# tum-vision/dvo_slam

Hardware: AMD Instinct MI355X
Metric: frame-pair alignments/s (640x480, 4-level pyramid) + finest-level HBM GB/s vs roofline (higher is better)
Workload: dtype f32 (Gram operands exact f16 hi + lo pairs on every level, f32 accumulate); 1 GPU; 1024 pairs (BASELINE config 4): independent 640x480 RGB-D frame pairs, seeds 0..1023, pair i on rank i mod 1, 4-level pyramid, FirstLevel=3, LastLevel=0, MaxIterationsPerLevel=100, Precision=5e-7, Mu=0; step = every rank re-ingests the raw planes of its shard from HBM (pyramids, sampling planes, point selection) and aligns it as one batch; the build of step k+1 (build stream) overlaps the match of; pairs=1024, pairs_per_gpu=1024, width=640, height=480, lanes=1 lane

## Files before the change

dvo_slam_amd/csrc/align_small.hip:

```cpp
#include "fast_sweep.h"
#include "launch.h"

namespace dvo_hip {

constexpr int kSmallCells = 5376;
constexpr int kSmallLoads = kSmallCells / kBlock;

__global__ __launch_bounds__(kBlock, 3) void k_sweep_small(
    const LevelGeom g, const PairPtrs* __restrict__ pairs, const PairState* __restrict__ states, int n_pairs,
    float* __restrict__ partials, float2* __restrict__ scratch, int blocks_per_xcd, int rows_per_wave, int* __restrict__ f16_range_flag) {
  const int tiles = g.tiles_x * g.tiles_y;
  const int total = tiles * n_pairs;
  const int xcd = blockIdx.x & 7, slot = blockIdx.x >> 3;
  const int item = xcd * blocks_per_xcd + slot;
  if (item >= total) return;
  const int pair = item / tiles, tile = item - pair * tiles;
  const PairState& st = states[pair];
  if (!st.active || st.level != g.level) return;
  const PairPtrs pp = pairs[pair];
  __shared__ __attribute__((aligned(16))) float slab[4][kSlabFloatsF16];
  __shared__ __attribute__((aligned(16))) float2 img[kSmallCells];
  __shared__ int counts[4];
  const int lane = threadIdx.x & 63, wave = __builtin_amdgcn_readfirstlane(threadIdx.x >> 6);
  const int n_px = g.w * g.h, plane_bytes = n_px * 8;
  const __amdgpu_buffer_rsrc_t refR = __builtin_amdgcn_make_buffer_rsrc(const_cast<float2*>(pp.refR), 0, plane_bytes, 0x00020000);
  const __amdgpu_buffer_rsrc_t curC = __builtin_amdgcn_make_buffer_rsrc(const_cast<float2*>(pp.curC), 0, plane_bytes, 0x00020000);
  const __amdgpu_buffer_rsrc_t resid = __builtin_amdgcn_make_buffer_rsrc(scratch + size_t(pair) * size_t(n_px), 0, plane_bytes, 0x00020000);

  const int pitch = g.w + 2, cells = pitch * (g.h + 2);
  {
    const float inv_pitch = 1.0f / float(pitch);
    f32x2 v[kSmallLoads];
#pragma unroll
    for (int j = 0; j < kSmallLoads; ++j) {
      const int c = min(int(threadIdx.x) + j * kBlock, cells - 1);
      int cy = int(float(c) * inv_pitch);
      int cx = c - cy * pitch;
      if (cx < 0) { cx += pitch; cy -= 1; }
      if (cx >= pitch) { cx -= pitch; cy += 1; }
      const int x = min(max(cx - 1, 0), g.w - 1), y = min(max(cy - 1, 0), g.h - 1);
      v[j] = __builtin_bit_cast(f32x2, __builtin_amdgcn_raw_buffer_load_b64(curC, (y * g.w + x) * 8, 0, 0));
    }
#pragma unroll
    for (int j = 0; j < kSmallLoads; ++j) {
      const int c = int(threadIdx.x) + j * kBlock;
      if (c < cells) img[c] = make_float2(v[j].x, v[j].y);
    }
  }

  float KT[12];
#pragma unroll
  for (int i = 0; i < 12; ++i) KT[i] = st.KT[i];
  const FastWeights wt(st);
  const FastRcpSource no_table = {__builtin_amdgcn_make_buffer_rsrc(static_cast<float*>(nullptr), 0, 0, 0x00020000), nullptr, 0};
  const unsigned gram_entries = kGramEntryTable.e[min(int(threadIdx.x), kNumAcc - 1)];
  const unsigned w2_bits = __builtin_bit_cast(unsigned, float(g.w - 2)), h2_bits = __builtin_bit_cast(unsigned, float(g.h - 2));
  const float inv_w = 1.0f / float(g.w);
  const float nanv = __builtin_nanf("");
  const int segments = (n_px + kTileW - 1) / kTileW;
  const int seg0 = tile * (kWavesPerBlock * rows_per_wave) + wave;
  float* my = slab[wave];
  f32x4 acc0 = {0.0f, 0.0f, 0.0f, 0.0f}, acc1 = {0.0f, 0.0f, 0.0f, 0.0f};
  int n_valid = 0;
  auto load_f = [&](int pixel) { return __builtin_bit_cast(float, __builtin_amdgcn_raw_buffer_load_b32(refR, pixel * 8 + 4, 0, 0)); };
  struct Ref {
    float z, i, left, right, up, down, tx, ty;
  };
  auto load_ref = [&](int seg) {
    const int pc = min(seg * kTileW + lane, n_px - 1);
    int row = int(float(pc) * inv_w);
    int col = pc - row * g.w;
    if (col < 0) { col += g.w; row -= 1; }
    if (col >= g.w) { col -= g.w; row += 1; }
    Ref r;
    const f32x2 zi = __builtin_bit_cast(f32x2, __builtin_amdgcn_raw_buffer_load_b64(refR, pc * 8, 0, 0));
    r.z = zi.x; r.i = zi.y;
    r.left = load_f(pc - (col > 0 ? 1 : 0));
    r.right = load_f(pc + (col < g.w - 1 ? 1 : 0));
    r.up = load_f(pc - (row > 0 ? g.w : 0));
    r.down = load_f(pc + (row < g.h - 1 ? g.w : 0));
    r.tx = g.tx[col];
    r.ty = g.ty[row];
    return r;
  };
  __syncthreads();
  Ref next = load_ref(min(seg0, segments - 1));
#pragma unroll 1
  for (int k = 0; k < rows_per_wave; ++k) {
    const int seg = seg0 + k * kWavesPerBlock;
    if (seg >= segments) break;
    const Ref ref = next;
    if (k + 1 < rows_per_wave) next = load_ref(min(seg + kWavesPerBlock, segments - 1));
    const int idx = seg * kTileW + lane;
    const bool in_image = idx < n_px;
    const float z = in_image ? ref.z : nanv;
    const float tx = ref.tx, ty = ref.ty;
    float u, v, qz;
    fast_project<0>(g, no_table, KT, fmaf(KT[0], tx, KT[2]), fmaf(KT[4], tx, KT[6]), fmaf(KT[8], tx, KT[10]), z, tx, ty, u, v, qz);
    const unsigned long long ok_mask = __builtin_amdgcn_ballot_w64(__builtin_bit_cast(unsigned, u) <= w2_bits) &
                                       __builtin_amdgcn_ballot_w64(__builtin_bit_cast(unsigned, v) <= h2_bits);
    const bool ok = __builtin_amdgcn_inverse_ballot_w64(ok_mask);
    const int u0 = int(u), v0 = int(v);
    FastRow r;
    r.z = z; r.i = ref.i;
    r.gx = ref.right - ref.left;
    r.gy = ref.down - ref.up;
    r.qz = qz;
    r.a1 = __builtin_amdgcn_fractf(u);
    r.b1 = __builtin_amdgcn_fractf(v);
    r.idx = v0 * pitch + u0;
    f32x2 P[4][4];
    {
      FastLdsCellPtr q = (FastLdsCellPtr)(img + (ok ? r.idx : 0));
#pragma unroll
      for (int rr = 0; rr < 4; ++rr)
#pragma unroll
        for (int cc = 0; cc < 4; ++cc)
          if ((rr == 1 || rr == 2) || (cc == 1 || cc == 2)) P[rr][cc] = q[rr * pitch + cc];
    }
    fast_row_tail<2, false, 0, false>(g, no_table, P, r, ok_mask, tx, ty, fmaf(tx, tx, 1.0f), wt, resid, in_image ? idx * 8 : 0x7ffffff8, 0, my, lane, acc0, acc1, n_valid);
  }

#pragma unroll
  for (int i = 0; i < 4; ++i) {
    my[((lane >> 4) * 4 + i) * 16 + (lane & 15)] = acc0[i];
    my[256 + ((lane >> 4) * 4 + i) * 16 + (lane & 15)] = acc1[i];
  }
  if (lane == 0) counts[wave] = n_valid;
  __syncthreads();
  fast_epilogue(slab, counts, gram_entries, partials + (size_t(pair) * tiles + tile) * kAccStride, f16_range_flag ? f16_range_flag + pair : nullptr);
}

bool small_sweep_takes(int w, int h) {
  return w % 2 == 0 && w >= 4 && h >= 4 && (w + 2) * (h + 2) <= kSmallCells;
}

void launch_sweep_small(hipStream_t s, int rows_per_wave, const LevelGeom& g, const PairPtrs* pairs, const PairState* states, int n_pairs,
                        float* partials, float2* scratch, int* f16_range_flag) {
  const int total = g.tiles_x * g.tiles_y * n_pairs;
  const int per_xcd = (total + 7) / 8;
  k_sweep_small<<<dim3(per_xcd * 8), dim3(kBlock), 0, s>>>(g, pairs, states, n_pairs, partials, scratch, per_xcd, rows_per_wave, f16_range_flag);
}

}
```

dvo_slam_amd/csrc/batch_policy.h:

```cpp
#pragma once

namespace dvo_hip {

struct BatchPolicy {
  int cus;
  explicit BatchPolicy(int compute_units) : cus(compute_units > 0 ? compute_units : 256) {}

  int resident_direct_max_pairs() const { return cus / 16; }
  bool resident_takes_coarse_levels(int n) const { return n * 4 <= cus; }
  bool resident_first_level_fits(int n) const { return n * 2 * 8 <= cus * 7; }
  bool taps_missing_prefers_first_level_only(int n) const { return n * 8 >= cus; }
  bool ingest_skips_taps(int n_frames) const { return n_frames * 8 >= cus; }

  bool short_gather_tiles(int n) const { return n >= cus; }
  int min_workgroups(int n) const { return n <= cus / 32 ? 2 * cus : n * 4 < cus ? 4 * cus : 8 * cus; }
  bool level_hand_over(int n) const { return n <= cus; }
  bool fused_loglik_on_large_levels(int n) const { return n >= 2 * cus; }
  int loglik_blocks(int n) const { return n >= cus ? 8 : n * 16 >= cus * 3 ? 16 : 32; }
  int deferred_ingest_lead(int n) const { return n * 4 >= cus * 3 ? 7 : 3; }
  bool finish_launch(int n) const { return !level_hand_over(n); }
  bool solver_two_waves(int n) const { return n > 2 * cus; }

  int small_level_tiles(int n) const {
    const int t = (3 * cus + n / 2) / (n > 0 ? n : 1);
    return t < 3 ? 3 : t > 8 ? 8 : t;
  }

  int defer_ingest_max_pairs() const { return cus; }
  int background_build_workgroups() const { return cus; }
};

}
```

dvo_slam_amd/csrc/capi.hip:

```cpp
#include <hip/hip_runtime.h>
#ifdef DVO_WITH_ROCTX
#include <rocprofiler-sdk-roctx/roctx.h>
#endif
#include <xmmintrin.h>

#include <algorithm>
#include <functional>
#include <climits>
#include <cstddef>
#include <cmath>
#include <cstdio>
#include <atomic>
#include <chrono>
#include <thread>
#include <condition_variable>
#include <cstdlib>
#include <cstring>
#include <mutex>
#include <string>
#include <vector>

#include "../../include/dvo_hip.h"
#include "device_types.h"
#include "batch_policy.h"
// ... 344 lines not shown
    dvo_hip_config cfg;
    bool keep_raw_copy;
  };
  std::vector<DeferredIngest> deferred;
  int opt_defer_ingest = 0;
  int opt_defer_ingest_pixels = 0;
  int opt_keep_raw_copy = 1;
  long long deferred_ingests = 0;
  int opt_build_workgroups = 0;
  int opt_stream_policy = 1;
  int opt_tail_speculation = 0;
  int opt_solver_waves = 0;
  int opt_ll_blocks = 0;
  int opt_compact_residuals = 1;
  int opt_gram_lo_parts = 1;
  int opt_min_workgroups = 0;
  int opt_condition_number = 0;
  int opt_fused_ll_pixels = 0;
  float last_sel_ithr = 0.0f, last_sel_dthr = 0.0f;
  int f32_gram_hold = 0;
  long long warmup_wait_us = 0;
  int opt_variant = 8;
  int opt_resident = -1;
  int opt_resident_rows = 0;
  int opt_resident_group = 0;
  int resident_timeouts = 0;
  long long resident_launches = 0;
  long long resident_levels = 0;
  long long host_ns[4] = {0, 0, 0, 0};
  long long host_batches = 0;
  std::chrono::steady_clock::time_point batch_entry;
  int opt_resident_flags = 0;
  int opt_sweep_tail = 0;
  long long tail_steps = 0;
  int opt_overlap_tails = 0;
  int opt_overlap_fraction = 8;
  int opt_tail_lists = 0;
  long long listed_steps = 0;
  long long overlapped_tails = 0;
  long long overlapped_steps = 0;
  long long tail_drains = 0;
  long long tail_wait_ns = 0;
  int opt_batch_groups = 0;
  bool is_twin = false;
  std::vector<GroupWorker*> group_workers;
  hipEvent_t roles_ready = nullptr;
  long long grouped_batches = 0;
  int opt_small_sweep = 0;
  int opt_small_tiles = 0;
  int opt_coarse = 0;
  int opt_coarse_pixels = 0;
  int opt_coarse_wgs = 0;
  long long coarse_launches = 0, coarse_levels = 0;
  int opt_deterministic = 0;
  int opt_ref_compat = 0;
  int opt_ref_order = 0;
  long long ref_order_passes = 0;
  DevBuf ref_order_planes;
  DevBuf rcp_table;
  int rcp_shift = 0;
  int rcp_packed = 0;
  int opt_resident_cooperative = 0;
  int compute_units = 0;
  std::vector<CameraGeom*> cameras;
  struct PooledBlock { void* p; size_t bytes; };
  std::vector<PooledBlock> frame_pool;
  size_t frame_pool_bytes = 0;
  static constexpr size_t kFramePoolMaxBytes = size_t(1) << 30;
  static constexpr size_t kFramePoolMaxBlocks = 64;
  Workspace ws[1];
  DevBuf misc, role_tbl_cur, role_tbl_ref, prep_tbl_cur, prep_tbl_ref;
  DevBuf sel_tbl_main, sel_tbl_build;
  unsigned long long sel_visits = 0;
  DevBuf lens_tbl;
  DevBuf graph_jobs, graph_outs;
  DevBuf rig_tbl;
  DevBuf colour_tbl, colour_stage;
  DevBuf map_tbl, map_stage;
  DevBuf render_tbl, render_zbuf, render_planes;
  hipEvent_t render_done = nullptr;
  static const int kTableSlots = 4;
  DevBuf build_tbl[kTableSlots];
  DevBuf* build_tbl_cur = nullptr;
  unsigned build_tbl_next = 0;
  PinnedRing tables;
  std::vector<dvo_hip_frame*> build_tbl_frames;
  hipStream_t build_stream = nullptr;
  static const int kBuildRing = 16;
  hipEvent_t build_events[kBuildRing] = {};
  unsigned long long build_seq = 0;
  unsigned long long main_waited_seq = 0;
  hipStream_t upload_stream = nullptr;
  hipEvent_t upload_done = nullptr;
  static const int kUploadRing = 3;
  DevBuf upload_buf[kUploadRing];
  unsigned long long upload_buf_seq[kUploadRing] = {};
  unsigned upload_next = 0;
  unsigned long long upload_waited_seq = 0;
};

namespace {
int flush_deferred(dvo_hip_context* ctx);
}

#define DVO_FLUSH_DEFERRED(ctx)                                     \
  do {                                                              \
// ... 277 lines not shown
  if (!ctx) return;
  (void)hipSetDevice(ctx->device);
  ctx->deferred.clear();
  destroy_group_workers(ctx);
  if (ctx->upload_stream) (void)hipStreamSynchronize(ctx->upload_stream);
  if (ctx->build_stream) (void)hipStreamSynchronize(ctx->build_stream);
  for (Workspace& w : ctx->ws) workspace_destroy(w);
  if (ctx->upload_done) (void)hipEventDestroy(ctx->upload_done);
  if (ctx->upload_stream) (void)hipStreamDestroy(ctx->upload_stream);
  for (hipEvent_t ev : ctx->build_events)
    if (ev) (void)hipEventDestroy(ev);
  if (ctx->build_stream) (void)hipStreamDestroy(ctx->build_stream);
  for (DevBuf& b : ctx->build_tbl) b.release();
  for (DevBuf* b : {&ctx->misc, &ctx->role_tbl_cur, &ctx->role_tbl_ref, &ctx->prep_tbl_cur, &ctx->prep_tbl_ref, &ctx->rcp_table, &ctx->ref_order_planes,
                    &ctx->sel_tbl_main, &ctx->sel_tbl_build, &ctx->lens_tbl, &ctx->rig_tbl, &ctx->graph_jobs, &ctx->graph_outs, &ctx->map_tbl, &ctx->map_stage, &ctx->colour_tbl, &ctx->colour_stage, &ctx->render_tbl, &ctx->render_zbuf, &ctx->render_planes}) b->release();
  if (ctx->render_done) (void)hipEventDestroy(ctx->render_done);
  for (DevBuf& b : ctx->upload_buf) b.release();
  for (const dvo_hip_context::PooledBlock& b : ctx->frame_pool) (void)hipFree(b.p);
  ctx->frame_pool.clear();
  ctx->tables.release();
  for (CameraGeom* c : ctx->cameras) {
    c->tables.release();
    delete c;
  }
  delete ctx;
}

const char* dvo_hip_last_error(const dvo_hip_context* ctx) { return ctx ? ctx->err.c_str() : g_create_error.c_str(); }

void* dvo_hip_context_stream(dvo_hip_context* ctx) { return ctx ? static_cast<void*>(ctx->stream) : nullptr; }

int dvo_hip_context_device(const dvo_hip_context* ctx) { return ctx ? ctx->device : -1; }

#include "capi_options.inc"

namespace {

int check_prepare_args(dvo_hip_context* ctx, int n_frames, dvo_hip_frame* const* frames, int role, const dvo_hip_config* cfg, const char* who) {
  if (!ctx || n_frames < 1 || !frames || !cfg || (role != DVO_HIP_ROLE_CURRENT && role != DVO_HIP_ROLE_REFERENCE))
    return fail(ctx, DVO_HIP_ERR_INVALID, who, "bad argument");
  if (cfg->first_level < cfg->last_level || cfg->last_level < 0 || cfg->first_level >= kMaxLevels)
    return fail(ctx, DVO_HIP_ERR_INVALID, who, "need 0 <= last_level <= first_level < DVO_HIP_MAX_LEVELS");
  for (int i = 0; i < n_frames; ++i) {
    if (!frames[i]) return fail(ctx, DVO_HIP_ERR_INVALID, who, "null entry");
    if (frames[i]->cam != frames[0]->cam || frames[i]->levels <= cfg->first_level)
      return fail(ctx, DVO_HIP_ERR_INVALID, who, "frames must share the camera and have first_level + 1 levels");
  }
  return DVO_HIP_OK;
}

int prepare_roles(dvo_hip_context* ctx, int n_frames, dvo_hip_frame* const* frames, int role, const dvo_hip_config* cfg) {
  const bool ref = role == DVO_HIP_ROLE_REFERENCE;
  int want[kMaxLevels];
  for (int l = 0; l < kMaxLevels; ++l) want[l] = l < frames[0]->cam->levels ? eager_current_flavor(ctx, frames[0]->cam, l, n_frames) : kCurAB;
  float ithr = ref ? cfg->intensity_derivative_threshold : 0.0f, dthr = ref ? cfg->depth_derivative_threshold : 0.0f;
  std::vector<dvo_hip_frame*> speculative;
  if (ref && (ithr < 0.0f || dthr < 0.0f)) {
    ithr = ctx->last_sel_ithr; dthr = ctx->last_sel_dthr;
    for (int i = 0; i < n_frames; ++i) {
      bool any = false;
      for (int l = cfg->last_level; l <= cfg->first_level; ++l) any |= frames[i]->lv[l].selected;
      if (!any) speculative.push_back(frames[i]);
    }
    if (speculative.empty()) return DVO_HIP_OK;
    n_frames = int(speculative.size());
    frames = speculative.data();
  }
  const int rc = ensure_roles(ctx, n_frames, frames, ref ? 1 : 0, cfg->last_level, cfg->first_level, ithr, dthr, true, want);
  if (rc != DVO_HIP_OK) return rc;
  DVO_HIP_TRY(ctx, hipGetLastError());
  return DVO_HIP_OK;
}

}

#include "capi_ingest.inc"
#include "capi_map.inc"
#include "capi_colour.inc"
#include "capi_graph.inc"

int dvo_hip_upload_wait(dvo_hip_context* ctx) {
  DVO_ENTER(ctx);
  if (!ctx) return DVO_HIP_ERR_INVALID;
  DVO_HIP_TRY(ctx, hipSetDevice(ctx->device));
  DVO_HIP_TRY(ctx, hipStreamSynchronize(ctx->upload_stream));
  return DVO_HIP_OK;
}

int dvo_hip_host_alloc(dvo_hip_context* ctx, size_t bytes, void** out) {
  DVO_LOCK(ctx);
  if (!ctx || !out || bytes == 0) return fail(ctx, DVO_HIP_ERR_INVALID, "host_alloc: bad argument");
  DVO_HIP_TRY(ctx, hipSetDevice(ctx->device));
  DVO_HIP_TRY(ctx, hipHostMalloc(out, bytes, hipHostMallocDefault));
  return DVO_HIP_OK;
}

void dvo_hip_host_free(dvo_hip_context* ctx, void* p) {
  DVO_LOCK(ctx);
  if (!p) return;
  if (ctx) (void)hipSetDevice(ctx->device);
  (void)hipHostFree(p);
}

int dvo_hip_frames_prepare(dvo_hip_context* ctx, int n_frames, dvo_hip_frame* const* frames, int role, const dvo_hip_config* cfg) {
  DVO_ENTER(ctx);
  const int rc = check_prepare_args(ctx, n_frames, frames, role, cfg, "frames_prepare");
  if (rc != DVO_HIP_OK) return rc;
// ... 212 lines not shown
  for (int i = 0; i < n_frames; ++i) {
    frames[i]->rig_on = false;
    frames[i]->rig = dvo_hip_depth_rig{};
  }
  return DVO_HIP_OK;
}

int dvo_hip_frame_set_level_selection(dvo_hip_context* ctx, dvo_hip_frame* frame, int level, const uint8_t* accepted) {
  DVO_ENTER(ctx);
  if (!ctx || !frame || level < 0 || level >= frame->levels) return fail(ctx, DVO_HIP_ERR_INVALID, "frame_set_level_selection: bad argument");
  if (!accepted) {
    FrameLevel& L = frame->lv[level];
    if (L.explicit_sel) L.selected = L.explicit_sel = L.q3 = false;
    return DVO_HIP_OK;
  }
  DVO_HIP_TRY(ctx, hipSetDevice(ctx->device));
  dvo_hip_frame* one[1] = {frame};
  int rc = wait_for_build(ctx, 1, one);
  if (rc == DVO_HIP_OK) rc = ensure_roles(ctx, 1, one, 0, level, level, 0.0f, 0.0f);
  if (rc != DVO_HIP_OK) return rc;
  FrameLevel& L = frame->lv[level];
  const size_t n = size_t(L.w) * L.h;
  DVO_HIP_TRY(ctx, ctx->misc.reserve(n));
  DVO_HIP_TRY(ctx, hipMemcpyAsync(ctx->misc.p, accepted, n, hipMemcpyHostToDevice, ctx->stream));
  DVO_HIP_TRY(ctx, hipMemsetAsync(frame->sel_count + level, 0, sizeof(int), ctx->stream));
  launch_pack_accepted(ctx->stream, L.A, ctx->misc.as<uint8_t>(), int(n), L.R, frame->sel_count + level);
  DVO_HIP_TRY(ctx, hipGetLastError());
  DVO_HIP_TRY(ctx, hipStreamSynchronize(ctx->stream));
  mark_selected(L, 0.0f, 0.0f);
  L.explicit_sel = true;
  return DVO_HIP_OK;
}

int dvo_hip_match_batch(dvo_hip_context* ctx, int n_pairs, dvo_hip_frame* const* references, dvo_hip_frame* const* currents,
                        const dvo_hip_config* cfg, dvo_hip_result* results, dvo_hip_level_stats* levels, int cap_levels,
                        dvo_hip_iteration_stats* iters, int cap_iters) {
  DVO_LOCK(ctx);
  if (!results) return fail(ctx, DVO_HIP_ERR_INVALID, "match: results is null");
  int rc = validate_batch(ctx, n_pairs, references, currents, cfg);
  if (rc != DVO_HIP_OK) return rc;
  if (cfg->use_initial_estimate)
    for (int i = 0; i < n_pairs; ++i)
      for (int k = 0; k < 16; ++k)
        if (!std::isfinite(results[i].transformation[k]))
          return fail(ctx, DVO_HIP_ERR_INVALID, "match: provided initialization is NaN (dense_tracking.cpp:139)");
  ctx->batch_entry = std::chrono::steady_clock::now();
  DVO_HIP_TRY(ctx, hipSetDevice(ctx->device));
  if (!ctx->deferred.empty()) {
    bool mine = false;
    for (int i = 0; i < n_pairs && !mine; ++i) mine = references[i]->deferred || currents[i]->deferred;
    if (mine) DVO_FLUSH_DEFERRED(ctx);
  }
  EffectiveVariantScope effective_variant_scope(ctx);
  rc = ensure_batch_roles(ctx, n_pairs, references, currents, cfg);
  if (rc != DVO_HIP_OK) return rc;

  const int groups = batch_groups_of(ctx, n_pairs);
  if (groups > 1) {
    rc = run_batch_grouped(ctx, groups, n_pairs, references, currents, cfg, results, levels, cap_levels, iters, cap_iters);
  } else {
    rc = run_batch(ctx, n_pairs, references, currents, cfg, results, levels, cap_levels, iters, cap_iters);
    if (rc != DVO_HIP_OK) ctx->err = ctx->ws[0].err;
  }
  if (!ctx->deferred.empty()) {
    const int rc_deferred = flush_deferred(ctx);
    if (rc == DVO_HIP_OK) rc = rc_deferred;
  }
  return rc;
}

int dvo_hip_match(dvo_hip_context* ctx, dvo_hip_frame* reference, dvo_hip_frame* current, const dvo_hip_config* cfg,
                  dvo_hip_result* result, dvo_hip_level_stats* levels, int cap_levels, dvo_hip_iteration_stats* iters, int cap_iters) {
  auto alone = [&]() {
    dvo_hip_frame* r[1] = {reference};
    dvo_hip_frame* c[1] = {current};
    return dvo_hip_match_batch(ctx, 1, r, c, cfg, result, levels, cap_levels, iters, cap_iters);
  };
  if (!ctx || !reference || !current || !cfg || !result || !ctx->opt_rendezvous) return alone();
  typedef dvo_hip_context::MatchRequest Request;
  constexpr int kExpectCalls = 16;
  auto same_config = [](const dvo_hip_config& a, const dvo_hip_config& b) {
    return a.first_level == b.first_level && a.last_level == b.last_level && a.max_iterations_per_level == b.max_iterations_per_level &&
           a.use_initial_estimate == b.use_initial_estimate && a.precision == b.precision && a.mu == b.mu &&
           a.intensity_derivative_threshold == b.intensity_derivative_threshold && a.depth_derivative_threshold == b.depth_derivative_threshold;
  };
  constexpr auto kPartnerWait = std::chrono::microseconds(60);
  Request me;
  me.reference = reference; me.current = current; me.cfg = cfg; me.result = result;
  me.levels = levels; me.cap_levels = cap_levels; me.iters = iters; me.cap_iters = cap_iters;
  Request* partner = nullptr;
  bool waiting = false;
  {
    std::lock_guard<std::mutex> lock(ctx->rendezvous_mutex);
    Request* w = ctx->rendezvous_waiting;
    if (w && w->current == current && same_config(*w->cfg, *cfg)) {
      partner = w;
      ctx->rendezvous_waiting = nullptr;
      w->state.store(1, std::memory_order_release);
      ctx->rendezvous_expect = kExpectCalls;
    } else if (ctx->rendezvous_busy_current == current) {
      ctx->rendezvous_expect = kExpectCalls;
    } else if (!w && ctx->rendezvous_expect > 0) {
      ctx->rendezvous_expect -= 1;
      ctx->rendezvous_waiting = &me;
      waiting = true;
    }
// ... 245 lines not shown
```

dvo_slam_amd/csrc/capi_frames.inc:

```
int stamp_build(dvo_hip_context* ctx, int n, dvo_hip_frame* const* frames) {
  const unsigned long long seq = ++ctx->build_seq;
  DVO_HIP_TRY(ctx, hipEventRecord(ctx->build_events[seq % dvo_hip_context::kBuildRing], ctx->build_stream));
  for (int i = 0; i < n; ++i) frames[i]->built_seq = seq;
  return DVO_HIP_OK;
}

int wait_for_ticket(dvo_hip_context* ctx, unsigned long long need, bool upload) {
  unsigned long long& waited = upload ? ctx->upload_waited_seq : ctx->main_waited_seq;
  hipStream_t stream = upload ? ctx->upload_stream : ctx->stream;
  if (need <= waited) return DVO_HIP_OK;
  const unsigned long long oldest_live = ctx->build_seq >= dvo_hip_context::kBuildRing ? ctx->build_seq - dvo_hip_context::kBuildRing + 1 : 1;
  const unsigned long long use = need < oldest_live ? oldest_live : need;
  DVO_HIP_TRY(ctx, hipStreamWaitEvent(stream, ctx->build_events[use % dvo_hip_context::kBuildRing], 0));
  waited = use;
  return DVO_HIP_OK;
}

int wait_for_build(dvo_hip_context* ctx, int n, dvo_hip_frame* const* frames) {
  unsigned long long need = 0;
  for (int i = 0; i < n; ++i)
    if (frames[i] && frames[i]->built_seq > need) need = frames[i]->built_seq;
  return wait_for_ticket(ctx, need, false);
}

// ... 83 lines not shown
  }
  std::vector<float> host;
  char* base = c->tables.as<char>();
  size_t off = 0;
  for (int l = 0; l < levels; ++l) {
    const float fx = c->K[l][0], fy = c->K[l][1], ox = c->K[l][2], oy = c->K[l][3];
    host.resize(size_t(c->w[l]) + c->h[l]);
    for (int x = 0; x < c->w[l]; ++x) host[x] = (float(x) - ox) / fx;
    for (int y = 0; y < c->h[l]; ++y) host[c->w[l] + y] = (float(y) - oy) / fy;
    c->tx[l] = reinterpret_cast<float*>(base + off);
    off += align_up(size_t(c->w[l]) * 4, 256);
    c->ty[l] = reinterpret_cast<float*>(base + off);
    off += align_up(size_t(c->h[l]) * 4, 256);
    e = hipMemcpy(c->tx[l], host.data(), size_t(c->w[l]) * 4, hipMemcpyHostToDevice);
    if (e == hipSuccess) e = hipMemcpy(c->ty[l], host.data() + c->w[l], size_t(c->h[l]) * 4, hipMemcpyHostToDevice);
    if (e != hipSuccess) {
      c->tables.release();
      delete c;
      ctx->err = std::string("hipMemcpy(camera tables): ") + hipGetErrorString(e);
      return DVO_HIP_ERR_HIP;
    }
  }
  ctx->cameras.push_back(c);
  *out = c;
  return DVO_HIP_OK;
}

void level_tiles(int w, int h, int rows_per_wave, bool linear, int* tiles_x, int* tiles_y) {
  const int th = kWavesPerBlock * rows_per_wave;
  if (linear) {
    const int segments = (w * h + kTileW - 1) / kTileW;
    *tiles_x = 1;
    *tiles_y = (segments + th - 1) / th;
  } else {
    *tiles_x = (w + kTileW - 1) / kTileW;
    *tiles_y = (h + th - 1) / th;
  }
}

bool level_uses_fast_window(const dvo_hip_context* ctx, int w, int h) {
  return ctx->opt_variant >= 8 && fast_sweep_takes_width(w) && w < 32768 && h < 32768;
}

bool level_uses_small(const dvo_hip_context* ctx, int w, int h);

bool level_is_linear(const dvo_hip_context* ctx, int w) { return ctx->opt_variant >= 5 && w % kTileW != 0 && !level_uses_fast_window(ctx, w, 4); }

bool level_uses_window(const dvo_hip_context* ctx, int w, int h) {
  return (ctx->opt_variant >= 6 && w % kTileW == 0 && w < 32768 && h < 32768) || level_uses_fast_window(ctx, w, h);
}

bool level_uses_small(const dvo_hip_context* ctx, int w, int h) {
  return ctx->opt_small_sweep && ctx->opt_variant >= 8 && !ctx->opt_ref_compat && !ctx->opt_ref_order && !level_uses_window(ctx, w, h) && level_is_linear(ctx, w) && small_sweep_takes(w, h);
}

LevelGeom make_geom(const dvo_hip_context* ctx, const CameraGeom* cam, int level, int rows_per_wave) {
  LevelGeom g;
  g.w = cam->w[level]; g.h = cam->h[level];
  g.fx = cam->K[level][0]; g.fy = cam->K[level][1]; g.ox = cam->K[level][2]; g.oy = cam->K[level][3];
  g.wi_x = 0.5f * g.fx / 255.0f; g.wi_y = 0.5f * g.fy / 255.0f;
  g.half_wi_x = 0.5f * g.wi_x; g.half_wi_y = 0.5f * g.wi_y; g.half_fx = 0.5f * g.fx; g.half_fy = 0.5f * g.fy;
  g.tx = cam->tx[level]; g.ty = cam->ty[level];
  g.level = level;
  g.pair_list = nullptr;
  g.skip_flags = nullptr;
  g.linear = level_is_linear(ctx, g.w) ? 1 : 0;
  level_tiles(g.w, g.h, rows_per_wave, g.linear != 0, &g.tiles_x, &g.tiles_y);
  g.rcp_table = ctx->opt_ref_compat ? ctx->rcp_table.as<float>() : nullptr;
  g.rcp_shift = ctx->rcp_shift;
  g.rcp_packed = ctx->opt_ref_compat == 1 ? ctx->rcp_packed : 0;
  g.gram_hi_j = !ctx->opt_gram_lo_parts && !ctx->opt_deterministic && !ctx->opt_ref_compat && ctx->opt_variant == 8 && size_t(g.w) * g.h >= 150000 ? 1 : 0;
  g.small = level_uses_small(ctx, g.w, g.h) ? 1 : 0;
  g.compact = ctx->opt_compact_residuals && !ctx->opt_ref_order && ctx->opt_variant >= 8 && rows_per_wave == 4 && fast_sweep_supports(g) ? 1 : 0;
  return g;
}

int pick_rows_per_wave(const dvo_hip_context* ctx, const CameraGeom* cam, int level, int n_pairs) {
  if (level_uses_window(ctx, cam->w[level], cam->h[level])) return 4;
  if (level_uses_small(ctx, cam->w[level], cam->h[level]) && ctx->opt_rows_per_wave == 0) {
    const int tiles = ctx->opt_small_tiles > 0 ? ctx->opt_small_tiles : BatchPolicy(ctx->compute_units).small_level_tiles(n_pairs);
    const int segments = (cam->w[level] * cam->h[level] + kTileW - 1) / kTileW;
    const int rows = (segments + kWavesPerBlock * tiles - 1) / (kWavesPerBlock * tiles);
    return rows < 1 ? 1 : rows;
  }
  if (ctx->opt_deterministic) return ctx->opt_rows_per_wave > 0 ? ctx->opt_rows_per_wave : 4;
  if (ctx->opt_rows_per_wave > 0) return ctx->opt_rows_per_wave;
  if (BatchPolicy(ctx->compute_units).short_gather_tiles(n_pairs) && ctx->opt_variant >= 7) return 2;
  const int candidates[4] = {8, 4, 2, 1};
  const size_t enough = ctx->opt_min_workgroups > 0 ? size_t(ctx->opt_min_workgroups) : size_t(BatchPolicy(ctx->compute_units).min_workgroups(n_pairs));
  for (int r : candidates) {
    int tx, ty;
    level_tiles(cam->w[level], cam->h[level], r, level_is_linear(ctx, cam->w[level]), &tx, &ty);
    if (size_t(tx) * ty * n_pairs >= enough) return r;
  }
  return 1;
}

static bool width_may_use_window(int w) { return w % kTileW == 0 || fast_sweep_takes_width(w); }
static bool level_may_read_plane_c(int w, int h) { return width_may_use_window(w) || small_sweep_takes(w, h); }

int frame_alloc(dvo_hip_context* ctx, int w, int h, const float K[4], int levels, dvo_hip_frame** out, size_t* raw_off) {
  if (!ctx) return DVO_HIP_ERR_INVALID;
  if (w < 4 || h < 4 || levels < 1 || levels > kMaxLevels || (w >> (levels - 1)) < 2 || (h >> (levels - 1)) < 2)
    return fail(ctx, DVO_HIP_ERR_INVALID, "frame_create: bad width/height/levels");
  DVO_HIP_TRY(ctx, hipSetDevice(ctx->device));
  const CameraGeom* cam = nullptr;
// ... 19 lines not shown
  for (size_t k = 0; k < ctx->frame_pool.size(); ++k)
    if (ctx->frame_pool[k].bytes == total) {
      f->pool.p = ctx->frame_pool[k].p;
      f->pool.bytes = total;
      ctx->frame_pool_bytes -= total;
      ctx->frame_pool.erase(ctx->frame_pool.begin() + long(k));
      break;
    }
  if (!f->pool.p) e = f->pool.reserve(total);
  if (e != hipSuccess) {
    delete f;
    ctx->err = std::string("hipMalloc(frame): ") + hipGetErrorString(e);
    return DVO_HIP_ERR_HIP;
  }
  char* base = f->pool.as<char>();
  for (int l = 0; l < levels; ++l) {
    FrameLevel& L = f->lv[l];
    L.w = cam->w[l]; L.h = cam->h[l];
    L.I = reinterpret_cast<float*>(base + offs[l][0]);
    L.Z = reinterpret_cast<float*>(base + offs[l][1]);
    L.A = reinterpret_cast<float4*>(base + offs[l][2]);
    L.B = reinterpret_cast<float2*>(base + offs[l][3]);
    L.R = reinterpret_cast<float2*>(base + offs[l][4]);
    L.C = level_may_read_plane_c(cam->w[l], cam->h[l]) ? reinterpret_cast<float2*>(base + offs[l][5]) : nullptr;
  }
  f->sel_count = reinterpret_cast<int*>(base + cnt_off);
  *out = f;
  return DVO_HIP_OK;
}

void fill_build_ptrs(dvo_hip_frame* f, FrameBuildPtrs& p) {
  p.grey = nullptr;
  p.raw = nullptr;
  p.keep_grey = nullptr;
  p.keep_raw = nullptr;
  for (int l = 0; l < f->levels; ++l) {
    p.I[l] = f->lv[l].I; p.Z[l] = f->lv[l].Z; p.A[l] = f->lv[l].A; p.B[l] = f->lv[l].B; p.R[l] = f->lv[l].R; p.C[l] = f->lv[l].C;
  }
  for (int l = f->levels; l < kMaxLevels; ++l) p.C[l] = nullptr;
  p.sel_count = f->sel_count;
  p.colour = nullptr;
  p.colour_pitch = 0;
  p.colour_format = 0;
  p.depth_f32 = nullptr;
  p.depth_pitch = 0;
  p.keep_planes = 0;
}

uint16_t* staging_depth(dvo_hip_frame* f) { return f->pool.as<uint16_t>(); }
uint8_t* staging_grey(dvo_hip_frame* f) { return f->pool.as<uint8_t>() + size_t(f->lv[0].w) * f->lv[0].h * 2; }

bool aligned_to(const void* p, size_t a) { return reinterpret_cast<uintptr_t>(p) % a == 0; }

int eager_current_flavor(const dvo_hip_context* ctx, const CameraGeom* cam, int level, int n_frames) {
  if (level_uses_small(ctx, cam->w[level], cam->h[level]))
    return BatchPolicy(ctx->compute_units).resident_first_level_fits(n_frames) ? (kCurAB | kCurC) : kCurC;
  if (!level_uses_window(ctx, cam->w[level], cam->h[level])) return kCurAB;
  return BatchPolicy(ctx->compute_units).ingest_skips_taps(n_frames) ? kCurC : (kCurAB | kCurC);
}

int rectify_frames(dvo_hip_context* ctx, int n, dvo_hip_frame* const* frames, const IngestSource& src) {
  const CameraGeom* cam = frames[0]->cam;
  const dvo_hip_lens& lens = frames[0]->lens;
  const bool image_f32 = src.format == DVO_HIP_PIXEL_F32, depth_f32 = src.depth_format == DVO_HIP_DEPTH_F32;
  std::vector<RectifyPtrs> host(static_cast<size_t>(n));
  for (int i = 0; i < n; ++i) host[i] = RectifyPtrs{src.planes[i], src.depth[i], frames[i]->lv[0].I, frames[i]->lv[0].Z};
  RectifyArgs a;
  a.map = lens_prepare(cam->K0, lens.K_raw, lens.D);
  a.w = cam->w[0];
  a.h = cam->h[0];
  a.image_pitch = int(src.pitch);
  a.depth_pitch = depth_f32 ? int(src.depth_pitch) : cam->w[0] * 2;
  a.red_first = pixel_red_first(src.format) ? 1 : 0;
  a.rectify_depth = lens.rectify_depth;
  a.depth_scale = src.depth_scale;
  const size_t bytes = host.size() * sizeof(RectifyPtrs);
  DVO_HIP_TRY(ctx, ctx->lens_tbl.reserve(bytes));
  DVO_HIP_TRY(ctx, ctx->tables.upload(ctx->build_stream, ctx->lens_tbl.p, host.data(), bytes));
  launch_rectify(ctx->build_stream, ctx->lens_tbl.as<RectifyPtrs>(), n, a, image_f32 ? kChF32 : pixel_channels(src.format), depth_f32,
                 ctx->opt_build_workgroups, ctx->opt_stream_policy != 0);
  DVO_HIP_TRY(ctx, hipGetLastError());
  return DVO_HIP_OK;
}

int register_frames(dvo_hip_context* ctx, int n, dvo_hip_frame* const* frames, const IngestSource& src) {
  const CameraGeom* cam = frames[0]->cam;
  const bool depth_f32 = src.depth_format == DVO_HIP_DEPTH_F32;
  std::vector<DepthRigPtrs> host(static_cast<size_t>(n));
  for (int i = 0; i < n; ++i) host[i] = DepthRigPtrs{src.depth[i], frames[i]->lv[0].Z};
  DepthRigArgs a;
  a.map = depth_rig_prepare(cam->K0, frames[0]->rig);
  a.w = cam->w[0];
  a.h = cam->h[0];
  a.depth_pitch = depth_f32 ? int(src.depth_pitch) : cam->w[0] * 2;
  a.depth_scale = src.depth_scale;
  const size_t bytes = host.size() * sizeof(DepthRigPtrs);
  DVO_HIP_TRY(ctx, ctx->rig_tbl.reserve(bytes));
  DVO_HIP_TRY(ctx, ctx->tables.upload(ctx->build_stream, ctx->rig_tbl.p, host.data(), bytes));
  launch_depth_register(ctx->build_stream, ctx->rig_tbl.as<DepthRigPtrs>(), n, a, depth_f32, ctx->opt_build_workgroups, ctx->opt_stream_policy != 0);
  DVO_HIP_TRY(ctx, hipGetLastError());
  return DVO_HIP_OK;
}

int frames_build(dvo_hip_context* ctx, int n, dvo_hip_frame* const* frames, const IngestSource* src, int role = -1, float ithr = 0.0f,
                 float dthr = 0.0f, bool keep_raw_copy = true) {
  Range range("build");
  const CameraGeom* cam = frames[0]->cam;
  const int levels = frames[0]->levels;
  const bool rig = src != nullptr && frames[0]->rig_on;
  std::vector<const void*> reg_planes;
  IngestSource registered;
  if (rig) {
    const int rc = register_frames(ctx, n, frames, *src);
    if (rc != DVO_HIP_OK) return rc;
    reg_planes.resize(size_t(n));
    for (int i = 0; i < n; ++i) reg_planes[size_t(i)] = frames[i]->lv[0].Z;
    registered = IngestSource{src->planes, src->format, src->pitch, reg_planes.data(), 1.0f, DVO_HIP_DEPTH_F32, size_t(cam->w[0]) * 4};
    src = &registered;
  }
  const bool lens = src != nullptr && frames[0]->lens_on;
  std::vector<const void*> rect_planes;
  IngestSource rectified;
  if (lens) {
    const int rc = rectify_frames(ctx, n, frames, *src);
    if (rc != DVO_HIP_OK) return rc;
    rect_planes.resize(2 * size_t(n));
    for (int i = 0; i < n; ++i) {
      rect_planes[size_t(i)] = frames[i]->lv[0].I;
      rect_planes[size_t(n) + i] = frames[i]->lv[0].Z;
    }
    const size_t row = size_t(cam->w[0]) * 4;
    rectified = IngestSource{rect_planes.data(), DVO_HIP_PIXEL_F32, row, rect_planes.data() + n, 1.0f, DVO_HIP_DEPTH_F32, row};
    src = &rectified;
  }
  std::vector<FrameBuildPtrs> host(n);
  bool wide = cam->w[0] % 4 == 0;
  const bool from_raw = src != nullptr;
  const bool image_f32 = from_raw && src->format == DVO_HIP_PIXEL_F32;
  const bool depth_f32 = from_raw && src->depth_format == DVO_HIP_DEPTH_F32;
  const bool colour = from_raw && src->format != 0 && !image_f32;
  const int channels = image_f32 ? kChF32 : colour ? pixel_channels(src->format) : 0;
  if (image_f32) wide = cam->w[0] % 2 == 0;
  const float depth_scale = from_raw ? src->depth_scale : 0.0f;
  const int flavor0 = eager_current_flavor(ctx, cam, 0, n);
  for (int i = 0; i < n; ++i) {
    dvo_hip_frame* f = frames[i];
    fill_build_ptrs(f, host[i]);
    for (int l = 0; l < levels; ++l) {
      f->lv[l].cur_have = 0;
      f->lv[l].selected = false;
      f->lv[l].explicit_sel = false;
      f->lv[l].q3 = false;
    }
    f->raw0 = from_raw;
    f->raw_copy = false;
    f->depth_scale = depth_scale;
    if (!from_raw) continue;
    if (role == 0) f->lv[0].cur_have = flavor0;
    if (role == 1) mark_selected(f->lv[0], ithr, dthr);
    if (colour || image_f32) {
      host[i].colour = static_cast<const uint8_t*>(src->planes[i]);
      host[i].colour_pitch = int(src->pitch);
      host[i].colour_format = src->format;
    } else {
      host[i].grey = static_cast<const uint8_t*>(src->planes[i]);
      host[i].colour_pitch = int(src->pitch);
    }
    if (depth_f32) {
      host[i].depth_f32 = static_cast<const float*>(src->depth[i]);
      host[i].depth_pitch = int(src->depth_pitch);
      if (role < 0 || (role == 1 && keep_raw_copy)) {
        host[i].keep_planes = lens ? 0 : 1;
        f->raw0 = false;
      }
      wide = wide && f32_strips_aligned(host[i].depth_f32, src->depth_pitch) &&
             (image_f32 ? f32_strips_aligned(host[i].colour, src->pitch)
                        : colour ? colour_strips_aligned(host[i].colour, src->pitch, channels) : aligned_to(host[i].grey, 2) && src->pitch % 2 == 0);
      continue;
    }
    host[i].raw = static_cast<const uint16_t*>(src->depth[i]);
    const bool in_place = !colour && host[i].raw == staging_depth(f) && host[i].grey == staging_grey(f);
    if (in_place) {
      f->raw_copy = true;
    } else if (role < 0 || (role == 1 && keep_raw_copy)) {
      host[i].keep_grey = staging_grey(f);
      host[i].keep_raw = staging_depth(f);
      f->raw_copy = true;
    }
    wide = wide && (colour ? colour_strips_aligned(host[i].colour, src->pitch, channels) : aligned_to(host[i].grey, 4)) &&
           aligned_to(host[i].raw, 8) && aligned_to(staging_grey(f), 4);
  }
  hipStream_t bs = ctx->build_stream;
  int slot = ctx->tables.holder(ctx->build_tbl, dvo_hip_context::kTableSlots, bs, host.data(), size_t(n) * sizeof(FrameBuildPtrs));
  if (slot < 0) slot = int(ctx->build_tbl_next++ % dvo_hip_context::kTableSlots);
  DevBuf& build_tbl = ctx->build_tbl[slot];
  DVO_HIP_TRY(ctx, build_tbl.reserve(size_t(n) * sizeof(FrameBuildPtrs)));
  DVO_HIP_TRY(ctx, ctx->tables.upload(bs, build_tbl.p, host.data(), size_t(n) * sizeof(FrameBuildPtrs)));
  const FrameBuildPtrs* tbl = build_tbl.as<FrameBuildPtrs>();
  ctx->build_tbl_frames.assign(frames, frames + n);
  ctx->build_tbl_cur = &build_tbl;
  int built = 1;
  if (from_raw) {
    built = levels < 4 ? levels : 4;
    int c_levels = 0;
    const bool strips = ingest_strips_supports(cam->w[0], wide, image_f32);
    if (role == 0 && strips) {
      for (int l = 1; l < built; ++l)
        if (eager_current_flavor(ctx, cam, l, n) & kCurC) c_levels |= 1 << l;
      for (int i = 0; i < n; ++i)
        for (int l = 1; l < built; ++l)
          if ((c_levels >> l & 1) && frames[i]->lv[l].C) frames[i]->lv[l].cur_have |= kCurC;
    }
    launch_build_from_raw(bs, tbl, n, depth_scale, cam->w[0], cam->h[0], levels, role, strips, ithr, dthr, ctx->opt_build_workgroups, flavor0, c_levels,
                          channels, ctx->opt_stream_policy != 0, depth_f32);
    if (role == 1) {
      const int rc = apply_selection(ctx, bs, n, frames, 0, 0, ctx->opt_build_workgroups);
      if (rc != DVO_HIP_OK) return rc;
    }
    if (strips) ctx->strip_ingests += n;
    if (colour) ctx->colour_ingests += n;
    if (depth_f32) ctx->f32_ingests += n;
    if (lens) ctx->lens_ingests += n;
    if (rig) ctx->depth_registrations += n;
  }
  for (int l = built; l < levels; ++l) launch_pyr_down(bs, tbl, n, l, cam->w[l - 1], cam->h[l - 1]);
  DVO_HIP_TRY(ctx, hipGetLastError());
  return stamp_build(ctx, n, frames);
}

int ensure_roles(dvo_hip_context* ctx, int n, dvo_hip_frame* const* frames, int role, int l0, int l1, float ithr, float dthr, bool eager = false,
                 const int* cur_want = nullptr) {
  const CameraGeom* cam = frames[0]->cam;
  const size_t slice = size_t(n) * sizeof(FrameBuildPtrs);
  DevBuf& table = eager ? (role == 0 ? ctx->prep_tbl_cur : ctx->prep_tbl_ref) : (role == 0 ? ctx->role_tbl_cur : ctx->role_tbl_ref);
  hipStream_t stream = eager ? ctx->build_stream : ctx->stream;
  const int cap = eager ? ctx->opt_build_workgroups : 0;
  const bool stream_nt = eager && ctx->opt_stream_policy != 0;
  struct Lack { int miss; bool need; };
  auto lack_of = [&](const dvo_hip_frame* f, int l) -> Lack {
    const FrameLevel& L = f->lv[l];
    if (role != 0) return Lack{0, !ref_ready(L, ithr, dthr)};
    const int want = (cur_want ? cur_want[l] : kCurAB) & (L.C ? (kCurAB | kCurC) : kCurAB);
    return Lack{want & ~L.cur_have, (want & ~L.cur_have) != 0};
  };
  if (l0 == 0)
    for (int i = 0; i < n; ++i) {
      const dvo_hip_frame* f = frames[i];
      if (!f->raw0 || f->lv[0].cur_have != 0 || f->raw_copy) continue;
      if (lack_of(f, 0).need) return fail(ctx, DVO_HIP_ERR_INVALID, "frame has neither sampling planes nor a raw copy at level 0");
    }
  bool launched = false;
  int uploads = 0;
  auto upload = [&](const std::vector<FrameBuildPtrs>& host, const FrameBuildPtrs** tbl, bool plane_pointers_only = true) -> int {
    if (plane_pointers_only && eager && ctx->build_tbl_cur && int(host.size()) == n && ctx->build_tbl_frames.size() == size_t(n) &&
        std::equal(frames, frames + n, ctx->build_tbl_frames.begin())) {
      *tbl = ctx->build_tbl_cur->as<FrameBuildPtrs>();
      return DVO_HIP_OK;
    }
    constexpr int kSlices = 4 * kMaxLevels;
    if (uploads == kSlices) {
      DVO_HIP_TRY(ctx, hipStreamSynchronize(stream));
      uploads = 0;
    }
    DVO_HIP_TRY(ctx, table.reserve(slice * kSlices));
    FrameBuildPtrs* up = reinterpret_cast<FrameBuildPtrs*>(table.as<char>() + slice * uploads++);
    DVO_HIP_TRY(ctx, ctx->tables.upload(stream, up, host.data(), host.size() * sizeof(FrameBuildPtrs)));
    *tbl = up;
    return DVO_HIP_OK;
  };
  if (l1 > l0) {
    LevelSpan span = level_span(l0, l1, cam->w, cam->h);
    bool uniform = n <= 64;
    for (int i = 0; i < n && uniform; ++i)
      for (int j = 0; j < i && uniform; ++j) uniform = frames[i] != frames[j];
    for (int l = l0; l <= l1 && uniform; ++l) {
      int miss_all = -1;
      for (int i = 0; i < n && uniform; ++i) {
        const dvo_hip_frame* f = frames[i];
        const Lack lack = lack_of(f, l);
        uniform = lack.need && !(l == 0 && f->raw0) && (role == 1 || f->lv[l].cur_have == 0) && (miss_all < 0 || lack.miss == miss_all);
        miss_all = lack.miss;
      }
      span.flavor[l] = miss_all;
    }
    if (uniform) {
      std::vector<FrameBuildPtrs> host(n);
      for (int i = 0; i < n; ++i) fill_build_ptrs(frames[i], host[i]);
      const FrameBuildPtrs* tbl = nullptr;
      const int rc = upload(host, &tbl);
      if (rc != DVO_HIP_OK) return rc;
      launch_derive_levels(stream, tbl, n, span, role, ithr, dthr, cap);
      for (int i = 0; i < n; ++i)
        for (int l = l0; l <= l1; ++l) {
          FrameLevel& L = frames[i]->lv[l];
          if (role == 0) L.cur_have |= span.flavor[l];
          else mark_selected(L, ithr, dthr);
        }
      if (role == 1) {
        const int rc = apply_selection(ctx, stream, n, frames, l0, l1, cap);
        if (rc != DVO_HIP_OK) return rc;
      }
      if (eager) {
        const int rc2 = stamp_build(ctx, n, frames);
        if (rc2 != DVO_HIP_OK) return rc2;
      }
      DVO_HIP_TRY(ctx, hipGetLastError());
      return DVO_HIP_OK;
    }
  }
  for (int l = l0; l <= l1; ++l) {
    std::vector<FrameBuildPtrs> from_planes[4], from_raw[4], ab_from_c, c_from_a, ref_from_c;
    std::vector<dvo_hip_frame*> ref_from_ab, selected;
    float raw_scale = 0.0f;
    bool deferred = false;
    for (int i = 0; i < n; ++i) {
      dvo_hip_frame* f = frames[i];
      FrameLevel& L = f->lv[l];
      const Lack lack = lack_of(f, l);
      const int miss = lack.miss;
      if (!lack.need) continue;
      FrameBuildPtrs p;
      fill_build_ptrs(f, p);
      if (l == 0 && f->raw0) {
        if (role == 0 && (L.cur_have & kCurC)) {
          ab_from_c.push_back(p);
        } else if (role == 0 && (L.cur_have & kCurAB)) {
          c_from_a.push_back(p);
        } else if (role == 1 && (L.cur_have & kCurAB)) {
          ref_from_ab.push_back(f);
        } else if (role == 1 && (L.cur_have & kCurC)) {
          ref_from_c.push_back(p);
        } else if (f->raw_copy && (raw_scale == 0.0f || f->depth_scale == raw_scale)) {
          raw_scale = f->depth_scale;
          p.grey = staging_grey(f);
          p.raw = staging_depth(f);
          from_raw[miss].push_back(p);
        } else if (f->raw_copy) {
          deferred = true;
          continue;
        } else {
          return fail(ctx, DVO_HIP_ERR_INVALID, "frame has neither sampling planes nor a raw copy at level 0");
        }
      } else {
        from_planes[miss].push_back(p);
      }
      if (role == 0) {
        L.cur_have |= miss;
      } else {
        mark_selected(L, ithr, dthr);
        selected.push_back(f);
      }
    }
    const FrameBuildPtrs* tbl = nullptr;
    for (int miss = 0; miss < 4; ++miss) {
      if (!from_planes[miss].empty()) {
        int rc = upload(from_planes[miss], &tbl);
        if (rc != DVO_HIP_OK) return rc;
        if (role == 0) launch_derive_current(stream, tbl, int(from_planes[miss].size()), l, cam->w[l], cam->h[l], cap, miss, stream_nt);
        else launch_derive_reference(stream, tbl, int(from_planes[miss].size()), l, cam->w[l], cam->h[l], ithr, dthr, cap, stream_nt);
        launched = true;
      }
      if (!from_raw[miss].empty()) {
        int rc = upload(from_raw[miss], &tbl, false);
        if (rc != DVO_HIP_OK) return rc;
        launch_build_from_raw(stream, tbl, int(from_raw[miss].size()), raw_scale, cam->w[0], cam->h[0], 1, role,
                              ingest_strips_supports(cam->w[0], true), ithr, dthr, cap, miss, 0, 0, stream_nt);
        launched = true;
      }
    }
    const struct { std::vector<FrameBuildPtrs>* list; int mode; } conversions[3] = {{&ab_from_c, 0}, {&c_from_a, 1}, {&ref_from_c, 2}};
    for (const auto& c : conversions) {
      if (c.list->empty()) continue;
      int rc = upload(*c.list, &tbl);
      if (rc != DVO_HIP_OK) return rc;
      launch_from_current_plane(stream, tbl, int(c.list->size()), l, cam->w[l], cam->h[l], c.mode, ithr, dthr, cap);
      launched = true;
    }
    for (dvo_hip_frame* f : ref_from_ab) {
      FrameLevel& L = f->lv[0];
      DVO_HIP_TRY(ctx, hipMemsetAsync(f->sel_count, 0, sizeof(int), stream));
      launch_select_pack(stream, L.A, L.B, L.w * L.h, ithr, dthr, L.R, f->sel_count, nullptr);
      launched = true;
    }
    if (!selected.empty()) {
      const int rc = apply_selection(ctx, stream, int(selected.size()), selected.data(), l, l, cap);
      if (rc != DVO_HIP_OK) return rc;
    }
    if (deferred) {
      if (eager && launched) {
        const int rc = stamp_build(ctx, n, frames);
        if (rc != DVO_HIP_OK) return rc;
      }
      DVO_HIP_TRY(ctx, hipStreamSynchronize(stream));
      return ensure_roles(ctx, n, frames, role, l0, l1, ithr, dthr, eager, cur_want);
    }
  }
  if (eager && launched) {
    const int rc = stamp_build(ctx, n, frames);
    if (rc != DVO_HIP_OK) return rc;
  }
// ... 5 lines not shown
```

dvo_slam_amd/csrc/capi_groups.inc:

```
void mirror_options(const dvo_hip_context* from, dvo_hip_context* to) {
#define DVO_MIRROR(f) to->f = from->f
  DVO_MIRROR(opt_rows_per_wave); DVO_MIRROR(opt_iters_per_sync); DVO_MIRROR(opt_tail_speculation); DVO_MIRROR(opt_solver_waves);
  DVO_MIRROR(opt_ll_blocks); DVO_MIRROR(opt_compact_residuals); DVO_MIRROR(opt_gram_lo_parts); DVO_MIRROR(opt_min_workgroups);
  DVO_MIRROR(opt_condition_number); DVO_MIRROR(opt_fused_ll_pixels); DVO_MIRROR(opt_variant); DVO_MIRROR(opt_resident);
  DVO_MIRROR(opt_resident_rows); DVO_MIRROR(opt_resident_group); DVO_MIRROR(opt_resident_flags); DVO_MIRROR(opt_resident_cooperative);
  DVO_MIRROR(opt_sweep_tail); DVO_MIRROR(opt_coarse); DVO_MIRROR(opt_coarse_pixels); DVO_MIRROR(opt_coarse_wgs);
  DVO_MIRROR(opt_deterministic); DVO_MIRROR(opt_ref_order); DVO_MIRROR(opt_small_sweep); DVO_MIRROR(opt_small_tiles); DVO_MIRROR(compute_units);
  DVO_MIRROR(opt_overlap_tails); DVO_MIRROR(opt_overlap_fraction); DVO_MIRROR(opt_tail_lists); DVO_MIRROR(opt_defer_ingest_pixels);
#undef DVO_MIRROR
}

void group_worker_main(GroupWorker* gw) {
  (void)hipSetDevice(gw->twin->device);
  for (;;) {
    std::unique_lock<std::mutex> lock(gw->m);
    gw->cv.wait(lock, [&] { return gw->has_job || gw->quit; });
    if (gw->quit) return;
    gw->has_job = false;
    lock.unlock();
    dvo_hip_context* t = gw->twin;
    t->batch_entry = std::chrono::steady_clock::now();
    int rc = DVO_HIP_OK;
    if (hipStreamWaitEvent(t->stream, gw->after, 0) != hipSuccess) {
      t->err = "match: a pair group could not wait for the batch's role planes";
      rc = DVO_HIP_ERR_HIP;
    }
    if (rc == DVO_HIP_OK) {
      rc = run_batch(t, gw->n, gw->refs, gw->curs, gw->cfg, gw->results, gw->levels, gw->cap_levels, gw->iters, gw->cap_iters);
      if (rc != DVO_HIP_OK) t->err = t->ws[0].err;
    }
    lock.lock();
    gw->rc = rc;
    gw->done = true;
    lock.unlock();
    gw->cv.notify_all();
  }
}

int batch_groups_of(const dvo_hip_context* ctx, int n) {
  if (ctx->is_twin || ctx->opt_ref_compat || ctx->opt_deterministic || ctx->opt_ref_order) return 1;
  return ctx->opt_batch_groups > 1 ? std::min(ctx->opt_batch_groups, std::max(1, n / 64)) : 1;
}

int ensure_group_workers(dvo_hip_context* ctx, int groups) {
  while (int(ctx->group_workers.size()) < groups - 1) {
    dvo_hip_context* twin = nullptr;
    const int rc = dvo_hip_context_create(ctx->device, &twin);
    if (rc != DVO_HIP_OK) return fail(ctx, rc, "match: could not create a pair group's context");
    twin->is_twin = true;
    GroupWorker* gw = new GroupWorker();
    gw->twin = twin;
    gw->thread = std::thread(group_worker_main, gw);
    ctx->group_workers.push_back(gw);
  }
  if (!ctx->roles_ready) DVO_HIP_TRY(ctx, hipEventCreateWithFlags(&ctx->roles_ready, hipEventDisableTiming));
  return DVO_HIP_OK;
}

void destroy_group_workers(dvo_hip_context* ctx) {
  for (GroupWorker* gw : ctx->group_workers) {
    {
// ... 57 lines not shown
```

dvo_slam_amd/csrc/capi_options.inc:

```
int dvo_hip_get_counter(dvo_hip_context* ctx, const char* key, long long* value) {
  if (!ctx || !key || !value) return DVO_HIP_ERR_INVALID;
  std::unique_lock<std::recursive_mutex> guard(ctx->mutex);
  if (std::strcmp(key, "resident_launches") == 0) *value = ctx->resident_launches;
  else if (std::strcmp(key, "resident_levels") == 0) *value = ctx->resident_levels;
  else if (std::strcmp(key, "resident_timeouts") == 0) *value = ctx->resident_timeouts;
  else if (std::strcmp(key, "grouped_batches") == 0) *value = ctx->grouped_batches;
  else if (std::strcmp(key, "compute_units") == 0) *value = BatchPolicy(ctx->compute_units).cus;
  else if (std::strcmp(key, "defer_ingest_max_pairs") == 0) *value = BatchPolicy(ctx->compute_units).defer_ingest_max_pairs();
  else if (std::strcmp(key, "background_build_workgroups") == 0) *value = BatchPolicy(ctx->compute_units).background_build_workgroups();
  else if (std::strcmp(key, "tail_steps") == 0) {
    *value = ctx->tail_steps;
    for (const GroupWorker* gw : ctx->group_workers) *value += gw->twin->tail_steps;
  }
  else if (std::strcmp(key, "overlapped_tails") == 0) *value = ctx->overlapped_tails;
  else if (std::strcmp(key, "overlapped_steps") == 0) *value = ctx->overlapped_steps;
  else if (std::strcmp(key, "listed_steps") == 0) *value = ctx->listed_steps;
  else if (std::strcmp(key, "tail_drains") == 0) *value = ctx->tail_drains;
  else if (std::strcmp(key, "tail_wait_us") == 0) *value = ctx->tail_wait_ns / 1000;
  else if (std::strcmp(key, "ref_order_passes") == 0) *value = ctx->ref_order_passes;
  else if (std::strcmp(key, "coarse_launches") == 0) *value = ctx->coarse_launches;
  else if (std::strcmp(key, "coarse_levels") == 0) *value = ctx->coarse_levels;
  else if (std::strcmp(key, "window_fallbacks") == 0) {
    unsigned long long v = 0;
    if (ctx->ws[0].win_fallbacks.p) {
      DVO_HIP_TRY(ctx, hipStreamSynchronize(ctx->stream));
      DVO_HIP_TRY(ctx, hipMemcpy(&v, ctx->ws[0].win_fallbacks.p, sizeof(v), hipMemcpyDeviceToHost));
    }
    *value = (long long)v;
  }
  else if (std::strcmp(key, "strip_ingests") == 0) *value = ctx->strip_ingests;
  else if (std::strcmp(key, "colour_ingests") == 0) *value = ctx->colour_ingests;
  else if (std::strcmp(key, "f32_ingests") == 0) *value = ctx->f32_ingests;
  else if (std::strcmp(key, "lens_ingests") == 0) *value = ctx->lens_ingests;
  else if (std::strcmp(key, "depth_registrations") == 0) *value = ctx->depth_registrations;
  else if (std::strcmp(key, "depth_rig_table_bytes") == 0) *value = (long long)ctx->rig_tbl.bytes;
  else if (std::strcmp(key, "map_inserts") == 0) *value = ctx->map_inserts;
  else if (std::strcmp(key, "map_removes") == 0) *value = ctx->map_removes;
  else if (std::strcmp(key, "map_rehashes") == 0) *value = ctx->map_rehashes;
  else if (std::strcmp(key, "map_renders") == 0) *value = ctx->map_renders;
  else if (std::strcmp(key, "map_points") == 0) *value = ctx->map_points;
  else if (std::strcmp(key, "map_dropped") == 0) *value = ctx->map_dropped;
  else if (std::strcmp(key, "graph_resident_solves") == 0) *value = ctx->graph_resident_solves;
  else if (std::strcmp(key, "warmup_wait_us") == 0) *value = ctx->warmup_wait_us;
  else if (std::strcmp(key, "rendezvous_pairs") == 0) {
    std::lock_guard<std::mutex> lock(ctx->rendezvous_mutex);
    *value = ctx->rendezvous_pairs;
  }
  else if (std::strcmp(key, "f16_range_repeats") == 0) *value = ctx->f16_range_repeats;
  else if (std::strcmp(key, "table_uploads_skipped") == 0) *value = ctx->tables.skipped;
  else if (std::strcmp(key, "deferred_ingests") == 0) *value = ctx->deferred_ingests;
  else if (std::strcmp(key, "host_batches") == 0) *value = ctx->host_batches;
  else if (std::strcmp(key, "host_ns_prepare") == 0) *value = ctx->host_ns[0];
  else if (std::strcmp(key, "host_ns_enqueue") == 0) *value = ctx->host_ns[1];
  else if (std::strcmp(key, "host_ns_wait") == 0) *value = ctx->host_ns[2];
  else if (std::strcmp(key, "host_ns_finish") == 0) *value = ctx->host_ns[3];
  else return fail(ctx, DVO_HIP_ERR_INVALID, "unknown counter");
  return DVO_HIP_OK;
}

int dvo_hip_set_option(dvo_hip_context* ctx, const char* key, int value) {
  DVO_LOCK(ctx);
  if (!ctx || !key) return DVO_HIP_ERR_INVALID;
  if (std::strcmp(key, "rows_per_wave") == 0) {
    if (value != 0 && value != 1 && value != 2 && value != 4 && value != 8 && value != 16)
      return fail(ctx, DVO_HIP_ERR_INVALID, "rows_per_wave must be 0,1,2,4,8,16");
    ctx->opt_rows_per_wave = value;
    return DVO_HIP_OK;
  }
  if (std::strcmp(key, "iters_per_sync") == 0) {
    if (value < 0) return fail(ctx, DVO_HIP_ERR_INVALID, "iters_per_sync must be >= 0");
    ctx->opt_iters_per_sync = value;
    return DVO_HIP_OK;
  }
  if (std::strcmp(key, "variant") == 0) {
// ... 34 lines not shown
    ctx->opt_resident = value;
    return DVO_HIP_OK;
  }
  if (std::strcmp(key, "small_sweep") == 0) {
    if (value != 0 && value != 1) return fail(ctx, DVO_HIP_ERR_INVALID, "small_sweep must be 0 or 1");
    ctx->opt_small_sweep = value;
    return DVO_HIP_OK;
  }
  if (std::strcmp(key, "small_tiles") == 0) {
    if (value < 0 || value > 32) return fail(ctx, DVO_HIP_ERR_INVALID, "small_tiles must be 0 (by batch size) .. 32");
    ctx->opt_small_tiles = value;
    return DVO_HIP_OK;
  }
  if (std::strcmp(key, "batch_groups") == 0) {
    if (value < 0 || value > 4) return fail(ctx, DVO_HIP_ERR_INVALID, "batch_groups must be 0 or 1 (one group) .. 4");
    ctx->opt_batch_groups = value;
    return DVO_HIP_OK;
  }
  if (std::strcmp(key, "solver_occupancy") == 0) {
    if (value != 0 && value != 3) return fail(ctx, DVO_HIP_ERR_INVALID, "solver_occupancy must be 0 or 3");
    g_solver_occupancy = value;
    return DVO_HIP_OK;
  }
  if (std::strcmp(key, "sweep_tail") == 0) {
    if (value < 0 || value > 2) return fail(ctx, DVO_HIP_ERR_INVALID, "sweep_tail must be 0, 1 (the whole step in the sweep's tail) or 2 (its wide half; the serial half in a launch behind it)");
    ctx->opt_sweep_tail = value;
    return DVO_HIP_OK;
  }
  if (std::strcmp(key, "overlap_tails") == 0) {
    if (value < 0 || value > 1) return fail(ctx, DVO_HIP_ERR_INVALID, "overlap_tails must be 0 (off) or 1 (a level's stragglers finish beside the next level)");
    ctx->opt_overlap_tails = value;
    return DVO_HIP_OK;
  }
  if (std::strcmp(key, "defer_ingest_pixels") == 0) {
    if (value < 0) return fail(ctx, DVO_HIP_ERR_INVALID, "defer_ingest_pixels must be >= 0");
    ctx->opt_defer_ingest_pixels = value;
    return DVO_HIP_OK;
  }
  if (std::strcmp(key, "tail_lists") == 0) {
    if (value < 0 || value > 1) return fail(ctx, DVO_HIP_ERR_INVALID, "tail_lists must be 0 or 1 (the last steps of a costly level are launched over the list of pairs still on it)");
    ctx->opt_tail_lists = value;
    return DVO_HIP_OK;
  }
  if (std::strcmp(key, "overlap_fraction") == 0) {
    if (value < 2 || value > 64) return fail(ctx, DVO_HIP_ERR_INVALID, "overlap_fraction must be in [2, 64]: a level's tail is split off once at most 1/value of the pairs is on it");
    ctx->opt_overlap_fraction = value;
    return DVO_HIP_OK;
  }
  if (std::strcmp(key, "coarse") == 0) {
    if (value < 0 || value > 1) return fail(ctx, DVO_HIP_ERR_INVALID, "coarse must be 0 (off) or 1 (whenever the levels admit it)");
    ctx->opt_coarse = value;
    return DVO_HIP_OK;
  }
  if (std::strcmp(key, "coarse_pixels") == 0) {
    if (value < 0) return fail(ctx, DVO_HIP_ERR_INVALID, "coarse_pixels must be >= 0");
    ctx->opt_coarse_pixels = value;
    return DVO_HIP_OK;
  }
  if (std::strcmp(key, "coarse_workgroups") == 0) {
    if (value != 0 && value != 3 && value != 4) return fail(ctx, DVO_HIP_ERR_INVALID, "coarse_workgroups must be 0, 3 or 4");
    ctx->opt_coarse_wgs = value;
    return DVO_HIP_OK;
  }
  if (std::strcmp(key, "resident_flags") == 0) {
    ctx->opt_resident_flags = value;
    return DVO_HIP_OK;
  }
  if (std::strcmp(key, "resident_cooperative") == 0) {
    ctx->opt_resident_cooperative = value != 0;
    return DVO_HIP_OK;
  }
  if (std::strcmp(key, "resident_rows") == 0) {
    if (value < 0) return fail(ctx, DVO_HIP_ERR_INVALID, "resident_rows must be >= 0");
    ctx->opt_resident_rows = value;
    return DVO_HIP_OK;
  }
  if (std::strcmp(key, "resident_group") == 0) {
    if (value < 0 || value > kResidentMaxGroup || (value & (value - 1))) return fail(ctx, DVO_HIP_ERR_INVALID, "resident_group must be 0 or a power of two <= 64");
    ctx->opt_resident_group = value;
    return DVO_HIP_OK;
  }
  if (std::strcmp(key, "build_workgroups") == 0) {
    if (value < 0) return fail(ctx, DVO_HIP_ERR_INVALID, "build_workgroups must be >= 0");
    ctx->opt_build_workgroups = value;
    return DVO_HIP_OK;
  }
  if (std::strcmp(key, "tail_speculation") == 0) {
    if (value < 0) return fail(ctx, DVO_HIP_ERR_INVALID, "tail_speculation must be >= 0");
    ctx->opt_tail_speculation = value;
    return DVO_HIP_OK;
  }
  if (std::strcmp(key, "solver_waves") == 0) {
    if (value != 0 && value != 2 && value != 4) return fail(ctx, DVO_HIP_ERR_INVALID, "solver_waves must be 0, 2 or 4");
    ctx->opt_solver_waves = value;
    return DVO_HIP_OK;
  }
  if (std::strcmp(key, "ll_blocks") == 0) {
    if (value < 0 || value > kLlBlocksPerPair) return fail(ctx, DVO_HIP_ERR_INVALID, "ll_blocks must be 0..32");
    ctx->opt_ll_blocks = value;
    return DVO_HIP_OK;
  }
  if (std::strcmp(key, "gram_lo_parts") == 0) {
    if (value != 0 && value != 1) return fail(ctx, DVO_HIP_ERR_INVALID, "gram_lo_parts must be 0 or 1");
    ctx->opt_gram_lo_parts = value;
    return DVO_HIP_OK;
  }
// ... 50 lines not shown
```

dvo_slam_amd/csrc/capi_schedule.inc:

```
struct BatchPlan {
  int n = 0, nlev = 0, cap_levels = 0, cap_iters = 0;
  SolverParams prm;
  const CameraGeom* cam = nullptr;
  std::vector<int> rpw;
  std::vector<LevelGeom> geom;
  PairPtrs* pair_ptrs = nullptr;
  std::vector<PairPtrs> host_ptrs;
  int coarse_levels = 0;
  bool ref_order = false;
};

int validate_batch(dvo_hip_context* ctx, int n, dvo_hip_frame* const* refs, dvo_hip_frame* const* curs, const dvo_hip_config* cfg) {
  if (!ctx || n < 1 || !refs || !curs || !cfg) return fail(ctx, DVO_HIP_ERR_INVALID, "match: null argument");
  if (cfg->first_level < cfg->last_level || cfg->last_level < 0 || cfg->first_level >= kMaxLevels)
    return fail(ctx, DVO_HIP_ERR_INVALID, "match: need 0 <= last_level <= first_level < DVO_HIP_MAX_LEVELS");
  if (cfg->max_iterations_per_level < 1) return fail(ctx, DVO_HIP_ERR_INVALID, "match: max_iterations_per_level < 1");
  const int need_levels = cfg->first_level + 1;
  const CameraGeom* cam = refs[0] ? refs[0]->cam : nullptr;
  for (int i = 0; i < n; ++i) {
    if (!refs[i] || !curs[i]) return fail(ctx, DVO_HIP_ERR_INVALID, "match: null frame");
    if (refs[i]->levels < need_levels || curs[i]->levels < need_levels)
      return fail(ctx, DVO_HIP_ERR_INVALID, "match: frame pyramid has fewer levels than first_level + 1");
    if (refs[i]->cam != cam || curs[i]->cam != cam)
      return fail(ctx, DVO_HIP_ERR_INVALID, "match: all frames of a batch must share size and intrinsics");
  }
  return DVO_HIP_OK;
}

void make_plan(const dvo_hip_context* ctx, const CameraGeom* cam, const dvo_hip_config* cfg, int n, BatchPlan& bp) {
  const int need_levels = cfg->first_level + 1;
  bp.n = n;
  bp.cam = cam;
  bp.nlev = cfg->first_level - cfg->last_level + 1;
  bp.cap_levels = bp.nlev;
  bp.cap_iters = bp.nlev * cfg->max_iterations_per_level;
  bp.prm.max_iterations = cfg->max_iterations_per_level;
  bp.prm.first_level = cfg->first_level;
  bp.prm.last_level = cfg->last_level;
  bp.prm.use_initial_estimate = cfg->use_initial_estimate;
  bp.prm.precision = cfg->precision;
  bp.prm.mu = cfg->mu;
  bp.ref_order = ctx->opt_ref_order != 0;
  bp.prm.cap_iters = bp.cap_iters;
  bp.prm.cap_levels = bp.cap_levels;
  bp.prm.max_points_level0 = cam->w0 * cam->h0;
  bp.prm.want_condition_number = ctx->opt_condition_number;
  bp.prm.record_prefilled = 0;
  bp.rpw.assign(need_levels, 1);
  bp.geom.resize(need_levels);
  for (int l = cfg->last_level; l <= cfg->first_level; ++l) {
    bp.rpw[l] = pick_rows_per_wave(ctx, cam, l, n);
    bp.geom[l] = make_geom(ctx, cam, l, bp.rpw[l]);
  }
}

int resident_levels_of(const dvo_hip_context* ctx, const dvo_hip_config* cfg, const CameraGeom* cam, int n, bool taps_missing);
bool window_taps_missing(const dvo_hip_context* ctx, const dvo_hip_config* cfg, int n, dvo_hip_frame* const* curs);

int ref_order_planes(dvo_hip_context* ctx, int n, dvo_hip_frame* const* refs, const dvo_hip_config* cfg) {
  const bool edit = ctx->opt_ref_order != 0;
  std::vector<RefOrderPlane> host;
  for (int i = 0; i < n; ++i)
    for (int l = cfg->last_level; l <= cfg->first_level; ++l) {
      FrameLevel& L = refs[i]->lv[l];
      if (L.q3 == edit) continue;
      L.q3 = edit;
      RefOrderPlane p;
      p.R = L.R;
      p.count = refs[i]->sel_count + l;
      p.saved = ref_order_saved_slot(refs[i]->sel_count, l);
      p.npx = L.w * L.h;
      p.pad = 0;
      host.push_back(p);
    }
  if (host.empty()) return DVO_HIP_OK;
  DVO_HIP_TRY(ctx, ctx->ref_order_planes.reserve(host.size() * sizeof(RefOrderPlane)));
  DVO_HIP_TRY(ctx, ctx->tables.upload(ctx->stream, ctx->ref_order_planes.p, host.data(), host.size() * sizeof(RefOrderPlane)));
  if (edit) launch_ref_order_drop_last(ctx->stream, ctx->ref_order_planes.as<RefOrderPlane>(), int(host.size()));
  else launch_ref_order_restore(ctx->stream, ctx->ref_order_planes.as<RefOrderPlane>(), int(host.size()));
  DVO_HIP_TRY(ctx, hipGetLastError());
  return DVO_HIP_OK;
}

int ensure_batch_roles(dvo_hip_context* ctx, int n, dvo_hip_frame* const* refs, dvo_hip_frame* const* curs, const dvo_hip_config* cfg,
                       bool launch_path_only = false) {
  Range range("build");
  ctx->last_sel_ithr = cfg->intensity_derivative_threshold;
  ctx->last_sel_dthr = cfg->depth_derivative_threshold;
  int rc = wait_for_build(ctx, n, refs);
  if (rc == DVO_HIP_OK) rc = wait_for_build(ctx, n, curs);
  if (rc != DVO_HIP_OK) return rc;
  const CameraGeom* cam = curs[0]->cam;
  const int resident = launch_path_only ? 0 : resident_levels_of(ctx, cfg, cam, n, window_taps_missing(ctx, cfg, n, curs));
  int want[kMaxLevels];
  for (int l = 0; l < kMaxLevels; ++l)
    want[l] = l > cfg->first_level - resident || l >= cam->levels || !(level_uses_window(ctx, cam->w[l], cam->h[l]) || level_uses_small(ctx, cam->w[l], cam->h[l])) ? kCurAB : kCurC;
  rc = ensure_roles(ctx, n, curs, 0, cfg->last_level, cfg->first_level, 0.0f, 0.0f, false, want);
  if (rc == DVO_HIP_OK)
    rc = ensure_roles(ctx, n, refs, 1, cfg->last_level, cfg->first_level, cfg->intensity_derivative_threshold, cfg->depth_derivative_threshold);
  if (rc == DVO_HIP_OK) rc = ref_order_planes(ctx, n, refs, cfg);
  return rc;
}

int prepare_buffers(Workspace& w, const dvo_hip_config* cfg, dvo_hip_frame* const* refs, dvo_hip_frame* const* curs, BatchPlan& bp,
                    bool upload_table = true) {
  const int n = bp.n, need_levels = cfg->first_level + 1;
  size_t max_tiles = 1;
  for (int l = cfg->last_level; l <= cfg->first_level; ++l) max_tiles = std::max(max_tiles, size_t(bp.geom[l].tiles_x) * bp.geom[l].tiles_y);
  size_t npx = 0;
  for (int l = cfg->last_level; l <= cfg->first_level; ++l) npx = std::max(npx, residual_entries(bp.geom[l]));
  DVO_WS_TRY(w, w.states.reserve(size_t(n) * sizeof(PairState)));

  DVO_WS_TRY(w, w.partials.reserve(size_t(n) * max_tiles * kAccStride * sizeof(float)));
  DVO_WS_TRY(w, w.scratch.reserve(size_t(n) * npx * sizeof(float2)));
  DVO_WS_TRY(w, w.ll_partials.reserve(size_t(n) * kLlBlocksPerPair * sizeof(double)));
  DVO_WS_TRY(w, w.lvl_stats.reserve(size_t(n) * bp.cap_levels * sizeof(dvo_hip_level_stats)));
  DVO_WS_TRY(w, w.it_stats.reserve(size_t(n) * bp.cap_iters * sizeof(dvo_hip_iteration_stats)));
  DVO_WS_TRY(w, w.results.reserve(size_t(n) * sizeof(dvo_hip_result)));
  DVO_WS_TRY(w, w.pair_sums.reserve(size_t(n) * kPairSumsStride * sizeof(double)));
  if (bp.ref_order) {
    int max_h = 1;
    for (int l = cfg->last_level; l <= cfg->first_level; ++l) max_h = std::max(max_h, bp.geom[l].h);
    DVO_WS_TRY(w, w.ref_rows.reserve(size_t(n) * max_h * sizeof(RefOrderSeg)));
    DVO_WS_TRY(w, w.ref_pairs.reserve(size_t(n) * sizeof(RefOrderPair)));
  }
  DVO_WS_TRY(w, w.t_init.reserve(size_t(n) * 16 * sizeof(double)));
  DVO_WS_TRY(w, w.counters.reserve(size_t(bp.cap_iters + 8 + kResidentErrorWords) * sizeof(unsigned long long) + align_up(size_t(n) * sizeof(int), 8)));
  if (!w.win_fallbacks.p) {
    DVO_WS_TRY(w, w.win_fallbacks.reserve(64));
    DVO_WS_TRY(w, hipMemsetAsync(w.win_fallbacks.p, 0, 64, w.stream));
  }
  if (w.f16_range_words < size_t(n)) {
    if (w.f16_range_flag) {
      DVO_WS_TRY(w, hipStreamSynchronize(w.stream));
      (void)hipHostFree(w.f16_range_flag);
      w.f16_range_flag = nullptr;
      w.f16_range_words = 0;
    }
    const size_t words = std::max<size_t>(64, size_t(n));
    DVO_WS_TRY(w, hipHostMalloc(reinterpret_cast<void**>(&w.f16_range_flag), words * sizeof(int), hipHostMallocCoherent | hipHostMallocMapped));
    std::memset(w.f16_range_flag, 0, words * sizeof(int));
    w.f16_range_words = words;
  }
  std::vector<PairPtrs>& host = bp.host_ptrs;
  host.assign(size_t(n) * need_levels, PairPtrs());
  for (int l = cfg->last_level; l <= cfg->first_level; ++l)
    for (int i = 0; i < n; ++i) {
      PairPtrs& p = host[size_t(l) * n + i];
      p.refR = refs[i]->lv[l].R;
// ... 140 lines not shown
ResidentPlan plan_resident(const dvo_hip_context* ctx, const dvo_hip_config* cfg, const BatchPlan& bp, bool taps_missing) {
  ResidentPlan rp;
  if (ctx->opt_resident == 0 || ctx->opt_deterministic || ctx->opt_ref_order) return rp;
  const int cus = ctx->compute_units > 0 ? ctx->compute_units : 256;
  const BatchPolicy policy(ctx->compute_units);
  const bool first_level_only = ctx->opt_resident < 0 && ctx->opt_resident_group == 0 &&
                                (!policy.resident_takes_coarse_levels(bp.n) || (policy.taps_missing_prefers_first_level_only(bp.n) && taps_missing));
  if (first_level_only && (!policy.resident_first_level_fits(bp.n) || level_uses_window(ctx, bp.cam->w[cfg->first_level], bp.cam->h[cfg->first_level]))) return rp;
  int group = 1;
  while (group * 2 <= kResidentMaxGroup && bp.n * group * 2 <= cus) group *= 2;
  if (ctx->opt_resident_group > 0) group = std::min(group, ctx->opt_resident_group);
  if (first_level_only) {
    group = 1;
    while (group * 2 <= kResidentMaxGroup && bp.n * group * 2 * 8 <= cus * 7) group *= 2;
  }
  rp.group = group;
  const int rows_max = ctx->opt_resident_rows > 0 ? ctx->opt_resident_rows : kResidentRowsDefault;
  for (int level = cfg->first_level; level >= cfg->last_level; --level) {
    const int segments = (bp.cam->w[level] * bp.cam->h[level] + kTileW - 1) / kTileW;
    const int rows = (segments + group * kResidentSweepers - 1) / (group * kResidentSweepers);
    if (ctx->opt_resident != 1 && rows > rows_max) break;
    if (first_level_only && rp.levels == 1) break;
    if (size_t(bp.cam->w[level]) * bp.cam->h[level] >= (size_t(1) << 24)) break;
    rp.levels += 1;
  }
  static const bool trace_plan = std::getenv("DVO_HIP_TRACE_PLAN") != nullptr;
  if (trace_plan)
    std::fprintf(stderr, "plan_resident: %d pairs, taps missing %d -> %s, %d workgroup(s) per pair, %d level(s) resident\n", bp.n, int(taps_missing),
                 first_level_only ? "first level only" : "coarse levels", rp.group, rp.levels);
  rp.direct = rp.levels == cfg->first_level - cfg->last_level + 1 && bp.n <= policy.resident_direct_max_pairs() &&
              size_t(bp.n) * bp.cap_iters * sizeof(dvo_hip_iteration_stats) <= kResidentDirectStatsBytes;
  return rp;
}

constexpr int kCoarseMaxPixels = 160 * 120;

void plan_coarse(const dvo_hip_context* ctx, const dvo_hip_config* cfg, BatchPlan& bp, const ResidentPlan& rp) {
  bp.coarse_levels = 0;
  if (ctx->opt_coarse == 0 || rp.levels > 0 || ctx->opt_variant != 8 || ctx->opt_ref_order) return;
  const int max_pixels = ctx->opt_coarse_pixels > 0 ? ctx->opt_coarse_pixels : kCoarseMaxPixels;
  for (int level = cfg->first_level; level >= cfg->last_level; --level) {
    if (bp.cam->w[level] * bp.cam->h[level] > max_pixels) break;
    const bool window_level = level_uses_window(ctx, bp.cam->w[level], bp.cam->h[level]);
    const int rpw = window_level ? 4 : kCoarseRowsPerWave;
    if (!window_level && ctx->opt_rows_per_wave > 0 && ctx->opt_rows_per_wave != rpw) break;
    const LevelGeom g = make_geom(ctx, bp.cam, level, rpw);
    if (!coarse_kernel_takes(g, window_level)) break;
    bp.rpw[level] = rpw;
    bp.geom[level] = g;
    bp.coarse_levels += 1;
  }
}

ResidentPlan plan_paths(const dvo_hip_context* ctx, const dvo_hip_config* cfg, BatchPlan& bp, bool taps_missing) {
  ResidentPlan rp = plan_resident(ctx, cfg, bp, taps_missing);
  if (ctx->opt_coarse == 1) {
    const ResidentPlan none;
    plan_coarse(ctx, cfg, bp, none);
    if (bp.coarse_levels > 0) rp = none;
  } else {
    plan_coarse(ctx, cfg, bp, rp);
  }
  return rp;
}

int resident_levels_of(const dvo_hip_context* ctx, const dvo_hip_config* cfg, const CameraGeom* cam, int n, bool taps_missing) {
  BatchPlan bp;
  make_plan(ctx, cam, cfg, n, bp);
  return plan_paths(ctx, cfg, bp, taps_missing).levels;
}

int run_resident(dvo_hip_context* ctx, Workspace& w, const dvo_hip_config* cfg, const BatchPlan& bp, const ResidentPlan& rp,
                 const double* tinit, bool want_stats) {
  hipStream_t s = w.stream;
  ResidentArgs args;
  std::memset(&args, 0, sizeof(args));
  for (int l = cfg->last_level; l <= cfg->first_level; ++l) args.geom[l] = bp.geom[l];
  args.pair_ptrs = bp.pair_ptrs;
  args.states = w.states.as<PairState>();
  args.levels = w.lvl_stats.as<dvo_hip_level_stats>();
  args.iters = w.it_stats.as<dvo_hip_iteration_stats>();
  args.T_init = w.t_init.as<double>();
  args.scratch = w.scratch.as<float2>();
  args.error_word = w.host_status + w.resident_error_word;
  args.prm = bp.prm;
  args.n_pairs = bp.n;
  args.group = rp.group;
  args.first_level = cfg->first_level;
  args.last_level = cfg->first_level - rp.levels + 1;
  args.flags = ctx->opt_resident_flags;
  args.results = args.last_level == cfg->last_level ? w.results.as<dvo_hip_result>() : nullptr;
  if (bp.n <= kResidentInline) {
    args.use_inline = 1;
    for (int l = cfg->last_level; l <= cfg->first_level; ++l)
      for (int i = 0; i < bp.n; ++i) args.inline_ptrs[l * bp.n + i] = bp.host_ptrs[size_t(l) * bp.n + i];
    std::memcpy(args.inline_T, tinit, size_t(bp.n) * 16 * sizeof(double));
  }
  if (rp.direct) {
    DVO_WS_TRY(w, w.direct_results.reserve(size_t(bp.n) * sizeof(dvo_hip_result)));
    DVO_WS_TRY(w, w.direct_done.reserve(64));
    args.results = w.direct_results.as<dvo_hip_result>();
    args.done_word = w.direct_done.as<int>();
    *static_cast<volatile int*>(args.done_word) = 0;
    if (want_stats) {
      DVO_WS_TRY(w, w.direct_levels.reserve(size_t(bp.n) * bp.cap_levels * sizeof(dvo_hip_level_stats)));
      DVO_WS_TRY(w, w.direct_iters.reserve(size_t(bp.n) * bp.cap_iters * sizeof(dvo_hip_iteration_stats)));
      args.host_levels = w.direct_levels.as<dvo_hip_level_stats>();
      args.host_iters = w.direct_iters.as<dvo_hip_iteration_stats>();
    }
  }
  ctx->resident_launches += 1;
  ctx->resident_levels += rp.levels;
  if (rp.group > 1) {
    const size_t bytes = size_t(bp.n) * rp.group * kResidentRing * kResidentSlots * sizeof(unsigned long long) + align_up(size_t(bp.n) * rp.group * sizeof(unsigned), 256);
    const bool grown = bytes > w.exchange.bytes;
    DVO_WS_TRY(w, w.exchange.reserve(bytes));
    const unsigned long long need64 = 2ull * unsigned(rp.levels) * unsigned(cfg->max_iterations_per_level) + 4ull;
    const unsigned need = need64 < 0x40000000ull ? unsigned(need64) : 0x40000000u;
    const long long shape = (long long)bp.n * rp.group;
    if (grown || shape != w.exchange_shape || need64 >= 0x40000000ull || w.resident_sequence > 0xffffffffu - need - 1u) {
      DVO_WS_TRY(w, hipMemsetAsync(w.exchange.p, 0, w.exchange.bytes, s));
      w.resident_sequence = 0;
      w.exchange_shape = shape;
    }
    args.exchange = w.exchange.as<unsigned long long>();
    args.sequence_base = w.resident_sequence;
    w.resident_sequence += need;
  }
  DVO_WS_TRY(w, launch_match_resident(s, args, ctx->opt_resident_cooperative != 0));
  return DVO_HIP_OK;
}

int run_coarse(dvo_hip_context* ctx, Workspace& w, const dvo_hip_config* cfg, const BatchPlan& bp) {
  CoarseArgs args;
  std::memset(&args, 0, sizeof(args));
  for (int l = cfg->last_level; l <= cfg->first_level; ++l) args.geom[l] = bp.geom[l];
  args.pair_ptrs = bp.pair_ptrs;
  args.states = w.states.as<PairState>();
  args.levels = w.lvl_stats.as<dvo_hip_level_stats>();
  args.iters = w.it_stats.as<dvo_hip_iteration_stats>();
  args.T_init = w.t_init.as<double>();
  args.partials = w.partials.as<float>();
  args.scratch = w.scratch.as<float2>();
  args.fallback_count = w.win_fallbacks.as<unsigned long long>();
  args.f16_range_flag = w.f16_range_flag;
  args.prm = bp.prm;
  args.n_pairs = bp.n;
  args.first_level = cfg->first_level;
  args.last_level = cfg->first_level - bp.coarse_levels + 1;
  for (int l = args.last_level; l <= args.first_level; ++l) {
    args.max_tiles = std::max(args.max_tiles, bp.geom[l].tiles_x * bp.geom[l].tiles_y);
    args.max_entries = std::max(args.max_entries, residual_entries(bp.geom[l]));
  }
  args.results = args.last_level == cfg->last_level ? w.results.as<dvo_hip_result>() : nullptr;
  ctx->coarse_launches += 1;
  ctx->coarse_levels += bp.coarse_levels;
  DVO_WS_TRY(w, launch_match_coarse(w.stream, args, ctx->opt_coarse_wgs == 3 ? 3 : 4));
  return DVO_HIP_OK;
}

std::mutex g_rare_path_mutex;

constexpr int kF32GramHoldBatches = 32;

struct BatchRun {
  dvo_hip_context* const ctx;
  Workspace& w;
  const hipStream_t s;
  const dvo_hip_config* const cfg;
  const int n;
  const BatchPolicy policy;
  BatchPlan bp;
  ResidentPlan rp;
  std::vector<double> tinit;
  size_t main_steps = 0, n_steps = 0;
  int level_from = 0;
  PairState* states = nullptr;
  dvo_hip_level_stats* d_levels = nullptr;
  dvo_hip_iteration_stats* d_iters = nullptr;
  float* partials = nullptr;
  float2* scratch = nullptr;
  double* ll_partials = nullptr;
  RefOrderPair* ref_order = nullptr;
  unsigned long long* tallies = nullptr;
  int* arrivals = nullptr;
  int per_level = 0, per_sync = 1;
  int step = kResidentErrorWords;
  BatchRun(dvo_hip_context* c, const dvo_hip_config* config, int n_pairs)
      : ctx(c), w(c->ws[0]), s(c->ws[0].stream), cfg(config), n(n_pairs), policy(c->compute_units) {}
};

struct LevelSchedule {
  bool fused_ll = false, two_waves = false;
  int ll_blocks = 0;
};
LevelSchedule schedule_of(const BatchRun& b, int level) {
  const dvo_hip_context* ctx = b.ctx;
  const LevelGeom& g = b.bp.geom[level];
  LevelSchedule ls;
  const int fuse_opt = ctx->opt_fused_ll_pixels;
  ls.fused_ll = !b.bp.ref_order && g.w * g.h <= (fuse_opt > 0 ? fuse_opt : (b.policy.fused_loglik_on_large_levels(b.n) && !ctx->opt_deterministic ? kFusedLoglikMaxPixelsBatch : kFusedLoglikMaxPixels));
  ls.ll_blocks = ctx->opt_ll_blocks > 0 ? std::min(ctx->opt_ll_blocks, kLlBlocksPerPair)
                 : (!g.compact || ctx->opt_deterministic ? kLlBlocksPerPair : b.policy.loglik_blocks(b.n));
  ls.two_waves = ctx->opt_solver_waves == 2 ||
                 (ctx->opt_solver_waves == 0 && ls.fused_ll && !g.compact && g.tiles_x * g.tiles_y <= 32 && b.policy.solver_two_waves(b.n));
  return ls;
}

#include "capi_lane.inc"

hipEvent_t g_trace_ev[2] = {nullptr, nullptr};
struct PrepTrace {
  const dvo_hip_context* ctx;
  hipStream_t s;
  double limit_ms;
  double ms[5] = {0, 0, 0, 0, 0};
  PrepTrace(const dvo_hip_context* c, hipStream_t stream) : ctx(c), s(stream) {
    static const double trace_slow_ms = std::getenv("DVO_HIP_TRACE_SLOW") ? std::atof(std::getenv("DVO_HIP_TRACE_SLOW")) : 0.0;
    limit_ms = trace_slow_ms;
    mark(0);
    if (limit_ms > 0.0) {
      if (!g_trace_ev[0]) { (void)hipEventCreate(&g_trace_ev[0]); (void)hipEventCreate(&g_trace_ev[1]); }
      (void)hipEventRecord(g_trace_ev[0], s);
    }
  }
  void mark(int k) { if (limit_ms > 0.0) ms[k] = std::chrono::duration<double, std::milli>(std::chrono::steady_clock::now() - ctx->batch_entry).count(); }
  void before_stream_wait() { if (limit_ms > 0.0) (void)hipEventRecord(g_trace_ev[1], s); }
  void after_stream_wait() {
    if (limit_ms <= 0.0) return;
    mark(4);
    float gpu_ms = -1.0f;
    if (ms[4] - ms[3] > limit_ms && hipEventElapsedTime(&gpu_ms, g_trace_ev[0], g_trace_ev[1]) == hipSuccess)
      std::fprintf(stderr, "dvo_hip: the stream wait took %.3f ms on the host; on the device %.3f ms passed between the batch's first and last command so far\n",
                   ms[4] - ms[3], gpu_ms);
  }
  void report(int n) {
    mark(4);
    if (limit_ms > 0.0 && ms[4] > limit_ms)
      std::fprintf(stderr, "dvo_hip: slow preparation of a %d-pair batch: roles %.3f, plan + buffers + tables %.3f, initial guesses + drain %.3f, status words %.3f, "
                   "stream wait + reset %.3f ms\n", n, ms[0], ms[1] - ms[0], ms[2] - ms[1], ms[3] - ms[2], ms[4] - ms[3]);
  }
};

int prepare_batch(BatchRun& b, SlowLane& lane, dvo_hip_frame* const* refs, dvo_hip_frame* const* curs, const dvo_hip_result* results) {
  dvo_hip_context* ctx = b.ctx;
  Workspace& w = b.w;
  const dvo_hip_config* cfg = b.cfg;
  const int n = b.n;
  BatchPlan& bp = b.bp;
  PrepTrace trace(ctx, b.s);
  make_plan(ctx, refs[0]->cam, cfg, n, bp);
  b.rp = plan_paths(ctx, cfg, bp, window_taps_missing(ctx, cfg, n, curs));
  const bool tables_inline = b.rp.direct && n <= kResidentInline;
  int rc = prepare_buffers(w, cfg, refs, curs, bp, !tables_inline);
  if (rc != DVO_HIP_OK) return rc;
  trace.mark(1);

  b.tinit.resize(size_t(n) * 16);
  for (int i = 0; i < n; ++i) std::memcpy(&b.tinit[size_t(i) * 16], results[i].transformation, 16 * sizeof(double));
  if (!tables_inline) DVO_WS_TRY(w, w.tables->upload(b.s, w.t_init.p, b.tinit.data(), b.tinit.size() * sizeof(double)));
  b.main_steps = size_t(bp.cap_iters) + 8 + kResidentErrorWords;
  rc = lane.reserve();
  if (rc != DVO_HIP_OK) return rc;
  b.n_steps = b.main_steps + lane.steps_cap();
  if (ctx->opt_tail_lists) DVO_WS_TRY(w, w.chain_list.reserve(align_up(size_t(n), 64) * sizeof(int)));
  if (w.needs_drain) {
    DVO_WS_TRY(w, w.lane.quiesce());
    DVO_WS_TRY(w, sync_stream(b.s));
    if (w.f16_range_flag) std::memset(w.f16_range_flag, 0, w.f16_range_words * sizeof(int));
  }
  w.needs_drain = true;
  trace.mark(2);
  rc = ensure_host_status(w, b.n_steps);
  if (rc != DVO_HIP_OK) return rc;
  trace.mark(3);
  w.resident_error_word = int(w.resident_launch_counter++ % kResidentErrorWords);
  if (b.rp.direct) {
    w.host_status[w.resident_error_word] = 0;
  } else {
    trace.before_stream_wait();
    if (w.device_may_lag) DVO_WS_TRY(w, sync_stream(b.s));
    w.device_may_lag = false;
    trace.after_stream_wait();
    std::memset(w.host_status, 0, b.n_steps * sizeof(int));
    DVO_WS_TRY(w, hipMemsetAsync(w.counters.p, 0, b.n_steps * sizeof(unsigned long long) + align_up(size_t(n) * sizeof(int), 8), b.s));
  }

  b.states = w.states.as<PairState>();
  b.d_levels = w.lvl_stats.as<dvo_hip_level_stats>();
  b.d_iters = w.it_stats.as<dvo_hip_iteration_stats>();
  b.partials = w.partials.as<float>();
  b.scratch = w.scratch.as<float2>();
  b.ll_partials = w.ll_partials.as<double>();
  b.ref_order = bp.ref_order ? w.ref_pairs.as<RefOrderPair>() : nullptr;
  b.tallies = w.counters.as<unsigned long long>();
  b.arrivals = reinterpret_cast<int*>(b.tallies + b.n_steps);
  b.per_level = cfg->max_iterations_per_level;
  b.per_sync = ctx->opt_iters_per_sync > 0 ? ctx->opt_iters_per_sync : 1;
  trace.report(n);
  return DVO_HIP_OK;
}

int flush_recorded_ingest(BatchRun& b) {
  if (b.ctx->deferred.empty()) return DVO_HIP_OK;
  const int rc_deferred = flush_deferred(b.ctx);
  if (rc_deferred != DVO_HIP_OK) b.w.err = b.ctx->err;
  return rc_deferred;
}

int run_prefixes(BatchRun& b, bool want_stats) {
  const dvo_hip_config* cfg = b.cfg;
  b.level_from = cfg->first_level;
  if (b.rp.levels > 0) {
    Range range("resident");
    int rc = run_resident(b.ctx, b.w, cfg, b.bp, b.rp, b.tinit.data(), want_stats);
    if (rc == DVO_HIP_OK) rc = flush_recorded_ingest(b);
    if (rc != DVO_HIP_OK) return rc;
    b.level_from = cfg->first_level - b.rp.levels;
  }
  if (b.bp.coarse_levels > 0) {
    Range range("coarse");
    int rc = run_coarse(b.ctx, b.w, cfg, b.bp);
    if (rc == DVO_HIP_OK) rc = flush_recorded_ingest(b);
    if (rc != DVO_HIP_OK) return rc;
    b.level_from = cfg->first_level - b.bp.coarse_levels;
  }
  return DVO_HIP_OK;
}

const char* const kRangePrep[kMaxLevels] = {"prep L0", "prep L1", "prep L2", "prep L3", "prep L4", "prep L5", "prep L6", "prep L7"};
const char* const kRangeErr[kMaxLevels] = {"err L0", "err L1", "err L2", "err L3", "err L4", "err L5", "err L6", "err L7"};
const char* const kRangeLinsys[kMaxLevels] = {"linsys L0", "linsys L1", "linsys L2", "linsys L3", "linsys L4", "linsys L5", "linsys L6", "linsys L7"};

struct LevelRun {
  int level = 0;
  LevelGeom g;
  const PairPtrs* pp = nullptr;
  NextLevel next;
  LevelSchedule schedule;
  bool tail = false;
  double* pair_sums = nullptr;
  LevelGeom g_run;
  int n_run = 0;
};

void enqueue_step_in_sweep(BatchRun& b, const LevelRun& L) {
  Workspace& w = b.w;
  Range range(kRangeErr[L.level]);
  const SolverStepArgs a = make_solver_step_args(b.states, b.n, b.bp.prm, b.partials, b.ll_partials, L.schedule.ll_blocks, b.scratch, b.d_levels, b.d_iters, b.tallies + b.step,
                                                 w.host_status + b.step, b.cfg->first_level - L.level, &L.next, b.arrivals, L.pair_sums);
  launch_residual_reduce(b.s, b.ctx->opt_variant, b.bp.rpw[L.level], L.level == 0, L.g, L.pp, b.states, b.n, b.partials, b.scratch, w.win_fallbacks.as<unsigned long long>(),
                         w.f16_range_flag, &a);
  if (L.pair_sums) {
    Range range2(kRangeLinsys[L.level]);
    launch_solver_serial(b.s, b.n, L.g, a);
  }
  b.ctx->tail_steps += 1;
}

void enqueue_step(BatchRun& b, const LevelRun& L) {
  dvo_hip_context* ctx = b.ctx;
  Workspace& w = b.w;
  const bool fused_ll = L.schedule.fused_ll;
  {
    Range range(kRangeErr[L.level]);
    launch_residual_reduce(b.s, ctx->opt_variant, b.bp.rpw[L.level], L.level == 0, L.g_run, L.pp, b.states, L.n_run, b.partials, b.scratch, w.win_fallbacks.as<unsigned long long>(),
                           w.f16_range_flag);
    if (b.ref_order) {
      launch_ref_order(b.s, L.g_run, b.states, L.n_run, b.scratch, w.ref_rows.as<RefOrderSeg>(), b.ref_order);
      ctx->ref_order_passes += 1;
    }
    if (!fused_ll) launch_loglik(b.s, L.g_run, b.states, L.n_run, b.partials, b.scratch, b.ll_partials, L.schedule.ll_blocks, ctx->opt_deterministic != 0, b.ref_order);
  }
  if (L.g_run.pair_list) ctx->listed_steps += 1;
  Range range(kRangeLinsys[L.level]);
  launch_solver_step(b.s, b.states, L.n_run, b.bp.prm, L.g_run, b.partials, b.ll_partials, L.schedule.ll_blocks, fused_ll ? b.scratch : nullptr, b.d_levels, b.d_iters,
                     b.tallies + b.step, w.host_status + b.step, L.schedule.two_waves, b.cfg->first_level - L.level, &L.next, b.ref_order);
}
// ... 294 lines not shown
```

dvo_slam_amd/csrc/device_types.h:

```cpp
#pragma once

#include <stdint.h>

#include "hd_compat.h"
#include "lens.h"
#include "depth_rig.h"
#include "cloud_map.h"
#include "cloud_colour.h"
#include "map_render.h"

#include "../../include/dvo_hip.h"

namespace dvo_hip {

constexpr int kMaxLevels = DVO_HIP_MAX_LEVELS;
constexpr int kBlock = 256;
constexpr int kWavesPerBlock = 4;
constexpr int kTileW = 64;

constexpr int kAccN = 0, kAccS = 1, kAccJ00 = 4, kAccJ11 = 25, kAccJ01 = 46, kAccB00 = 67, kAccB01 = 73, kAccB11 = 79;
constexpr int kNumAcc = 85;
constexpr int kAccStride = 88;

struct LevelGeom {
// ... 230 lines not shown
constexpr int kResidentMaxGroup = 64;
constexpr int kResidentRing = 4;
constexpr int kResidentSlots = 96;
constexpr int kResidentSlotLl = 88;

constexpr int kResidentInline = 4;
constexpr int kResidentFlagNoQuietPoll = 2;
constexpr int kResidentFlagWithhold = 4;

struct ResidentArgs {
  LevelGeom geom[kMaxLevels];
  const PairPtrs* pair_ptrs;
  PairState* states;
  dvo_hip_level_stats* levels;
  dvo_hip_iteration_stats* iters;
  const double* T_init;
  float2* scratch;
  unsigned long long* exchange;
  int* error_word;
  SolverParams prm;
  int n_pairs, group;
  int first_level, last_level;
  unsigned sequence_base;
  dvo_hip_result* results;
  PairPtrs inline_ptrs[kMaxLevels * kResidentInline];
  double inline_T[kResidentInline * 16];
  int use_inline;
  dvo_hip_level_stats* host_levels;
  dvo_hip_iteration_stats* host_iters;
  int* done_word;
  int flags;
};

constexpr int kCoarseRowsPerWave = 2;
struct CoarseArgs {
  LevelGeom geom[kMaxLevels];
  const PairPtrs* pair_ptrs;
  PairState* states;
  dvo_hip_level_stats* levels;
  dvo_hip_iteration_stats* iters;
  const double* T_init;
  float* partials;
  float2* scratch;
  int max_tiles;
  size_t max_entries;
  unsigned long long* fallback_count;
  int* f16_range_flag;
  SolverParams prm;
  int n_pairs;
  int first_level, last_level;
  dvo_hip_result* results;
};

}
```

dvo_slam_amd/csrc/fast_sweep.h:

```cpp
#pragma once
#include <type_traits>

#include "gram_f16.h"


namespace dvo_hip {

constexpr int kFastTileRows = 16;
constexpr int kFastPitch = 96;
constexpr int kFastCols = 84;
constexpr int kFastPairs = kFastCols / 2;
constexpr int kFastRows = 28;
constexpr int kFastRowGroups = 6;
constexpr int kFastLoads = (kFastRows + kFastRowGroups - 1) / kFastRowGroups;
constexpr int kFastCells = kFastPitch * kFastRows;

typedef short __attribute__((ext_vector_type(2))) fast_i16x2;
typedef unsigned __attribute__((ext_vector_type(2))) fast_u32x2;
typedef unsigned __attribute__((__vector_size__(2 * sizeof(unsigned)))) fast_u32v2;
typedef const volatile __attribute__((address_space(3))) f32x2* FastLdsCellPtr;

__device__ __forceinline__ void fast_wave_min2max2_lane63(int& a, int& b, int& c, int& d) {
#define DVO_STAGE(ctrl)                                                                                            \
  asm volatile("s_nop 1\n\t"                                                                                       \
// ... 275 lines not shown
  const f32x2 d1 = fast_lerp2(P[1][2] - P[1][0], P[1][3] - P[1][1], a1);
  const f32x2 d2 = fast_lerp2(P[2][2] - P[2][0], P[2][3] - P[2][1], a1);
  const f32x2 cVx = fast_lerp2(d1, d2, b1);
  const float cI = cV.x, cZ = cV.y, cIx = cVx.x, cZx = cVx.y, cIy = cVy.x, cZy = cVy.y;
  const float r0 = (cI - r.i) * (1.0f / 255.0f);
  const float r1 = cZ - r.qz;
  const float dz = r.z - 0.4f;
  const float thr = fmaf(dz * -0.038f, dz, -0.024f);
  const unsigned long long valid_mask = ok_mask & __builtin_amdgcn_ballot_w64(r1 > thr) & __builtin_amdgcn_ballot_w64(!__builtin_isunordered(cZx, cZy));
  const bool valid = __builtin_amdgcn_inverse_ballot_w64(valid_mask);
  if constexpr (COMPACT) {
    const int below = __builtin_amdgcn_mbcnt_hi(unsigned(valid_mask >> 32), __builtin_amdgcn_mbcnt_lo(unsigned(valid_mask), 0));
    const f32x2 rr2 = {r0, r1};
    __builtin_amdgcn_raw_buffer_store_b64(__builtin_bit_cast(fast_u32v2, rr2), resid, valid ? below * 8 : 0x7ffffff8, off_s + n_valid * 8, AUX);
  } else {
    const f32x2 rr2 = {valid ? r0 : __builtin_nanf(""), r1};
    __builtin_amdgcn_raw_buffer_store_b64(__builtin_bit_cast(fast_u32v2, rr2), resid, off_v, off_s, AUX);
  }
  n_valid += __popcll(valid_mask);
  const float tq = fmaf(wt.P2x, r1, wt.P00 * r0);
  float sw_any;
  if constexpr (COMPAT != 0) {
    const float arg = fmaf(tq, r0, fmaf(wt.P11 * r1, r1, 5.0f));
    sw_any = __builtin_amdgcn_sqrtf(fmaf(wt.wm, fast_rcp_host<COMPAT>(table, arg), wt.wa));
  } else {
    sw_any = wt.wc * fast_rsqrt(fmaf(tq, r0, fmaf(wt.P11 * r1, r1, wt.wk)));
  }
  const float sw = valid ? sw_any : 0.0f;
  const float gix = mul_legacy(sw * g.half_wi_x, cIx + r.gx), giy = mul_legacy(sw * g.half_wi_y, cIy + r.gy);
  const float gzx = mul_legacy(sw * g.half_fx, cZx), gzy = mul_legacy(sw * g.half_fy, cZy);
  const float iz = rcp_for_inline_asm(r.z);
  const float txy = tx * ty, cy = fmaf(ty, ty, 1.0f);
  const float sz = mul_legacy(sw, r.z);
  float c[14];
  c[0] = mul_legacy(gix, iz);
  c[1] = mul_legacy(giy, iz);
  c[2] = fmaf(-ty, c[1], -tx * c[0]);
  c[3] = fmaf(-giy, cy, -gix * txy);
  c[4] = fmaf(gix, cx, giy * txy);
  c[5] = fmaf(giy, tx, -gix * ty);
  c[6] = mul_legacy(gzx, iz);
  c[7] = mul_legacy(gzy, iz);
  c[8] = fmaf(-ty, c[7], fmaf(-tx, c[6], -sw));
  c[9] = fmaf(-ty, fmaf(gzx, tx, sz), -gzy * cy);
  c[10] = fmaf(tx, fmaf(gzy, ty, sz), gzx * cx);
  c[11] = fmaf(gzy, tx, -gzx * ty);
  const float sr = sw * kResidualScale;
  c[12] = mul_legacy(sr, r0);
  c[13] = mul_legacy(sr, r1);
  fast_gram_row<STORE, HI_J>(my, lane, c, acc0, acc1);
}

template <bool WT = false>
__device__ __forceinline__ void fast_epilogue(float (*slab)[kSlabFloatsF16], const int* counts, unsigned gram_entries, float* __restrict__ out_row,
                                              int* __restrict__ f16_range_flag) {
  auto put = [&](int i, float v) {
    if constexpr (WT) __hip_atomic_store(out_row + i, v, __ATOMIC_RELAXED, __HIP_MEMORY_SCOPE_AGENT);
    else out_row[i] = v;
  };
  const int kk = threadIdx.x;
  if (kk < kNumAcc) {
    auto G = [&](int e) {
      const int et = (e & 15) * 16 + (e >> 4);
      float t = 0.0f;
#pragma unroll
      for (int w4 = 0; w4 < 4; ++w4) t += (slab[w4][e] + slab[w4][256 + e]) + slab[w4][256 + et];
      const float s = ((e & 15) >= 12 ? 1.0f / kResidualScale : 1.0f) * ((e >> 4) >= 12 ? 1.0f / kResidualScale : 1.0f);
      return t * s;
    };
    float v;
    if (kk == kAccN) {
      v = float((counts[0] + counts[1]) + (counts[2] + counts[3]));
    } else {
      const int e1 = gram_entries & 0xff, e2 = gram_entries >> 8;
      v = G(e1);
      if (e2 != 0xff) v += G(e2);
      if (f16_range_flag && !(__builtin_fabsf(v) < __builtin_inff())) __hip_atomic_store(f16_range_flag, 1, __ATOMIC_RELAXED, __HIP_MEMORY_SCOPE_SYSTEM);
    }
    put(kk, v);
  } else if (kk < kNumAcc + 2) {
    const int q = (kk - kNumAcc) * 2;
    put(kAccCounts + (kk - kNumAcc), float(counts[q] + 512 * counts[q + 1]));
  }
}

__device__ __forceinline__ void fast_count_fallbacks(unsigned long long* __restrict__ fallback_count, unsigned n_fallback, int lane) {
  const unsigned long long lanes = __ballot(n_fallback != 0);
  if (lanes) {
    unsigned t = n_fallback;
    for (int off = 32; off > 0; off >>= 1) t += __shfl_down(t, off, 64);
    if (lane == 0) atomicAdd(fallback_count, (unsigned long long)t);
  }
}

struct FastLds {
  float (*slab)[kSlabFloatsF16];
  float2* win;
  int (*bbox)[2];
  int* counts;
};

template <int STORE, bool PARTIAL, bool COMPACT, int COMPAT, bool HI_J, bool WT = false>
__device__ __forceinline__ void fast_sweep_tile(const LevelGeom& g, const float* KT, const FastWeights& wt, const PairPtrs& pp, int pair, int tile,
                                                float* __restrict__ partials, float2* __restrict__ scratch, const FastLds& lds,
                                                const FastRcpSource& rcp_table, unsigned long long* __restrict__ fallback_count,
                                                int* __restrict__ f16_range_flag) {
  constexpr int RPW = kFastTileRows / 4;
  const int tiles = g.tiles_x * g.tiles_y;
  const int tile_x = tile % g.tiles_x, tile_y = tile / g.tiles_x;
  const int plane_bytes = g.w * g.h * 8;
  const __amdgpu_buffer_rsrc_t refR = __builtin_amdgcn_make_buffer_rsrc(const_cast<float2*>(pp.refR), 0, plane_bytes, 0x00020000);
  const __amdgpu_buffer_rsrc_t curC = __builtin_amdgcn_make_buffer_rsrc(const_cast<float2*>(pp.curC), 0, plane_bytes, 0x00020000);
  const __amdgpu_buffer_rsrc_t resid = COMPACT ? __builtin_amdgcn_make_buffer_rsrc(scratch + size_t(pair) * tiles * kCompactTileEntries, 0, tiles * kCompactTileEntries * 8, 0x00020000)
                                               : __builtin_amdgcn_make_buffer_rsrc(scratch + size_t(pair) * size_t(g.w) * g.h, 0, plane_bytes, 0x00020000);
  const __amdgpu_buffer_rsrc_t resid_none = __builtin_amdgcn_make_buffer_rsrc(scratch, 0, 0, 0x00020000);
  const int lane = threadIdx.x & 63, wave = __builtin_amdgcn_readfirstlane(threadIdx.x >> 6);
  const unsigned gram_entries = kGramEntryTable.e[min(int(threadIdx.x), kNumAcc - 1)];
  const int u_r = PARTIAL ? min(tile_x * kTileW + lane, g.w - 1) : tile_x * kTileW + lane;
  const unsigned long long col_mask = PARTIAL ? __builtin_amdgcn_ballot_w64(tile_x * kTileW + lane < g.w) : ~0ull;
  const int row_bytes = g.w * 8;
  const float tx_u = g.tx[u_r];
  const float cx_u = fmaf(tx_u, tx_u, 1.0f);

  float (*slab)[kSlabFloatsF16] = lds.slab;
  float2* win = lds.win;
  int (*bbox)[2] = lds.bbox;
  int* counts = lds.counts;
  float* my = slab[wave];
  const int off_px = u_r * 8;
  const int off_store = !PARTIAL || tile_x * kTileW + lane < g.w ? off_px : plane_bytes;
  const int off_edge = (lane == 0 ? max(u_r - 1, 0) : lane == 63 ? min(u_r + 1, g.w - 1) : u_r) * 8 + 4;

  const int row0 = tile_y * kFastTileRows + wave;
  float ty_rows[RPW];
#pragma unroll
  for (int k = 0; k < RPW; ++k) ty_rows[k] = g.ty[min(row0 + k * 4, g.h - 1)];
// ... 92 lines not shown
```

dvo_slam_amd/csrc/launch.h:

```cpp
#pragma once

#include <hip/hip_runtime.h>

#include "device_types.h"

namespace dvo_hip {

struct RefOrderSeg;
struct RefOrderPair;
struct RefOrderPlane;

void launch_pyr_down(hipStream_t s, const FrameBuildPtrs* tbl, int n_frames, int level, int w, int h);
void launch_build_from_raw(hipStream_t s, const FrameBuildPtrs* tbl, int n_frames, float scale, int w0, int h0, int levels, int role, bool strips,
                           float ithr, float dthr, int max_workgroups, int cur_flavor = kCurAB, int c_levels = 0, int colour_channels = 0,
                           bool stream_nt = false, bool depth_f32 = false);
bool derive_strips_supports(int w);
void launch_derive_strips(hipStream_t s, const FrameBuildPtrs* tbl, int n_frames, int level, int w, int h, int role, float ithr, float dthr,
                          int max_workgroups, int cur_flavor, bool stream_nt = false);
bool ingest_strips_supports(int w0, bool wide, bool f32_image = false);
bool f32_strips_aligned(const void* plane, size_t pitch);
bool colour_strips_aligned(const void* colour, size_t pitch, int channels);
void launch_ingest_strips(hipStream_t s, const FrameBuildPtrs* tbl, int n_frames, float scale, int w0, int h0, int levels, int role,
                          float ithr, float dthr, int max_workgroups, int cur_flavor, int c_levels, int colour_channels = 0, bool stream_nt = false,
                          bool depth_f32 = false);
// ... 42 lines not shown
void launch_map_render(hipStream_t s, const MapTable& m, const MapView* views, const RenderPlanes* out, int n_views, long long pixels, const RenderArgs& a,
                       unsigned long long* zbuf, bool colour);
bool map_render_preloads();

struct PgGraph;
struct PgCgState;
void launch_pg_linearise(hipStream_t s, const PgGraph& g, const double* poses, bool with_blocks, double* cost_partials);
void launch_pg_gather(hipStream_t s, const PgGraph& g, double* max_partials);
void launch_pg_cg_init(hipStream_t s, const PgGraph& g, PgCgState* st, double lambda, double* rz_partials);
void launch_pg_multiply(hipStream_t s, const PgGraph& g, PgCgState* st, const double* rz_partials, double* pap_partials, int it, double lambda,
                        double tolerance, bool given);
void launch_pg_cg_update(hipStream_t s, const PgGraph& g, PgCgState* st, const double* pap_partials, double* rz_partials, int it);
void launch_pg_apply(hipStream_t s, const PgGraph& g, double lambda, const double* poses, double* out, double* scale_partials);
void launch_pg_reduce(hipStream_t s, const double* a, int n_a, const double* b, int n_b, double* out);
struct PgResidentJob;
struct PgResidentOut;
struct PgResidentIteration;
void launch_pg_resident(hipStream_t s, const PgResidentJob* jobs, int n_graphs, PgResidentOut* outs, PgResidentIteration* records, int max_records,
                        size_t stage_bytes);

void launch_residual_reduce(hipStream_t s, int variant, int rows_per_wave, bool finest_level, const LevelGeom& g, const PairPtrs* pairs,
                            const PairState* states, int n_pairs, float* partials, float2* scratch, unsigned long long* window_fallbacks = nullptr,
                            int* f16_range_flag = nullptr, const SolverStepArgs* tail = nullptr);
bool sweep_has_tail(int variant, int rows_per_wave, const LevelGeom& g);
bool sweep_fast_has_tail(int variant, const LevelGeom& g);
bool mfma_sweep_has_tail(int variant, int rows_per_wave, const LevelGeom& g);
void launch_residual_reduce_mfma(hipStream_t s, int rows_per_wave, bool finest_level, const LevelGeom& g, const PairPtrs* pairs,
                                 const PairState* states, int n_pairs, float* partials, float2* scratch, int mode = 0,
                                 int* f16_range_flag = nullptr, const SolverStepArgs* tail = nullptr);
bool window_sweep_supports(const LevelGeom& g);
void launch_sweep_window(hipStream_t s, bool f16, const LevelGeom& g, const PairPtrs* pairs, const PairState* states, int n_pairs,
                         float* partials, float2* scratch, unsigned long long* fallback_count, int* f16_range_flag = nullptr);
bool fast_sweep_takes_width(int w);
bool fast_sweep_supports(const LevelGeom& g);
void launch_sweep_fast(hipStream_t s, int variant, const LevelGeom& g, const PairPtrs* pairs, const PairState* states, int n_pairs,
                       float* partials, float2* scratch, unsigned long long* fallback_count, int* f16_range_flag = nullptr,
                       const SolverStepArgs* tail = nullptr);
bool small_sweep_takes(int w, int h);
void launch_sweep_small(hipStream_t s, int rows_per_wave, const LevelGeom& g, const PairPtrs* pairs, const PairState* states, int n_pairs,
                        float* partials, float2* scratch, int* f16_range_flag = nullptr);
void launch_stream_mix(hipStream_t s, const PairPtrs* pairs, int n_pairs, int n_px, float2* scratch, float* sink, bool window_planes = false);
void launch_loglik(hipStream_t s, const LevelGeom& g, const PairState* states, int n_pairs, const float* partials,
                   const float2* scratch, double* ll_partials, int blocks_per_pair, bool one_schedule = false, const RefOrderPair* ref_order = nullptr);

void launch_ref_order(hipStream_t s, const LevelGeom& g, const PairState* states, int n_pairs, const float2* scratch, RefOrderSeg* rows, RefOrderPair* out);
void launch_ref_order_drop_last(hipStream_t s, const RefOrderPlane* planes, int n_planes);
void launch_ref_order_restore(hipStream_t s, const RefOrderPlane* planes, int n_planes);

hipError_t launch_match_resident(hipStream_t s, const ResidentArgs& args, bool cooperative);

bool coarse_kernel_takes(const LevelGeom& g, bool window_level);
hipError_t launch_match_coarse(hipStream_t s, const CoarseArgs& args, int workgroups_per_cu);

extern int g_solver_occupancy;
void launch_init_pairs(hipStream_t s, PairState* states, int n_pairs, SolverParams prm, const double* T_init);
void launch_level_begin(hipStream_t s, PairState* states, int n_pairs, SolverParams prm, LevelGeom g, int level,
                        const PairPtrs* pairs, dvo_hip_level_stats* levels, const double* T_init_or_null = nullptr,
                        const unsigned char* flags = nullptr, int which = 0, int from_level = -1);
void launch_mark_stragglers(hipStream_t s, const PairState* states, int n_pairs, int level, unsigned char* flags, int* list, int cap, bool list_only = false);
void launch_clear_flags(hipStream_t s, unsigned char* flags, int n_pairs);
bool sweep_takes_pair_list(int variant, int rows_per_wave, const LevelGeom& g);
void launch_solver_step(hipStream_t s, PairState* states, int n_pairs, SolverParams prm, LevelGeom g,
                        const float* partials, const double* ll_partials, int ll_blocks_per_pair, const float2* scratch_for_fused_ll,
                        dvo_hip_level_stats* levels, dvo_hip_iteration_stats* iters, unsigned long long* step_tally,
                        int* host_status, bool two_waves = false, int level_slot_hint = -1, const NextLevel* next_or_null = nullptr,
                        const RefOrderPair* ref_order = nullptr);
void launch_solver_serial(hipStream_t s, int n_pairs, LevelGeom g, const SolverStepArgs& a);
void launch_finish(hipStream_t s, const PairState* states, int n_pairs, SolverParams prm,
                   const dvo_hip_level_stats* levels, const dvo_hip_iteration_stats* iters, dvo_hip_result* results);
void launch_force_active(hipStream_t s, PairState* states, int n_pairs);
void launch_set_fixed_state(hipStream_t s, PairState* states, LevelGeom g, const float* T34_dev, const float* Pprev_dev, int first);
void launch_single_shot_out(hipStream_t s, LevelGeom g, const float* partials, const double* ll_partials, int ll_blocks_per_pair,
                            int n_selected, dvo_hip_iteration_out* out_dev, const RefOrderPair* ref_order = nullptr);

}
```

dvo_slam_amd/csrc/mfma_sweep.h:

```cpp
#pragma once
#include "gram_f16.h"

namespace dvo_hip {

struct RefRow {
  float z, i, up, down, left_or_edge, right;
};

template <int MODE>
__host__ __device__ constexpr int mfma_slab_floats() { return MODE >= 1 ? kSlabFloatsF16 : kSlabFloats; }

template <int RPW, bool LINEAR, int MODE, bool WT = false>
__device__ __forceinline__ void mfma_sweep_tile(const LevelGeom& g, const float* KT_src, const float* P_prev_src, bool first, const PairPtrs& pp, int pair,
                                                int tile, float* __restrict__ partials, float2* __restrict__ scratch, float* slab_mem, int* counts,
                                                int* __restrict__ f16_range_flag) {
  constexpr bool F16 = MODE >= 1;
  constexpr bool FAST = MODE == 2;
  const int tiles = g.tiles_x * g.tiles_y;
  float KT[12], Pp[4];
#pragma unroll
  for (int i = 0; i < 12; ++i) KT[i] = KT_src[i];
#pragma unroll
  for (int i = 0; i < 4; ++i) Pp[i] = P_prev_src[i];
  const __amdgpu_buffer_rsrc_t refR = __builtin_amdgcn_make_buffer_rsrc(const_cast<float2*>(pp.refR), 0, g.w * g.h * 8, 0x00020000);
  TapPlanes taps;
  taps.A = __builtin_amdgcn_make_buffer_rsrc(const_cast<float4*>(pp.curA), 0, g.w * g.h * 16, 0x00020000);
  taps.B = __builtin_amdgcn_make_buffer_rsrc(const_cast<float2*>(pp.curB), 0, g.w * g.h * 8, 0x00020000);
  taps.rowA = g.w * 16;
  taps.rowB = g.w * 8;

  const int lane = threadIdx.x & 63, wave = __builtin_amdgcn_readfirstlane(threadIdx.x >> 6);
  const int u_r = LINEAR ? lane : (tile % g.tiles_x) * kTileW + lane;
  const int row0 = (tile / g.tiles_x) * (kWavesPerBlock * RPW) + wave;
  const size_t pix_base = size_t(pair) * size_t(g.w) * g.h;
  const float nanv = __builtin_nanf("");
  const bool col_ok = LINEAR || u_r < g.w;
  const int n_px = g.w * g.h;
  const float inv_w = 1.0f / float(g.w);
  const float tx_u = LINEAR ? 0.0f : g.tx[col_ok ? u_r : 0];
  const float cx_u = fmaf(tx_u, tx_u, 1.0f);
  const float P2x = Pp[1] + Pp[2];

  constexpr int kMySlabFloats = F16 ? kSlabFloatsF16 : kSlabFloats;
  float (*slab)[kMySlabFloats] = reinterpret_cast<float (*)[kMySlabFloats]>(slab_mem);
  float* my = slab[wave];
  f32x4* wr = reinterpret_cast<f32x4*>(my + lane * 4);
  const float* rd = my + ((lane >> 2) & 3) * kQuadStride + (lane >> 4) * 4 + (lane & 3);

  f32x4 acc0 = {0.0f, 0.0f, 0.0f, 0.0f}, acc1 = {0.0f, 0.0f, 0.0f, 0.0f};
  int n_valid = 0;

  const float P00 = Pp[0], P11 = Pp[3];
  const int u_c = LINEAR ? lane : min(u_r, g.w - 1);
  auto load_f = [&](int pixel) { return __builtin_bit_cast(float, __builtin_amdgcn_raw_buffer_load_b32(refR, pixel * 8 + 4, 0, 0)); };
  auto load_ref = [&](int v_r) {
    RefRow r;
    if constexpr (LINEAR) {
      const int idx = min(v_r * kTileW + lane, n_px - 1);
      int row = int(float(idx) * inv_w);
      int col = idx - row * g.w;
      if (col < 0) { col += g.w; row -= 1; }
      if (col >= g.w) { col -= g.w; row += 1; }
      const f32x2 zi = __builtin_bit_cast(f32x2, __builtin_amdgcn_raw_buffer_load_b64(refR, idx * 8, 0, 0));
      r.z = zi.x; r.i = zi.y;
      r.left_or_edge = load_f(idx - (col > 0 ? 1 : 0));
      r.right = load_f(idx + (col < g.w - 1 ? 1 : 0));
      r.up = load_f(idx - (row > 0 ? g.w : 0));
      r.down = load_f(idx + (row < g.h - 1 ? g.w : 0));
    } else {
      const int v = min(v_r, g.h - 1);
      const int idx = v * g.w + u_c;
      const f32x2 zi = __builtin_bit_cast(f32x2, __builtin_amdgcn_raw_buffer_load_b64(refR, idx * 8, 0, 0));
      r.z = zi.x; r.i = zi.y;
      r.up = load_f(idx - (v > 0 ? g.w : 0));
      r.down = load_f(idx + (v < g.h - 1 ? g.w : 0));
      r.left_or_edge = 0.0f;
      r.right = 0.0f;
      if (lane == 0) r.left_or_edge = load_f(idx - (u_c > 0 ? 1 : 0));
      if (lane == 63) r.left_or_edge = load_f(idx + (u_c < g.w - 1 ? 1 : 0));
    }
    return r;
  };
// ... 65 lines not shown
      const f32x2 cZg = blend(f32x2{t.B00.x, t.B00.y}, f32x2{t.B10.x, t.B10.y}, f32x2{t.B01.x, t.B01.y}, f32x2{t.B11.x, t.B11.y});
      o.r0 = (cIZ.x - ref.y) * (1.0f / 255.0f);
      o.r1 = cIZ.y - p.qz;
      const float dz = p.Z - 0.4f;
      o.gix = g.wi_x * (cIg.x + ref.z);
      o.giy = g.wi_y * (cIg.y + ref.w);
      o.gzx = g.fx * cZg.x;
      o.gzy = g.fy * cZg.y;
      o.X = p.X; o.Y = p.Y; o.Z = p.Z;
      valid = p.ok && o.r1 > fmaf(dz * -0.038f, dz, -0.024f) && !__builtin_isunordered(cZg.x, cZg.y);
    } else {
      valid = pixel_finish_flat(g, ref, p, t, o) && p.ok;
    }
    n_valid += __popcll(__ballot(valid));
    if (in_image) {
      const float2 rr = valid ? make_float2(o.r0, o.r1) : make_float2(nanv, nanv);
      if constexpr (WT) __hip_atomic_store(reinterpret_cast<unsigned long long*>(scratch + pix_base + pix), __builtin_bit_cast(unsigned long long, rr), __ATOMIC_RELAXED, __HIP_MEMORY_SCOPE_AGENT);
      else scratch[pix_base + pix] = rr;
    }
    if constexpr (F16) {
      const float sw_any = first ? 1.0f : g.rcp_table ? tdist_weight_sqrt_compat(g.rcp_table, g.rcp_shift, o.r0, o.r1, Pp)
                                                      : tdist_weight_sqrt_fast(o.r0, o.r1, P00, P2x, P11);
      gram_f16_row(my, lane, o, valid ? sw_any : 0.0f, tx_p, ty_p, cx, acc0, acc1);
      return;
    }
    if (valid) {
      const float sw = first ? 1.0f : g.rcp_table ? tdist_weight_sqrt_compat(g.rcp_table, g.rcp_shift, o.r0, o.r1, Pp)
                                                  : tdist_weight_sqrt_fast(o.r0, o.r1, P00, P2x, P11);
      float J0[6], J1[6];
      jacobian_rows_fast(o, sw, tx_p, ty_p, cx, fmaf(ty_p, ty_p, 1.0f), J0, J1);
      wr[0] = f32x4{J0[0], J0[1], J0[2], J0[3]};
      wr[kQuadStride / 4] = f32x4{J0[4], J0[5], J1[0], J1[1]};
      wr[2 * (kQuadStride / 4)] = f32x4{J1[2], J1[3], J1[4], J1[5]};
      wr[3 * (kQuadStride / 4)] = f32x4{sw * o.r0, sw * o.r1, 0.0f, 0.0f};
    } else {
      const f32x4 zero = {0.0f, 0.0f, 0.0f, 0.0f};
      wr[0] = zero;
      wr[kQuadStride / 4] = zero;
      wr[2 * (kQuadStride / 4)] = zero;
      wr[3 * (kQuadStride / 4)] = zero;
    }
    __builtin_amdgcn_fence(__ATOMIC_RELEASE, "wavefront");
    __builtin_amdgcn_wave_barrier();
    __builtin_amdgcn_fence(__ATOMIC_ACQUIRE, "wavefront");
#pragma unroll
    for (int grp = 0; grp < 16; grp += 2) {
      const float a0 = rd[grp * 16], a1 = rd[grp * 16 + 16];
      acc0 = __builtin_amdgcn_mfma_f32_16x16x4f32(a0, a0, acc0, 0, 0, 0);
      acc1 = __builtin_amdgcn_mfma_f32_16x16x4f32(a1, a1, acc1, 0, 0, 0);
    }
    __builtin_amdgcn_fence(__ATOMIC_RELEASE, "wavefront");
    __builtin_amdgcn_wave_barrier();
  };
  RefRow ref_a = load_ref(row0), ref_b = ref_a;
#pragma unroll 1
  for (int k = 0; k < RPW; k += 2) {
    const int v_r = row0 + k * kWavesPerBlock;
    if (k + 1 < RPW) ref_b = load_ref(v_r + kWavesPerBlock);
    sweep_row(v_r, ref_a);
    if (k + 1 < RPW) {
      if (k + 2 < RPW) ref_a = load_ref(v_r + 2 * kWavesPerBlock);
      sweep_row(v_r + kWavesPerBlock, ref_b);
    }
  }

#pragma unroll
  for (int i = 0; i < 4; ++i)
    if (!F16) my[((lane >> 4) * 4 + i) * 16 + (lane & 15)] = acc0[i] + acc1[i];
  if constexpr (F16) gram_f16_finish(my, lane, acc0, acc1, f16_range_flag ? f16_range_flag + pair : nullptr);
  if (lane == 0) counts[wave] = n_valid;
  __syncthreads();
  const int k = threadIdx.x;
  if (k < kNumAcc) {
    auto G = [&](int e) { return (slab[0][e] + slab[1][e]) + (slab[2][e] + slab[3][e]); };
    float v;
    if (k == kAccN) {
      v = float((counts[0] + counts[1]) + (counts[2] + counts[3]));
    } else {
      int e1, e2;
      gram_entries_of_accumulator(k, e1, e2);
      v = G(e1);
      if (e2 >= 0) v += G(e2);
    }
    if constexpr (WT) __hip_atomic_store(partials + (size_t(pair) * tiles + tile) * kAccStride + k, v, __ATOMIC_RELAXED, __HIP_MEMORY_SCOPE_AGENT);
    else partials[(size_t(pair) * tiles + tile) * kAccStride + k] = v;
  }
}

}
```

dvo_slam_amd/csrc/reduce_scale.h:

```cpp
#pragma once

#include "pixel_math.h"

namespace dvo_hip {

constexpr int kReduceInFlight = 32;

template <int WAVES = kWavesPerBlock, int IN_FLIGHT = kReduceInFlight>
__device__ inline void reduce_partials(const float* __restrict__ partials, int pair, int tiles, double* sh, double* sums) {
  static_assert(WAVES == 2 || WAVES == 4, "two or four wavefronts");
  constexpr int kPlayed = kWavesPerBlock / WAVES;
  constexpr int kInFlight = IN_FLIGHT / kPlayed;
  const int lane = threadIdx.x & 63, wave = threadIdx.x >> 6;
  const float* base = partials + size_t(pair) * tiles * kAccStride;
  const bool hi = lane < kAccStride - 64;
  double a0[kPlayed], a1[kPlayed];
#pragma unroll
  for (int r = 0; r < kPlayed; ++r) a0[r] = a1[r] = 0.0;
  for (int t0 = wave; t0 < tiles; t0 += kInFlight * kWavesPerBlock) {
    float v0[kPlayed][kInFlight], v1[kPlayed][kInFlight];
#pragma unroll
    for (int r = 0; r < kPlayed; ++r)
#pragma unroll
      for (int j = 0; j < kInFlight; ++j) {
        const int t = t0 + r * WAVES + j * kWavesPerBlock;
        const float* row = base + size_t(t < tiles ? t : tiles - 1) * kAccStride;
        v0[r][j] = row[lane];
        v1[r][j] = row[hi ? 64 + lane : 64];
      }
#pragma unroll
    for (int r = 0; r < kPlayed; ++r)
#pragma unroll
      for (int j = 0; j < kInFlight; ++j) {
        const bool in = t0 + r * WAVES + j * kWavesPerBlock < tiles;
        a0[r] += in ? double(v0[r][j]) : 0.0;
        a1[r] += in ? double(v1[r][j]) : 0.0;
      }
  }
#pragma unroll
  for (int r = 0; r < kPlayed; ++r) {
    sh[(wave + r * WAVES) * kAccStride + lane] = a0[r];
    if (hi) sh[(wave + r * WAVES) * kAccStride + 64 + lane] = a1[r];
  }
  __syncthreads();
  if (threadIdx.x < kAccStride) {
    const int k = threadIdx.x;
    sums[k] = (sh[k] + sh[kAccStride + k]) + (sh[2 * kAccStride + k] + sh[3 * kAccStride + k]);
  }
  __syncthreads();
}

constexpr int kScaleLoadsInFlight = 16;
constexpr int kScaleRowsPerRound = 16 * kScaleLoadsInFlight;
constexpr int kScaleStageFloats = kWavesPerBlock * kScaleRowsPerRound * 4;

__device__ inline void reduce_partials_scale(const float* __restrict__ partials, int pair, int tiles, float* stage, double* sh, double* sums) {
  const int lane = threadIdx.x & 63, wave = threadIdx.x >> 6;
  const float* base = partials + size_t(pair) * tiles * kAccStride;
  const int my_rows = tiles > wave ? (tiles - wave + kWavesPerBlock - 1) / kWavesPerBlock : 0;
  float* mine = stage + wave * kScaleRowsPerRound * 4;
  double a0 = 0.0;
  for (int r0 = 0; r0 < my_rows; r0 += kScaleRowsPerRound) {
    float v[kScaleLoadsInFlight];
#pragma unroll
    for (int j = 0; j < kScaleLoadsInFlight; ++j) {
      const int r = r0 + j * 16 + (lane >> 2);
      const int t = wave + (r < my_rows ? r : my_rows - 1) * kWavesPerBlock;
      v[j] = base[size_t(t) * kAccStride + (lane & 3)];
    }
#pragma unroll
    for (int j = 0; j < kScaleLoadsInFlight; ++j) mine[(j * 16 + (lane >> 2)) * 4 + (lane & 3)] = v[j];
    __builtin_amdgcn_fence(__ATOMIC_RELEASE, "wavefront");
    __builtin_amdgcn_wave_barrier();
    __builtin_amdgcn_fence(__ATOMIC_ACQUIRE, "wavefront");
    if (lane < 4) {
      const int count = min(kScaleRowsPerRound, my_rows - r0);
      for (int r = 0; r < count; ++r) a0 += double(mine[r * 4 + lane]);
    }
    __builtin_amdgcn_fence(__ATOMIC_RELEASE, "wavefront");
    __builtin_amdgcn_wave_barrier();
  }
  if (lane < 4) sh[wave * 4 + lane] = a0;
  __syncthreads();
  if (threadIdx.x < 4) {
    const int k = threadIdx.x;
    sums[k] = (sh[k] + sh[4 + k]) + (sh[8 + k] + sh[12 + k]);
  }
  __syncthreads();
}

__device__ inline int scale_from_sums(const double* sums, float* C, float* P) {
  const double d = sums[kAccN] - 3.0;
  scale_to_precision(sums[kAccS] / d, sums[kAccS + 1] / d, sums[kAccS + 2] / d, C, P);
  return int(sums[kAccN] + 0.5);
}

}
```

dvo_slam_amd/csrc/sweep_parts.h:

```cpp
#pragma once

#include "align_common.h"

namespace dvo_hip {

typedef float __attribute__((ext_vector_type(4))) f32x4;
typedef float __attribute__((ext_vector_type(2))) f32x2;

constexpr int kQuadStride = 264;
constexpr int kSlabFloats = 4 * kQuadStride;

struct TapPlanes {
  __amdgpu_buffer_rsrc_t A, B;
  int rowA, rowB;
  __device__ __forceinline__ void fetch(int base, PixelTaps& t) const {
    const int oa = base * 16, ob = base * 8;
    const f32x4 a00 = __builtin_bit_cast(f32x4, __builtin_amdgcn_raw_buffer_load_b128(A, oa, 0, 0));
    const f32x4 a10 = __builtin_bit_cast(f32x4, __builtin_amdgcn_raw_buffer_load_b128(A, oa + 16, 0, 0));
    const f32x4 a01 = __builtin_bit_cast(f32x4, __builtin_amdgcn_raw_buffer_load_b128(A, oa, rowA, 0));
    const f32x4 a11 = __builtin_bit_cast(f32x4, __builtin_amdgcn_raw_buffer_load_b128(A, oa + 16, rowA, 0));
    const f32x2 b00 = __builtin_bit_cast(f32x2, __builtin_amdgcn_raw_buffer_load_b64(B, ob, 0, 0));
    const f32x2 b10 = __builtin_bit_cast(f32x2, __builtin_amdgcn_raw_buffer_load_b64(B, ob + 8, 0, 0));
    const f32x2 b01 = __builtin_bit_cast(f32x2, __builtin_amdgcn_raw_buffer_load_b64(B, ob, rowB, 0));
    const f32x2 b11 = __builtin_bit_cast(f32x2, __builtin_amdgcn_raw_buffer_load_b64(B, ob + 8, rowB, 0));
    t.A00 = make_float4(a00.x, a00.y, a00.z, a00.w); t.A10 = make_float4(a10.x, a10.y, a10.z, a10.w);
    t.A01 = make_float4(a01.x, a01.y, a01.z, a01.w); t.A11 = make_float4(a11.x, a11.y, a11.z, a11.w);
    t.B00 = make_float2(b00.x, b00.y); t.B10 = make_float2(b10.x, b10.y);
    t.B01 = make_float2(b01.x, b01.y); t.B11 = make_float2(b11.x, b11.y);
  }
};

__device__ __forceinline__ void gram_entries_of_accumulator(int k, int& e1, int& e2) {
  auto E = [](int r, int c) { return r * 16 + c; };
  e2 = -1;
  if (k == kAccS) e1 = E(12, 12);
  else if (k == kAccS + 1) e1 = E(12, 13);
  else if (k == kAccS + 2) e1 = E(13, 13);
  else if (k < kAccB00) {
    const int blockId = (k - kAccJ00) / 21;
    int o = (k - kAccJ00) % 21, i = 0;
    while (o >= 6 - i) { o -= 6 - i; ++i; }
    const int j = i + o;
    if (blockId == 0) e1 = E(i, j);
    else if (blockId == 1) e1 = E(6 + i, 6 + j);
    else { e1 = E(i, 6 + j); e2 = E(j, 6 + i); }
  } else if (k < kAccB01) e1 = E(k - kAccB00, 12);
  else if (k < kAccB11) { e1 = E(k - kAccB01, 13); e2 = E(6 + (k - kAccB01), 12); }
  else e1 = E(6 + (k - kAccB11), 13);
}

struct GramEntryTable {
  unsigned short e[kNumAcc];
};
constexpr GramEntryTable make_gram_entry_table() {
  GramEntryTable t{};
  auto E = [](int r, int c) { return r * 16 + c; };
  for (int k = 0; k < kNumAcc; ++k) {
    int e1 = 0, e2 = 0xff;
    if (k == kAccN) e1 = 0;
    else if (k == kAccS) e1 = E(12, 12);
    else if (k == kAccS + 1) e1 = E(12, 13);
    else if (k == kAccS + 2) e1 = E(13, 13);
    else if (k < kAccB00) {
      const int blockId = (k - kAccJ00) / 21;
      int o = (k - kAccJ00) % 21, i = 0;
      while (o >= 6 - i) { o -= 6 - i; ++i; }
      const int j = i + o;
      if (blockId == 0) e1 = E(i, j);
      else if (blockId == 1) e1 = E(6 + i, 6 + j);
      else { e1 = E(i, 6 + j); e2 = E(j, 6 + i); }
    } else if (k < kAccB01) e1 = E(k - kAccB00, 12);
    else if (k < kAccB11) { e1 = E(k - kAccB01, 13); e2 = E(6 + (k - kAccB01), 12); }
    else e1 = E(6 + (k - kAccB11), 13);
    t.e[k] = (unsigned short)(e1 | e2 << 8);
  }
  return t;
}
__device__ __constant__ const GramEntryTable kGramEntryTable = make_gram_entry_table();

}
```

Before: 95170 alignments/s.

## Add persistent per-pair LDS level kernel fusing sweep, reduction and GN step

Result: slower. 93770 alignments/s (-1.5%).

```diff
diff --git a/dvo_slam_amd/csrc/align_level_lds.hip b/dvo_slam_amd/csrc/align_level_lds.hip
--- /dev/null
+++ b/dvo_slam_amd/csrc/align_level_lds.hip
@@ -0,0 +1,200 @@
+#include "small_sweep.h"
+#include "mfma_sweep.h"
+#include "solver_step.h"
+#include "launch.h"
+
+namespace dvo_hip {
+
+namespace {
+
+__device__ __forceinline__ int lds_uniform(int v) { return __builtin_amdgcn_readfirstlane(v); }
+__device__ __forceinline__ float lds_uniform(float v) { return __builtin_bit_cast(float, __builtin_amdgcn_readfirstlane(__builtin_bit_cast(int, v))); }
+
+constexpr int kLdsReduceInFlight = 8;
+constexpr int kLdsLlLoads = 4;
+
+struct alignas(16) LevelLdsState {
+  PairState st;
+  dvo_hip_level_stats lvl;
+  dvo_hip_iteration_stats rec;
+  double sums[kAccStride];
+  double ll_waves[kWavesPerBlock];
+  double Amat[36], bvec[6];
+  int counts[16];
+  int information_ready, rec_index;
+};
+
+constexpr size_t lds_align16(size_t b) { return (b + 15) & ~size_t(15); }
+__host__ __device__ constexpr size_t level_lds_img_bytes(int w, int h) { return lds_align16(size_t(w + 2) * size_t(h + 2) * sizeof(float2)); }
+constexpr size_t level_lds_bytes(int teams, int w, int h) {
+  return level_lds_img_bytes(w, h) + size_t(teams) * kWavesPerBlock * kSlabFloatsF16 * sizeof(float) + lds_align16(sizeof(LevelLdsState));
+}
+static_assert((kSlabFloatsF16 * sizeof(float)) % 16 == 0, "carved at multiples of 16 bytes");
+static_assert(size_t(kWavesPerBlock) * kSlabFloatsF16 * sizeof(float) >= sizeof(dvo_hip_result), "the result is composed in the idle slabs");
+static_assert(level_lds_bytes(1, 80, 60) <= 42 * 1280, "three 256-thread workgroups per compute unit at 80 x 60");
+static_assert(size_t(2) * kSlabFloatsF16 * sizeof(float) >= sizeof(double) * kWavesPerBlock * kAccStride, "the reduction's staging area borrows two slabs");
+
+}
+
+template <int G, int WAVES_PER_SIMD, bool GATHER>
+__global__ __launch_bounds__(G * kBlock, WAVES_PER_SIMD) void k_level_lds(const LevelLdsArgs a) {
+  static_assert(!GATHER || G == 1, "the gathering tile function is written for four wavefronts");
+  constexpr int kThreads = G * kBlock;
+  extern __shared__ __attribute__((aligned(16))) char lds_raw[];
+  float2* img = reinterpret_cast<float2*>(lds_raw);
+  const size_t img_bytes = level_lds_img_bytes(a.g.w, a.g.h);
+  float (*slab)[kSlabFloatsF16] = reinterpret_cast<float (*)[kSlabFloatsF16]>(lds_raw + img_bytes);
+  LevelLdsState& L = *reinterpret_cast<LevelLdsState*>(lds_raw + img_bytes + size_t(G) * kWavesPerBlock * kSlabFloatsF16 * sizeof(float));
+  PairState& st = L.st;
+  double* sh = reinterpret_cast<double*>(&slab[0][0]);
+
+  const int pair = blockIdx.x;
+  const int tid = threadIdx.x, lane = tid & 63;
+  const int wave = lds_uniform(tid >> 6), team = wave >> 2, wave4 = wave & 3, tid4 = tid & (kBlock - 1);
+  const LevelGeom& g = a.g;
+  const PairPtrs pp = a.pair_ptrs[pair];
+  const int n_px = g.w * g.h, plane_bytes = n_px * 8;
+  const __amdgpu_buffer_rsrc_t refR = __builtin_amdgcn_make_buffer_rsrc(const_cast<float2*>(pp.refR), 0, plane_bytes, 0x00020000);
+  const __amdgpu_buffer_rsrc_t curC = __builtin_amdgcn_make_buffer_rsrc(const_cast<float2*>(pp.curC), 0, plane_bytes, 0x00020000);
+  const __amdgpu_buffer_rsrc_t resid = __builtin_amdgcn_make_buffer_rsrc(a.scratch + size_t(pair) * size_t(n_px), 0, plane_bytes, 0x00020000);
+  const int tiles = g.tiles_x * g.tiles_y;
+  float* my_partials = a.partials + size_t(pair) * tiles * kAccStride;
+  const float2* my_residuals = a.scratch + size_t(pair) * size_t(n_px);
+  int* my_flag = a.f16_range_flag ? a.f16_range_flag + pair : nullptr;
+
+  small_stage_level<kThreads>(g, curC, img);
+  if (tid == 0) gn_init_pair(st, a.prm, a.T_init + size_t(pair) * 16);
+  __syncthreads();
+  const int level_slot = lds_uniform(st.n_levels);
+  const bool have_level = level_slot < a.prm.cap_levels;
+  SolverParams local = a.prm;
+  local.cap_levels = have_level ? level_slot + 1 : 0;
+  local.record_prefilled = 1;
+  if (tid == 0) gn_level_begin(st, local, g, g.level, *pp.n_selected, &L.lvl - level_slot);
+  __syncthreads();
+
+  const SmallSweepSetup su(g);
+  const unsigned gram_entries = kGramEntryTable.e[min(tid4, kNumAcc - 1)];
+  RefRow ref_carry = {};
+  const int max_passes = a.prm.max_iterations + 1;
+#pragma unroll 1
+  for (int pass = 0; pass < max_passes; ++pass) {
+    float KT[12], Pp[4];
+#pragma unroll
+    for (int i = 0; i < 12; ++i) KT[i] = lds_uniform(st.KT[i]);
+#pragma unroll
+    for (int i = 0; i < 4; ++i) Pp[i] = lds_uniform(st.P_prev[i]);
+    const FastWeights wt(Pp, lds_uniform(st.first) != 0);
+    if constexpr (GATHER) {
+      const LdsTaps taps = {img, g.w, g.w + 2, 1.0f / float(g.w)};
+      const bool first = lds_uniform(st.first) != 0;
+#pragma unroll 1
+      for (int tile = 0; tile < tiles; ++tile) {
+        mfma_sweep_tile<kCoarseRowsPerWave, true, 2, false, LdsTaps, true>(g, KT, Pp, first, pp, 0, tile, my_partials, a.scratch + size_t(pair) * size_t(n_px),
+                                                                           &slab[0][0], L.counts, my_flag, &taps, &ref_carry, pass > 0 || tile > 0,
+                                                                           tile + 1 < tiles ? tile + 1 : 0);
+        __syncthreads();
+      }
+    } else {
+#pragma unroll 1
+      for (int t0 = 0; t0 < tiles; t0 += G) {
+        const int tile = t0 + team;
+        if (tile < tiles) small_sweep_tile(g, su, KT, wt, refR, resid, img, tile, wave4, lane, a.rows_per_wave, slab[wave], &L.counts[wave]);
+        __syncthreads();
+        if (tile < tiles) fast_epilogue_at(tid4, slab + team * kWavesPerBlock, L.counts + team * kWavesPerBlock, gram_entries, my_partials + size_t(tile) * kAccStride, my_flag);
+        __syncthreads();
+      }
+    }
+
+    if (wave < kWavesPerBlock) reduce_partials_rows<kWavesPerBlock, kLdsReduceInFlight>(my_partials, 0, tiles, sh);
+    for (int i = tid; i < int(sizeof(dvo_hip_iteration_stats) / 8); i += kThreads) reinterpret_cast<double*>(&L.rec)[i] = dvo_nan();
+    __syncthreads();
+    if (tid < kAccStride) reduce_partials_combine(sh, L.sums);
+    __syncthreads();
+    if (tid < 42) {
+      const double d = L.sums[kAccN] - 3.0;
+      float Cc[3], Pc[4];
+      scale_to_precision(L.sums[kAccS] / d, L.sums[kAccS + 1] / d, L.sums[kAccS + 2] / d, Cc, Pc);
+      const double p00 = double(Pc[0]), p01 = double(Pc[1]), p11 = double(Pc[3]);
+      const int k = tid;
+      if (k < 36) {
+        const int i = k / 6, j = k - i * 6, lo = i < j ? i : j, hi = i < j ? j : i;
+        const int o = lo * 6 - lo * (lo - 1) / 2 + (hi - lo);
+        L.Amat[k] = gn_contract(p00, p01, p11, L.sums[kAccJ00 + o], L.sums[kAccJ01 + o], L.sums[kAccJ11 + o]);
+      } else {
+        L.bvec[k - 36] = gn_contract(p00, p01, p11, L.sums[kAccB00 + k - 36], L.sums[kAccB01 + k - 36], L.sums[kAccB11 + k - 36]);
+      }
+    }
+    if (wave < kWavesPerBlock) {
+      float C[3], P[4];
+      const int n = scale_from_sums(L.sums, C, P);
+      double t = 0.0;
+      if (n >= 6) t = loglik_partial<kLdsLlLoads>(my_residuals, n_px, P, 0, 1);
+      const double total = wave_sum_double(t);
+      if (lane == 0) L.ll_waves[wave] = total;
+    }
+    __syncthreads();
+    if (tid == 0) {
+      const double ll_sum = (L.ll_waves[0] + L.ll_waves[1]) + (L.ll_waves[2] + L.ll_waves[3]);
+      L.rec_index = st.n_iters_total;
+      SolverParams step = local;
+      step.cap_iters = L.rec_index + 1;
+      GnAssist assist = {L.Amat, L.bvec, 1, 0};
+      gn_step(st, step, g, L.sums, ll_sum, &L.lvl - level_slot, &L.rec - L.rec_index, nullptr, &assist);
+      L.information_ready = assist.information_ready;
+    }
+    __syncthreads();
+    if (L.information_ready && tid < 36) L.rec.information[tid] = L.Amat[tid];
+    __syncthreads();
+    if (L.rec_index < a.prm.cap_iters) coop_copy<kThreads>(a.iters + size_t(pair) * a.prm.cap_iters + L.rec_index, &L.rec);
+    if (!lds_uniform(st.active)) break;
+    __syncthreads();
+  }
+  __syncthreads();
+  if (have_level) coop_copy<kThreads>(a.levels + size_t(pair) * a.prm.cap_levels + level_slot, &L.lvl);
+  coop_copy<kThreads>(&a.states[pair], &st);
+  if (a.results) {
+    __threadfence();
+    __syncthreads();
+    dvo_hip_result* result = reinterpret_cast<dvo_hip_result*>(&slab[0][0]);
+    if (tid == 0) gn_finish(st, a.prm, a.levels + size_t(pair) * a.prm.cap_levels, a.iters + size_t(pair) * a.prm.cap_iters, result);
+    __syncthreads();
+    coop_copy<kThreads>(a.results + pair, result);
+    if (tid == 0) a.states[pair].finished = 1;
+  }
+}
+
+namespace {
+
+template <int G, int WAVES_PER_SIMD, bool GATHER>
+hipError_t launch_level_lds_as(hipStream_t s, const LevelLdsArgs& args) {
+  static thread_local int raised_on = -1;
+  int device = 0;
+  hipError_t e = hipGetDevice(&device);
+  if (e != hipSuccess) return e;
+  const size_t largest = size_t(kSmallCells) * sizeof(float2) + level_lds_bytes(G, 0, 0);
+  if (raised_on != device) {
+    e = hipFuncSetAttribute(reinterpret_cast<const void*>(&k_level_lds<G, WAVES_PER_SIMD, GATHER>), hipFuncAttributeMaxDynamicSharedMemorySize, int(largest));
+    if (e != hipSuccess) return e;
+    raised_on = device;
+  }
+  const size_t bytes = level_lds_bytes(G, args.g.w, args.g.h);
+  if (bytes > largest) return hipErrorInvalidValue;
+  k_level_lds<G, WAVES_PER_SIMD, GATHER><<<dim3(args.n_pairs), dim3(G * kBlock), bytes, s>>>(args);
+  return hipGetLastError();
+}
+
+}
+
+hipError_t launch_level_lds(hipStream_t s, const LevelLdsArgs& args, int threads) {
+  if (!args.g.small) {
+    if (args.rows_per_wave != kCoarseRowsPerWave) return hipErrorInvalidValue;
+    return launch_level_lds_as<1, 3, true>(s, args);
+  }
+  if (threads == 256) return launch_level_lds_as<1, 3, false>(s, args);
+  if (threads == 512) return launch_level_lds_as<2, 4, false>(s, args);
+  if (threads == 1024) return launch_level_lds_as<4, 4, false>(s, args);
+  return hipErrorInvalidValue;
+}
+
+}
diff --git a/dvo_slam_amd/csrc/align_small.hip b/dvo_slam_amd/csrc/align_small.hip
--- a/dvo_slam_amd/csrc/align_small.hip
+++ b/dvo_slam_amd/csrc/align_small.hip
@@ -1,10 +1,7 @@
-#include "fast_sweep.h"
+#include "small_sweep.h"
 #include "launch.h"
 
 namespace dvo_hip {
-
-constexpr int kSmallCells = 5376;
-constexpr int kSmallLoads = kSmallCells / kBlock;
 
 __global__ __launch_bounds__(kBlock, 3) void k_sweep_small(
     const LevelGeom g, const PairPtrs* __restrict__ pairs, const PairState* __restrict__ states, int n_pairs,
@@ -27,106 +24,16 @@
   const __amdgpu_buffer_rsrc_t curC = __builtin_amdgcn_make_buffer_rsrc(const_cast<float2*>(pp.curC), 0, plane_bytes, 0x00020000);
   const __amdgpu_buffer_rsrc_t resid = __builtin_amdgcn_make_buffer_rsrc(scratch + size_t(pair) * size_t(n_px), 0, plane_bytes, 0x00020000);
 
-  const int pitch = g.w + 2, cells = pitch * (g.h + 2);
-  {
-    const float inv_pitch = 1.0f / float(pitch);
-    f32x2 v[kSmallLoads];
-#pragma unroll
-    for (int j = 0; j < kSmallLoads; ++j) {
-      const int c = min(int(threadIdx.x) + j * kBlock, cells - 1);
-      int cy = int(float(c) * inv_pitch);
-      int cx = c - cy * pitch;
-      if (cx < 0) { cx += pitch; cy -= 1; }
-      if (cx >= pitch) { cx -= pitch; cy += 1; }
-      const int x = min(max(cx - 1, 0), g.w - 1), y = min(max(cy - 1, 0), g.h - 1);
-      v[j] = __builtin_bit_cast(f32x2, __builtin_amdgcn_raw_buffer_load_b64(curC, (y * g.w + x) * 8, 0, 0));
-    }
-#pragma unroll
-    for (int j = 0; j < kSmallLoads; ++j) {
-      const int c = int(threadIdx.x) + j * kBlock;
-      if (c < cells) img[c] = make_float2(v[j].x, v[j].y);
-    }
-  }
+  small_stage_level<kBlock>(g, curC, img);
 
   float KT[12];
 #pragma unroll
   for (int i = 0; i < 12; ++i) KT[i] = st.KT[i];
   const FastWeights wt(st);
-  const FastRcpSource no_table = {__builtin_amdgcn_make_buffer_rsrc(static_cast<float*>(nullptr), 0, 0, 0x00020000), nullptr, 0};
+  const SmallSweepSetup su(g);
   const unsigned gram_entries = kGramEntryTable.e[min(int(threadIdx.x), kNumAcc - 1)];
-  const unsigned w2_bits = __builtin_bit_cast(unsigned, float(g.w - 2)), h2_bits = __builtin_bit_cast(unsigned, float(g.h - 2));
-  const float inv_w = 1.0f / float(g.w);
-  const float nanv = __builtin_nanf("");
-  const int segments = (n_px + kTileW - 1) / kTileW;
-  const int seg0 = tile * (kWavesPerBlock * rows_per_wave) + wave;
-  float* my = slab[wave];
-  f32x4 acc0 = {0.0f, 0.0f, 0.0f, 0.0f}, acc1 = {0.0f, 0.0f, 0.0f, 0.0f};
-  int n_valid = 0;
-  auto load_f = [&](int pixel) { return __builtin_bit_cast(float, __builtin_amdgcn_raw_buffer_load_b32(refR, pixel * 8 + 4, 0, 0)); };
-  struct Ref {
-    float z, i, left, right, up, down, tx, ty;
-  };
-  auto load_ref = [&](int seg) {
-    const int pc = min(seg * kTileW + lane, n_px - 1);
-    int row = int(float(pc) * inv_w);
-    int col = pc - row * g.w;
-    if (col < 0) { col += g.w; row -= 1; }
-    if (col >= g.w) { col -= g.w; row += 1; }
-    Ref r;
-    const f32x2 zi = __builtin_bit_cast(f32x2, __builtin_amdgcn_raw_buffer_load_b64(refR, pc * 8, 0, 0));
-    r.z = zi.x; r.i = zi.y;
-    r.left = load_f(pc - (col > 0 ? 1 : 0));
-    r.right = load_f(pc + (col < g.w - 1 ? 1 : 0));
-    r.up = load_f(pc - (row > 0 ? g.w : 0));
-    r.down = load_f(pc + (row < g.h - 1 ? g.w : 0));
-    r.tx = g.tx[col];
-    r.ty = g.ty[row];
-    return r;
-  };
   __syncthreads();
-  Ref next = load_ref(min(seg0, segments - 1));
-#pragma unroll 1
-  for (int k = 0; k < rows_per_wave; ++k) {
-    const int seg = seg0 + k * kWavesPerBlock;
-    if (seg >= segments) break;
-    const Ref ref = next;
-    if (k + 1 < rows_per_wave) next = load_ref(min(seg + kWavesPerBlock, segments - 1));
-    const int idx = seg * kTileW + lane;
-    const bool in_image = idx < n_px;
-    const float z = in_image ? ref.z : nanv;
-    const float tx = ref.tx, ty = ref.ty;
-    float u, v, qz;
-    fast_project<0>(g, no_table, KT, fmaf(KT[0], tx, KT[2]), fmaf(KT[4], tx, KT[6]), fmaf(KT[8], tx, KT[10]), z, tx, ty, u, v, qz);
-    const unsigned long long ok_mask = __builtin_amdgcn_ballot_w64(__builtin_bit_cast(unsigned, u) <= w2_bits) &
-                                       __builtin_amdgcn_ballot_w64(__builtin_bit_cast(unsigned, v) <= h2_bits);
-    const bool ok = __builtin_amdgcn_inverse_ballot_w64(ok_mask);
-    const int u0 = int(u), v0 = int(v);
-    FastRow r;
-    r.z = z; r.i = ref.i;
-    r.gx = ref.right - ref.left;
-    r.gy = ref.down - ref.up;
-    r.qz = qz;
-    r.a1 = __builtin_amdgcn_fractf(u);
-    r.b1 = __builtin_amdgcn_fractf(v);
-    r.idx = v0 * pitch + u0;
-    f32x2 P[4][4];
-    {
-      FastLdsCellPtr q = (FastLdsCellPtr)(img + (ok ? r.idx : 0));
-#pragma unroll
-      for (int rr = 0; rr < 4; ++rr)
-#pragma unroll
-        for (int cc = 0; cc < 4; ++cc)
-          if ((rr == 1 || rr == 2) || (cc == 1 || cc == 2)) P[rr][cc] = q[rr * pitch + cc];
-    }
-    fast_row_tail<2, false, 0, false>(g, no_table, P, r, ok_mask, tx, ty, fmaf(tx, tx, 1.0f), wt, resid, in_image ? idx * 8 : 0x7ffffff8, 0, my, lane, acc0, acc1, n_valid);
-  }
-
-#pragma unroll
-  for (int i = 0; i < 4; ++i) {
-    my[((lane >> 4) * 4 + i) * 16 + (lane & 15)] = acc0[i];
-    my[256 + ((lane >> 4) * 4 + i) * 16 + (lane & 15)] = acc1[i];
-  }
-  if (lane == 0) counts[wave] = n_valid;
+  small_sweep_tile(g, su, KT, wt, refR, resid, img, tile, wave, lane, rows_per_wave, slab[wave], &counts[wave]);
   __syncthreads();
   fast_epilogue(slab, counts, gram_entries, partials + (size_t(pair) * tiles + tile) * kAccStride, f16_range_flag ? f16_range_flag + pair : nullptr);
 }
diff --git a/dvo_slam_amd/csrc/batch_policy.h b/dvo_slam_amd/csrc/batch_policy.h
--- a/dvo_slam_amd/csrc/batch_policy.h
+++ b/dvo_slam_amd/csrc/batch_policy.h
@@ -26,6 +26,8 @@
     return t < 3 ? 3 : t > 8 ? 8 : t;
   }
 
+  int level_lds_min_pairs() const { return 2 * cus; }
+
   int defer_ingest_max_pairs() const { return cus; }
   int background_build_workgroups() const { return cus; }
 };
diff --git a/dvo_slam_amd/csrc/capi.hip b/dvo_slam_amd/csrc/capi.hip
--- a/dvo_slam_amd/csrc/capi.hip
+++ b/dvo_slam_amd/csrc/capi.hip
@@ -420,6 +420,12 @@
   int opt_coarse_pixels = 0;
   int opt_coarse_wgs = 0;
   long long coarse_launches = 0, coarse_levels = 0;
+  int opt_level_lds = -1;
+  int opt_level_lds_threads = 0;
+  long long level_lds_launches = 0, level_lds_pairs = 0;
+  long long current_planes_derived = 0;
+  bool batch_wants_level_lds = false;
+  bool stats_fit = true;
   int opt_deterministic = 0;
   int opt_ref_compat = 0;
   int opt_ref_order = 0;
@@ -803,7 +809,7 @@
 int prepare_roles(dvo_hip_context* ctx, int n_frames, dvo_hip_frame* const* frames, int role, const dvo_hip_config* cfg) {
   const bool ref = role == DVO_HIP_ROLE_REFERENCE;
   int want[kMaxLevels];
-  for (int l = 0; l < kMaxLevels; ++l) want[l] = l < frames[0]->cam->levels ? eager_current_flavor(ctx, frames[0]->cam, l, n_frames) : kCurAB;
+  for (int l = 0; l < kMaxLevels; ++l) want[l] = l < frames[0]->cam->levels ? eager_current_flavor(ctx, frames[0]->cam, l, n_frames, cfg->first_level) : kCurAB;
   float ithr = ref ? cfg->intensity_derivative_threshold : 0.0f, dthr = ref ? cfg->depth_derivative_threshold : 0.0f;
   std::vector<dvo_hip_frame*> speculative;
   if (ref && (ithr < 0.0f || dthr < 0.0f)) {
@@ -1122,6 +1128,11 @@
     if (mine) DVO_FLUSH_DEFERRED(ctx);
   }
   EffectiveVariantScope effective_variant_scope(ctx);
+  {
+    const int n_levels = cfg->first_level - cfg->last_level + 1;
+    ctx->stats_fit = !(levels && cap_levels > 0 && cap_levels < n_levels) && !(iters && cap_iters > 0 && cap_iters < n_levels * cfg->max_iterations_per_level);
+    ctx->batch_wants_level_lds = level_lds_wanted(ctx, n_pairs);
+  }
   rc = ensure_batch_roles(ctx, n_pairs, references, currents, cfg);
   if (rc != DVO_HIP_OK) return rc;
 
diff --git a/dvo_slam_amd/csrc/capi_frames.inc b/dvo_slam_amd/csrc/capi_frames.inc
--- a/dvo_slam_amd/csrc/capi_frames.inc
+++ b/dvo_slam_amd/csrc/capi_frames.inc
@@ -159,6 +159,23 @@
 
 bool level_uses_small(const dvo_hip_context* ctx, int w, int h) {
   return ctx->opt_small_sweep && ctx->opt_variant >= 8 && !ctx->opt_ref_compat && !ctx->opt_ref_order && !level_uses_window(ctx, w, h) && level_is_linear(ctx, w) && small_sweep_takes(w, h);
+}
+
+bool level_lds_admits(const dvo_hip_context* ctx, int w, int h) {
+  return ctx->opt_level_lds != 0 && ctx->opt_variant == 8 && !ctx->opt_deterministic && !ctx->opt_ref_compat && !ctx->opt_ref_order &&
+         (ctx->opt_rows_per_wave == 0 || (ctx->opt_rows_per_wave == kCoarseRowsPerWave && !ctx->opt_small_sweep)) && !level_uses_window(ctx, w, h) &&
+         level_is_linear(ctx, w) && small_sweep_takes(w, h) && size_t(w) * h < (size_t(1) << 24);
+}
+bool level_lds_wanted(const dvo_hip_context* ctx, int n_pairs) {
+  return ctx->opt_level_lds == 1 ||
+         (ctx->opt_level_lds < 0 && ctx->opt_small_sweep != 0 && n_pairs >= BatchPolicy(ctx->compute_units).level_lds_min_pairs());
+}
+int level_lds_threads(const dvo_hip_context* ctx) { return ctx->opt_level_lds_threads > 0 ? ctx->opt_level_lds_threads : kLevelLdsThreadsDefault; }
+int level_lds_rows_per_wave(const dvo_hip_context* ctx, const CameraGeom* cam, int level) {
+  const int tiles = ctx->opt_small_tiles > 0 ? ctx->opt_small_tiles : level_lds_threads(ctx) / kBlock;
+  const int segments = (cam->w[level] * cam->h[level] + kTileW - 1) / kTileW;
+  const int rows = (segments + kWavesPerBlock * tiles - 1) / (kWavesPerBlock * tiles);
+  return rows < 1 ? 1 : rows;
 }
 
 LevelGeom make_geom(const dvo_hip_context* ctx, const CameraGeom* cam, int level, int rows_per_wave) {
@@ -284,9 +301,12 @@
 
 bool aligned_to(const void* p, size_t a) { return reinterpret_cast<uintptr_t>(p) % a == 0; }
 
-int eager_current_flavor(const dvo_hip_context* ctx, const CameraGeom* cam, int level, int n_frames) {
+int eager_current_flavor(const dvo_hip_context* ctx, const CameraGeom* cam, int level, int n_frames, int first_level) {
   if (level_uses_small(ctx, cam->w[level], cam->h[level]))
     return BatchPolicy(ctx->compute_units).resident_first_level_fits(n_frames) ? (kCurAB | kCurC) : kCurC;
+  if (level == first_level && level_lds_admits(ctx, cam->w[level], cam->h[level]) && level_lds_wanted(ctx, n_frames) &&
+      !BatchPolicy(ctx->compute_units).resident_first_level_fits(n_frames))
+    return kCurC;
   if (!level_uses_window(ctx, cam->w[level], cam->h[level])) return kCurAB;
   return BatchPolicy(ctx->compute_units).ingest_skips_taps(n_frames) ? kCurC : (kCurAB | kCurC);
 }
@@ -374,7 +394,7 @@
   const int channels = image_f32 ? kChF32 : colour ? pixel_channels(src->format) : 0;
   if (image_f32) wide = cam->w[0] % 2 == 0;
   const float depth_scale = from_raw ? src->depth_scale : 0.0f;
-  const int flavor0 = eager_current_flavor(ctx, cam, 0, n);
+  const int flavor0 = eager_current_flavor(ctx, cam, 0, n, levels - 1);
   for (int i = 0; i < n; ++i) {
     dvo_hip_frame* f = frames[i];
     fill_build_ptrs(f, host[i]);
@@ -438,7 +458,7 @@
     const bool strips = ingest_strips_supports(cam->w[0], wide, image_f32);
     if (role == 0 && strips) {
       for (int l = 1; l < built; ++l)
-        if (eager_current_flavor(ctx, cam, l, n) & kCurC) c_levels |= 1 << l;
+        if (eager_current_flavor(ctx, cam, l, n, levels - 1) & kCurC) c_levels |= 1 << l;
       for (int i = 0; i < n; ++i)
         for (int l = 1; l < built; ++l)
           if ((c_levels >> l & 1) && frames[i]->lv[l].C) frames[i]->lv[l].cur_have |= kCurC;
@@ -527,6 +547,7 @@
           FrameLevel& L = frames[i]->lv[l];
           if (role == 0) L.cur_have |= span.flavor[l];
           else mark_selected(L, ithr, dthr);
+          if (role == 0 && !eager) ctx->current_planes_derived += 1;
         }
       if (role == 1) {
         const int rc = apply_selection(ctx, stream, n, frames, l0, l1, cap);
@@ -578,6 +599,7 @@
       }
       if (role == 0) {
         L.cur_have |= miss;
+        if (!eager) ctx->current_planes_derived += 1;
       } else {
         mark_selected(L, ithr, dthr);
         selected.push_back(f);
diff --git a/dvo_slam_amd/csrc/capi_groups.inc b/dvo_slam_amd/csrc/capi_groups.inc
--- a/dvo_slam_amd/csrc/capi_groups.inc
+++ b/dvo_slam_amd/csrc/capi_groups.inc
@@ -7,6 +7,7 @@
   DVO_MIRROR(opt_sweep_tail); DVO_MIRROR(opt_coarse); DVO_MIRROR(opt_coarse_pixels); DVO_MIRROR(opt_coarse_wgs);
   DVO_MIRROR(opt_deterministic); DVO_MIRROR(opt_ref_order); DVO_MIRROR(opt_small_sweep); DVO_MIRROR(opt_small_tiles); DVO_MIRROR(compute_units);
   DVO_MIRROR(opt_overlap_tails); DVO_MIRROR(opt_overlap_fraction); DVO_MIRROR(opt_tail_lists); DVO_MIRROR(opt_defer_ingest_pixels);
+  DVO_MIRROR(opt_level_lds); DVO_MIRROR(opt_level_lds_threads); DVO_MIRROR(batch_wants_level_lds); DVO_MIRROR(stats_fit);
 #undef DVO_MIRROR
 }
 
diff --git a/dvo_slam_amd/csrc/capi_options.inc b/dvo_slam_amd/csrc/capi_options.inc
--- a/dvo_slam_amd/csrc/capi_options.inc
+++ b/dvo_slam_amd/csrc/capi_options.inc
@@ -20,6 +20,9 @@
   else if (std::strcmp(key, "ref_order_passes") == 0) *value = ctx->ref_order_passes;
   else if (std::strcmp(key, "coarse_launches") == 0) *value = ctx->coarse_launches;
   else if (std::strcmp(key, "coarse_levels") == 0) *value = ctx->coarse_levels;
+  else if (std::strcmp(key, "level_lds_launches") == 0) *value = ctx->level_lds_launches;
+  else if (std::strcmp(key, "level_lds_pairs") == 0) *value = ctx->level_lds_pairs;
+  else if (std::strcmp(key, "current_planes_derived") == 0) *value = ctx->current_planes_derived;
   else if (std::strcmp(key, "window_fallbacks") == 0) {
     unsigned long long v = 0;
     if (ctx->ws[0].win_fallbacks.p) {
@@ -160,6 +163,16 @@
     ctx->opt_coarse = value;
     return DVO_HIP_OK;
   }
+  if (std::strcmp(key, "level_lds") == 0) {
+    if (value < -1 || value > 1) return fail(ctx, DVO_HIP_ERR_INVALID, "level_lds must be -1 (by batch size), 0 (off) or 1 (whenever the first level admits it)");
+    ctx->opt_level_lds = value;
+    return DVO_HIP_OK;
+  }
+  if (std::strcmp(key, "level_lds_threads") == 0) {
+    if (value != 0 && value != 256 && value != 512 && value != 1024) return fail(ctx, DVO_HIP_ERR_INVALID, "level_lds_threads must be 0 (default), 256, 512 or 1024");
+    ctx->opt_level_lds_threads = value;
+    return DVO_HIP_OK;
+  }
   if (std::strcmp(key, "coarse_pixels") == 0) {
     if (value < 0) return fail(ctx, DVO_HIP_ERR_INVALID, "coarse_pixels must be >= 0");
     ctx->opt_coarse_pixels = value;
diff --git a/dvo_slam_amd/csrc/capi_schedule.inc b/dvo_slam_amd/csrc/capi_schedule.inc
--- a/dvo_slam_amd/csrc/capi_schedule.inc
+++ b/dvo_slam_amd/csrc/capi_schedule.inc
@@ -7,6 +7,7 @@
   PairPtrs* pair_ptrs = nullptr;
   std::vector<PairPtrs> host_ptrs;
   int coarse_levels = 0;
+  int lds_level = -1;
   bool ref_order = false;
 };
 
@@ -54,7 +55,7 @@
   }
 }
 
-int resident_levels_of(const dvo_hip_context* ctx, const dvo_hip_config* cfg, const CameraGeom* cam, int n, bool taps_missing);
+int resident_levels_of(const dvo_hip_context* ctx, const dvo_hip_config* cfg, const CameraGeom* cam, int n, bool taps_missing, int* lds_level = nullptr);
 bool window_taps_missing(const dvo_hip_context* ctx, const dvo_hip_config* cfg, int n, dvo_hip_frame* const* curs);
 
 int ref_order_planes(dvo_hip_context* ctx, int n, dvo_hip_frame* const* refs, const dvo_hip_config* cfg) {
@@ -91,10 +92,11 @@
   if (rc == DVO_HIP_OK) rc = wait_for_build(ctx, n, curs);
   if (rc != DVO_HIP_OK) return rc;
   const CameraGeom* cam = curs[0]->cam;
-  const int resident = launch_path_only ? 0 : resident_levels_of(ctx, cfg, cam, n, window_taps_missing(ctx, cfg, n, curs));
+  int lds_level = -1;
+  const int resident = launch_path_only ? 0 : resident_levels_of(ctx, cfg, cam, n, window_taps_missing(ctx, cfg, n, curs), &lds_level);
   int want[kMaxLevels];
   for (int l = 0; l < kMaxLevels; ++l)
-    want[l] = l > cfg->first_level - resident || l >= cam->levels || !(level_uses_window(ctx, cam->w[l], cam->h[l]) || level_uses_small(ctx, cam->w[l], cam->h[l])) ? kCurAB : kCurC;
+    want[l] = l == lds_level ? kCurC : l > cfg->first_level - resident || l >= cam->levels || !(level_uses_window(ctx, cam->w[l], cam->h[l]) || level_uses_small(ctx, cam->w[l], cam->h[l])) ? kCurAB : kCurC;
   rc = ensure_roles(ctx, n, curs, 0, cfg->last_level, cfg->first_level, 0.0f, 0.0f, false, want);
   if (rc == DVO_HIP_OK)
     rc = ensure_roles(ctx, n, refs, 1, cfg->last_level, cfg->first_level, cfg->intensity_derivative_threshold, cfg->depth_derivative_threshold);
@@ -341,6 +343,18 @@
   }
 }
 
+void plan_level_lds(const dvo_hip_context* ctx, const dvo_hip_config* cfg, BatchPlan& bp, const ResidentPlan& rp) {
+  bp.lds_level = -1;
+  const int level = cfg->first_level;
+  if (rp.levels > 0 || bp.coarse_levels > 0 || !ctx->stats_fit) return;
+  if (!level_lds_admits(ctx, bp.cam->w[level], bp.cam->h[level]) || !ctx->batch_wants_level_lds) return;
+  const bool small = level_uses_small(ctx, bp.cam->w[level], bp.cam->h[level]);
+  bp.rpw[level] = small ? level_lds_rows_per_wave(ctx, bp.cam, level) : kCoarseRowsPerWave;
+  bp.geom[level] = make_geom(ctx, bp.cam, level, bp.rpw[level]);
+  if (bp.geom[level].compact || bp.geom[level].rcp_table || bp.geom[level].gram_hi_j) return;
+  bp.lds_level = level;
+}
+
 ResidentPlan plan_paths(const dvo_hip_context* ctx, const dvo_hip_config* cfg, BatchPlan& bp, bool taps_missing) {
   ResidentPlan rp = plan_resident(ctx, cfg, bp, taps_missing);
   if (ctx->opt_coarse == 1) {
@@ -350,13 +364,16 @@
   } else {
     plan_coarse(ctx, cfg, bp, rp);
   }
+  plan_level_lds(ctx, cfg, bp, rp);
   return rp;
 }
 
-int resident_levels_of(const dvo_hip_context* ctx, const dvo_hip_config* cfg, const CameraGeom* cam, int n, bool taps_missing) {
+int resident_levels_of(const dvo_hip_context* ctx, const dvo_hip_config* cfg, const CameraGeom* cam, int n, bool taps_missing, int* lds_level) {
   BatchPlan bp;
   make_plan(ctx, cam, cfg, n, bp);
-  return plan_paths(ctx, cfg, bp, taps_missing).levels;
+  const int levels = plan_paths(ctx, cfg, bp, taps_missing).levels;
+  if (lds_level) *lds_level = bp.lds_level;
+  return levels;
 }
 
 int run_resident(dvo_hip_context* ctx, Workspace& w, const dvo_hip_config* cfg, const BatchPlan& bp, const ResidentPlan& rp,
@@ -445,6 +462,29 @@
   ctx->coarse_launches += 1;
   ctx->coarse_levels += bp.coarse_levels;
   DVO_WS_TRY(w, launch_match_coarse(w.stream, args, ctx->opt_coarse_wgs == 3 ? 3 : 4));
+  return DVO_HIP_OK;
+}
+
+int run_level_lds(dvo_hip_context* ctx, Workspace& w, const dvo_hip_config* cfg, const BatchPlan& bp) {
+  LevelLdsArgs args;
+  std::memset(&args, 0, sizeof(args));
+  const int level = bp.lds_level;
+  args.g = bp.geom[level];
+  args.pair_ptrs = bp.pair_ptrs + size_t(level) * bp.n;
+  args.states = w.states.as<PairState>();
+  args.levels = w.lvl_stats.as<dvo_hip_level_stats>();
+  args.iters = w.it_stats.as<dvo_hip_iteration_stats>();
+  args.T_init = w.t_init.as<double>();
+  args.partials = w.partials.as<float>();
+  args.scratch = w.scratch.as<float2>();
+  args.f16_range_flag = w.f16_range_flag;
+  args.prm = bp.prm;
+  args.n_pairs = bp.n;
+  args.rows_per_wave = bp.rpw[level];
+  args.results = level == cfg->last_level ? w.results.as<dvo_hip_result>() : nullptr;
+  ctx->level_lds_launches += 1;
+  ctx->level_lds_pairs += bp.n;
+  DVO_WS_TRY(w, launch_level_lds(w.stream, args, level_lds_threads(ctx)));
   return DVO_HIP_OK;
 }
 
@@ -540,6 +580,14 @@
   PrepTrace trace(ctx, b.s);
   make_plan(ctx, refs[0]->cam, cfg, n, bp);
   b.rp = plan_paths(ctx, cfg, bp, window_taps_missing(ctx, cfg, n, curs));
+  if (bp.lds_level >= 0) {
+    bool planes = true;
+    for (int i = 0; i < n && planes; ++i) planes = (curs[i]->lv[bp.lds_level].cur_have & kCurC) != 0;
+    if (!planes) {
+      w.err = "match: the current frames lack plane C of the level the LDS level kernel was planned for";
+      return DVO_HIP_ERR_INVALID;
+    }
+  }
   const bool tables_inline = b.rp.direct && n <= kResidentInline;
   int rc = prepare_buffers(w, cfg, refs, curs, bp, !tables_inline);
   if (rc != DVO_HIP_OK) return rc;
@@ -613,6 +661,13 @@
     if (rc == DVO_HIP_OK) rc = flush_recorded_ingest(b);
     if (rc != DVO_HIP_OK) return rc;
     b.level_from = cfg->first_level - b.bp.coarse_levels;
+  }
+  if (b.bp.lds_level >= 0) {
+    Range range("level lds");
+    int rc = run_level_lds(b.ctx, b.w, cfg, b.bp);
+    if (rc == DVO_HIP_OK) rc = flush_recorded_ingest(b);
+    if (rc != DVO_HIP_OK) return rc;
+    b.level_from = cfg->first_level - 1;
   }
   return DVO_HIP_OK;
 }
diff --git a/dvo_slam_amd/csrc/device_types.h b/dvo_slam_amd/csrc/device_types.h
--- a/dvo_slam_amd/csrc/device_types.h
+++ b/dvo_slam_amd/csrc/device_types.h
@@ -306,4 +306,20 @@
   dvo_hip_result* results;
 };
 
+struct LevelLdsArgs {
+  LevelGeom g;
+  const PairPtrs* pair_ptrs;
+  PairState* states;
+  dvo_hip_level_stats* levels;
+  dvo_hip_iteration_stats* iters;
+  const double* T_init;
+  float* partials;
+  float2* scratch;
+  int* f16_range_flag;
+  SolverParams prm;
+  int n_pairs;
+  int rows_per_wave;
+  dvo_hip_result* results;
+};
+
 }
diff --git a/dvo_slam_amd/csrc/fast_sweep.h b/dvo_slam_amd/csrc/fast_sweep.h
--- a/dvo_slam_amd/csrc/fast_sweep.h
+++ b/dvo_slam_amd/csrc/fast_sweep.h
@@ -351,13 +351,12 @@
 }
 
 template <bool WT = false>
-__device__ __forceinline__ void fast_epilogue(float (*slab)[kSlabFloatsF16], const int* counts, unsigned gram_entries, float* __restrict__ out_row,
-                                              int* __restrict__ f16_range_flag) {
+__device__ __forceinline__ void fast_epilogue_at(int kk, float (*slab)[kSlabFloatsF16], const int* counts, unsigned gram_entries, float* __restrict__ out_row,
+                                                 int* __restrict__ f16_range_flag) {
   auto put = [&](int i, float v) {
     if constexpr (WT) __hip_atomic_store(out_row + i, v, __ATOMIC_RELAXED, __HIP_MEMORY_SCOPE_AGENT);
     else out_row[i] = v;
   };
-  const int kk = threadIdx.x;
   if (kk < kNumAcc) {
     auto G = [&](int e) {
       const int et = (e & 15) * 16 + (e >> 4);
@@ -381,6 +380,12 @@
     const int q = (kk - kNumAcc) * 2;
     put(kAccCounts + (kk - kNumAcc), float(counts[q] + 512 * counts[q + 1]));
   }
+}
+
+template <bool WT = false>
+__device__ __forceinline__ void fast_epilogue(float (*slab)[kSlabFloatsF16], const int* counts, unsigned gram_entries, float* __restrict__ out_row,
+                                              int* __restrict__ f16_range_flag) {
+  fast_epilogue_at<WT>(threadIdx.x, slab, counts, gram_entries, out_row, f16_range_flag);
 }
 
 __device__ __forceinline__ void fast_count_fallbacks(unsigned long long* __restrict__ fallback_count, unsigned n_fallback, int lane) {
diff --git a/dvo_slam_amd/csrc/launch.h b/dvo_slam_amd/csrc/launch.h
--- a/dvo_slam_amd/csrc/launch.h
+++ b/dvo_slam_amd/csrc/launch.h
@@ -118,6 +118,9 @@
 bool coarse_kernel_takes(const LevelGeom& g, bool window_level);
 hipError_t launch_match_coarse(hipStream_t s, const CoarseArgs& args, int workgroups_per_cu);
 
+constexpr int kLevelLdsThreadsDefault = 256;
+hipError_t launch_level_lds(hipStream_t s, const LevelLdsArgs& args, int threads);
+
 extern int g_solver_occupancy;
 void launch_init_pairs(hipStream_t s, PairState* states, int n_pairs, SolverParams prm, const double* T_init);
 void launch_level_begin(hipStream_t s, PairState* states, int n_pairs, SolverParams prm, LevelGeom g, int level,
diff --git a/dvo_slam_amd/csrc/mfma_sweep.h b/dvo_slam_amd/csrc/mfma_sweep.h
--- a/dvo_slam_amd/csrc/mfma_sweep.h
+++ b/dvo_slam_amd/csrc/mfma_sweep.h
@@ -10,10 +10,12 @@
 template <int MODE>
 __host__ __device__ constexpr int mfma_slab_floats() { return MODE >= 1 ? kSlabFloatsF16 : kSlabFloats; }
 
-template <int RPW, bool LINEAR, int MODE, bool WT = false>
+template <int RPW, bool LINEAR, int MODE, bool WT = false, typename TAPS = TapPlanes, bool CARRY = false>
 __device__ __forceinline__ void mfma_sweep_tile(const LevelGeom& g, const float* KT_src, const float* P_prev_src, bool first, const PairPtrs& pp, int pair,
                                                 int tile, float* __restrict__ partials, float2* __restrict__ scratch, float* slab_mem, int* counts,
-                                                int* __restrict__ f16_range_flag) {
+                                                int* __restrict__ f16_range_flag, const TAPS* lds_taps = nullptr, RefRow* carry = nullptr,
+                                                bool have_carry = false, int next_tile = 0) {
+  static_assert(!CARRY || LINEAR, "the carried row is a linear level's");
   constexpr bool F16 = MODE >= 1;
   constexpr bool FAST = MODE == 2;
   const int tiles = g.tiles_x * g.tiles_y;
@@ -23,11 +25,15 @@
 #pragma unroll
   for (int i = 0; i < 4; ++i) Pp[i] = P_prev_src[i];
   const __amdgpu_buffer_rsrc_t refR = __builtin_amdgcn_make_buffer_rsrc(const_cast<float2*>(pp.refR), 0, g.w * g.h * 8, 0x00020000);
-  TapPlanes taps;
-  taps.A = __builtin_amdgcn_make_buffer_rsrc(const_cast<float4*>(pp.curA), 0, g.w * g.h * 16, 0x00020000);
-  taps.B = __builtin_amdgcn_make_buffer_rsrc(const_cast<float2*>(pp.curB), 0, g.w * g.h * 8, 0x00020000);
-  taps.rowA = g.w * 16;
-  taps.rowB = g.w * 8;
+  TAPS taps;
+  if constexpr (__is_same(TAPS, TapPlanes)) {
+    taps.A = __builtin_amdgcn_make_buffer_rsrc(const_cast<float4*>(pp.curA), 0, g.w * g.h * 16, 0x00020000);
+    taps.B = __builtin_amdgcn_make_buffer_rsrc(const_cast<float2*>(pp.curB), 0, g.w * g.h * 8, 0x00020000);
+    taps.rowA = g.w * 16;
+    taps.rowB = g.w * 8;
+  } else {
+    taps = *lds_taps;
+  }
 
   const int lane = threadIdx.x & 63, wave = __builtin_amdgcn_readfirstlane(threadIdx.x >> 6);
   const int u_r = LINEAR ? lane : (tile % g.tiles_x) * kTileW + lane;
@@ -199,7 +205,14 @@
     __builtin_amdgcn_fence(__ATOMIC_RELEASE, "wavefront");
     __builtin_amdgcn_wave_barrier();
   };
-  RefRow ref_a = load_ref(row0), ref_b = ref_a;
+  RefRow ref_a;
+  if constexpr (CARRY) {
+    if (have_carry) ref_a = *carry;
+    else ref_a = load_ref(row0);
+  } else {
+    ref_a = load_ref(row0);
+  }
+  RefRow ref_b = ref_a;
 #pragma unroll 1
   for (int k = 0; k < RPW; k += 2) {
     const int v_r = row0 + k * kWavesPerBlock;
@@ -211,6 +224,7 @@
     }
   }
 
+  if constexpr (CARRY) *carry = load_ref(next_tile * (kWavesPerBlock * RPW) + wave);
 #pragma unroll
   for (int i = 0; i < 4; ++i)
     if (!F16) my[((lane >> 4) * 4 + i) * 16 + (lane & 15)] = acc0[i] + acc1[i];
diff --git a/dvo_slam_amd/csrc/reduce_scale.h b/dvo_slam_amd/csrc/reduce_scale.h
--- a/dvo_slam_amd/csrc/reduce_scale.h
+++ b/dvo_slam_amd/csrc/reduce_scale.h
@@ -7,7 +7,7 @@
 constexpr int kReduceInFlight = 32;
 
 template <int WAVES = kWavesPerBlock, int IN_FLIGHT = kReduceInFlight>
-__device__ inline void reduce_partials(const float* __restrict__ partials, int pair, int tiles, double* sh, double* sums) {
+__device__ __forceinline__ void reduce_partials_rows(const float* __restrict__ partials, int pair, int tiles, double* sh) {
   static_assert(WAVES == 2 || WAVES == 4, "two or four wavefronts");
   constexpr int kPlayed = kWavesPerBlock / WAVES;
   constexpr int kInFlight = IN_FLIGHT / kPlayed;
@@ -42,11 +42,18 @@
     sh[(wave + r * WAVES) * kAccStride + lane] = a0[r];
     if (hi) sh[(wave + r * WAVES) * kAccStride + 64 + lane] = a1[r];
   }
+}
+
+__device__ __forceinline__ void reduce_partials_combine(const double* sh, double* sums) {
+  const int k = threadIdx.x;
+  sums[k] = (sh[k] + sh[kAccStride + k]) + (sh[2 * kAccStride + k] + sh[3 * kAccStride + k]);
+}
+
+template <int WAVES = kWavesPerBlock, int IN_FLIGHT = kReduceInFlight>
+__device__ inline void reduce_partials(const float* __restrict__ partials, int pair, int tiles, double* sh, double* sums) {
+  reduce_partials_rows<WAVES, IN_FLIGHT>(partials, pair, tiles, sh);
   __syncthreads();
-  if (threadIdx.x < kAccStride) {
-    const int k = threadIdx.x;
-    sums[k] = (sh[k] + sh[kAccStride + k]) + (sh[2 * kAccStride + k] + sh[3 * kAccStride + k]);
-  }
+  if (threadIdx.x < kAccStride) reduce_partials_combine(sh, sums);
   __syncthreads();
 }
 
diff --git a/dvo_slam_amd/csrc/small_sweep.h b/dvo_slam_amd/csrc/small_sweep.h
--- /dev/null
+++ b/dvo_slam_amd/csrc/small_sweep.h
@@ -0,0 +1,119 @@
+#pragma once
+#include "fast_sweep.h"
+
+namespace dvo_hip {
+
+constexpr int kSmallCells = 5376;
+
+template <int THREADS>
+__device__ __forceinline__ void small_stage_level(const LevelGeom& g, __amdgpu_buffer_rsrc_t curC, float2* img) {
+  constexpr int kLoads = (kSmallCells + THREADS - 1) / THREADS;
+  const int pitch = g.w + 2, cells = pitch * (g.h + 2);
+  const float inv_pitch = 1.0f / float(pitch);
+  f32x2 v[kLoads];
+#pragma unroll
+  for (int j = 0; j < kLoads; ++j) {
+    const int c = min(int(threadIdx.x) + j * THREADS, cells - 1);
+    int cy = int(float(c) * inv_pitch);
+    int cx = c - cy * pitch;
+    if (cx < 0) { cx += pitch; cy -= 1; }
+    if (cx >= pitch) { cx -= pitch; cy += 1; }
+    const int x = min(max(cx - 1, 0), g.w - 1), y = min(max(cy - 1, 0), g.h - 1);
+    v[j] = __builtin_bit_cast(f32x2, __builtin_amdgcn_raw_buffer_load_b64(curC, (y * g.w + x) * 8, 0, 0));
+  }
+#pragma unroll
+  for (int j = 0; j < kLoads; ++j) {
+    const int c = int(threadIdx.x) + j * THREADS;
+    if (c < cells) img[c] = make_float2(v[j].x, v[j].y);
+  }
+}
+
+struct SmallSweepSetup {
+  FastRcpSource no_table;
+  unsigned w2_bits, h2_bits;
+  float inv_w, nanv;
+  int segments;
+  __device__ __forceinline__ explicit SmallSweepSetup(const LevelGeom& g)
+      : no_table{__builtin_amdgcn_make_buffer_rsrc(static_cast<float*>(nullptr), 0, 0, 0x00020000), nullptr, 0},
+        w2_bits(__builtin_bit_cast(unsigned, float(g.w - 2))), h2_bits(__builtin_bit_cast(unsigned, float(g.h - 2))),
+        inv_w(1.0f / float(g.w)), nanv(__builtin_nanf("")), segments((g.w * g.h + kTileW - 1) / kTileW) {}
+};
+
+__device__ __forceinline__ void small_sweep_tile(const LevelGeom& g, const SmallSweepSetup& su, const float* KT, const FastWeights& wt,
+                                                 __amdgpu_buffer_rsrc_t refR, __amdgpu_buffer_rsrc_t resid, const float2* img, int tile, int wave4,
+                                                 int lane, int rows_per_wave, float* my, int* count) {
+  const int n_px = g.w * g.h, pitch = g.w + 2;
+  const FastRcpSource& no_table = su.no_table;
+  const unsigned w2_bits = su.w2_bits, h2_bits = su.h2_bits;
+  const float inv_w = su.inv_w, nanv = su.nanv;
+  const int segments = su.segments;
+  const int seg0 = tile * (kWavesPerBlock * rows_per_wave) + wave4;
+  f32x4 acc0 = {0.0f, 0.0f, 0.0f, 0.0f}, acc1 = {0.0f, 0.0f, 0.0f, 0.0f};
+  int n_valid = 0;
+  auto load_f = [&](int pixel) { return __builtin_bit_cast(float, __builtin_amdgcn_raw_buffer_load_b32(refR, pixel * 8 + 4, 0, 0)); };
+  struct Ref {
+    float z, i, left, right, up, down, tx, ty;
+  };
+  auto load_ref = [&](int seg) {
+    const int pc = min(seg * kTileW + lane, n_px - 1);
+    int row = int(float(pc) * inv_w);
+    int col = pc - row * g.w;
+    if (col < 0) { col += g.w; row -= 1; }
+    if (col >= g.w) { col -= g.w; row += 1; }
+    Ref r;
+    const f32x2 zi = __builtin_bit_cast(f32x2, __builtin_amdgcn_raw_buffer_load_b64(refR, pc * 8, 0, 0));
+    r.z = zi.x; r.i = zi.y;
+    r.left = load_f(pc - (col > 0 ? 1 : 0));
+    r.right = load_f(pc + (col < g.w - 1 ? 1 : 0));
+    r.up = load_f(pc - (row > 0 ? g.w : 0));
+    r.down = load_f(pc + (row < g.h - 1 ? g.w : 0));
+    r.tx = g.tx[col];
+    r.ty = g.ty[row];
+    return r;
+  };
+  Ref next = load_ref(min(seg0, segments - 1));
+#pragma unroll 1
+  for (int k = 0; k < rows_per_wave; ++k) {
+    const int seg = seg0 + k * kWavesPerBlock;
+    if (seg >= segments) break;
+    const Ref ref = next;
+    if (k + 1 < rows_per_wave) next = load_ref(min(seg + kWavesPerBlock, segments - 1));
+    const int idx = seg * kTileW + lane;
+    const bool in_image = idx < n_px;
+    const float z = in_image ? ref.z : nanv;
+    const float tx = ref.tx, ty = ref.ty;
+    float u, v, qz;
+    fast_project<0>(g, no_table, KT, fmaf(KT[0], tx, KT[2]), fmaf(KT[4], tx, KT[6]), fmaf(KT[8], tx, KT[10]), z, tx, ty, u, v, qz);
+    const unsigned long long ok_mask = __builtin_amdgcn_ballot_w64(__builtin_bit_cast(unsigned, u) <= w2_bits) &
+                                       __builtin_amdgcn_ballot_w64(__builtin_bit_cast(unsigned, v) <= h2_bits);
+    const bool ok = __builtin_amdgcn_inverse_ballot_w64(ok_mask);
+    const int u0 = int(u), v0 = int(v);
+    FastRow r;
+    r.z = z; r.i = ref.i;
+    r.gx = ref.right - ref.left;
+    r.gy = ref.down - ref.up;
+    r.qz = qz;
+    r.a1 = __builtin_amdgcn_fractf(u);
+    r.b1 = __builtin_amdgcn_fractf(v);
+    r.idx = v0 * pitch + u0;
+    f32x2 P[4][4];
+    {
+      FastLdsCellPtr q = (FastLdsCellPtr)(img + (ok ? r.idx : 0));
+#pragma unroll
+      for (int rr = 0; rr < 4; ++rr)
+#pragma unroll
+        for (int cc = 0; cc < 4; ++cc)
+          if ((rr == 1 || rr == 2) || (cc == 1 || cc == 2)) P[rr][cc] = q[rr * pitch + cc];
+    }
+    fast_row_tail<2, false, 0, false>(g, no_table, P, r, ok_mask, tx, ty, fmaf(tx, tx, 1.0f), wt, resid, in_image ? idx * 8 : 0x7ffffff8, 0, my, lane, acc0, acc1, n_valid);
+  }
+
+#pragma unroll
+  for (int i = 0; i < 4; ++i) {
+    my[((lane >> 4) * 4 + i) * 16 + (lane & 15)] = acc0[i];
+    my[256 + ((lane >> 4) * 4 + i) * 16 + (lane & 15)] = acc1[i];
+  }
+  if (lane == 0) *count = n_valid;
+}
+
+}
diff --git a/dvo_slam_amd/csrc/sweep_parts.h b/dvo_slam_amd/csrc/sweep_parts.h
--- a/dvo_slam_amd/csrc/sweep_parts.h
+++ b/dvo_slam_amd/csrc/sweep_parts.h
@@ -27,6 +27,36 @@
     t.A01 = make_float4(a01.x, a01.y, a01.z, a01.w); t.A11 = make_float4(a11.x, a11.y, a11.z, a11.w);
     t.B00 = make_float2(b00.x, b00.y); t.B10 = make_float2(b10.x, b10.y);
     t.B01 = make_float2(b01.x, b01.y); t.B11 = make_float2(b11.x, b11.y);
+  }
+};
+
+struct LdsTaps {
+  const float2* img;
+  int w, pitch;
+  float inv_w;
+  __device__ __forceinline__ void fetch(int base, PixelTaps& t) const {
+#pragma clang fp contract(off)
+    int v0 = int(float(base) * inv_w);
+    int u0 = base - v0 * w;
+    if (u0 < 0) { u0 += w; v0 -= 1; }
+    if (u0 >= w) { u0 -= w; v0 += 1; }
+    typedef const __attribute__((address_space(3))) f32x2* Cell;
+    const Cell q = (Cell)(img + (v0 * pitch + u0));
+    f32x2 c[4][4];
+#pragma unroll
+    for (int rr = 0; rr < 4; ++rr)
+#pragma unroll
+      for (int cc = 0; cc < 4; ++cc)
+        if ((rr == 1 || rr == 2) || (cc == 1 || cc == 2)) c[rr][cc] = q[rr * pitch + cc];
+    auto tap = [&](int rr, int cc, float4& A, float2& B) {
+      const f32x2 dx = (c[rr][cc + 1] - c[rr][cc - 1]) * 0.5f, dy = (c[rr + 1][cc] - c[rr - 1][cc]) * 0.5f;
+      A = make_float4(c[rr][cc].x, c[rr][cc].y, dx.x, dy.x);
+      B = make_float2(dx.y, dy.y);
+    };
+    tap(1, 1, t.A00, t.B00);
+    tap(1, 2, t.A10, t.B10);
+    tap(2, 1, t.A01, t.B01);
+    tap(2, 2, t.A11, t.B11);
   }
 };
 
```
